# nabeelscicom/DistilCodec_nabeel

Hardware: AMD Instinct MI355X
Metric: 24 kHz samples/s encode+decode at 1/8 GPU; code-index bit-exact vs CPU (higher is better)
Workload: dtype f32

## Files before the change

### distilcodec_nabeel_amd/_native.py

```python
from __future__ import annotations

import ctypes
import glob
import hashlib
import os

import torch

_PKG = os.path.dirname(os.path.abspath(__file__))
LIB_PATH = os.environ.get("DCX_LIB") or os.path.join(_PKG, "libdcx.so")
CSRC = os.path.join(_PKG, "csrc")
HEADER = os.path.join(os.path.dirname(_PKG), "include", "distilcodec_amd.h")

DCX_OK = 0
DCX_ERR_INVALID_ARG = -1
DCX_ERR_MISSING_WEIGHT = -2
DCX_ERR_STATE = -3
DCX_ERR_HIP = -4
DCX_ERR_OOM = -5
DCX_ERR_WORKSPACE = -6
DCX_ERR_UNSUPPORTED = -7
DCX_GEMM_F32 = 0
DCX_GEMM_X6 = 1
DCX_GEMM_BF16 = 2


class NativeUnavailable(RuntimeError):
    pass


class NativeError(RuntimeError):
    def __init__(self, status: int, msg: str):
        super().__init__(f"dcx status {status}: {msg}")
        self.status = status


class DcxConfig(ctypes.Structure):
    _fields_ = [
        ("sample_rate", ctypes.c_int32),
        ("n_fft", ctypes.c_int32), ("hop", ctypes.c_int32), ("win", ctypes.c_int32),
        ("n_mels", ctypes.c_int32),
        ("f_min", ctypes.c_float), ("f_max", ctypes.c_float),
        ("enc_depths", ctypes.c_int32 * 4), ("enc_dims", ctypes.c_int32 * 4),
        ("vq_dim", ctypes.c_int32), ("codebook_dim", ctypes.c_int32), ("codebook_size", ctypes.c_int32),
        ("gen_channels", ctypes.c_int32), ("gen_pre_k", ctypes.c_int32), ("gen_post_k", ctypes.c_int32),
        ("n_ups", ctypes.c_int32), ("up_rates", ctypes.c_int32 * 8), ("up_kernels", ctypes.c_int32 * 8),
        ("n_res", ctypes.c_int32), ("res_kernels", ctypes.c_int32 * 4),
        ("res_dilations", (ctypes.c_int32 * 4) * 4),
    ]


_P = ctypes.c_void_p
_I32 = ctypes.c_int32
_I64 = ctypes.c_int64
_SZ = ctypes.c_size_t

SIGNATURES = {
    "dcx_default_config": (None, [ctypes.POINTER(DcxConfig)]),
    "dcx_create": (ctypes.c_int, [ctypes.POINTER(DcxConfig), ctypes.POINTER(_P)]),
    "dcx_destroy": (None, [_P]),
    "dcx_last_error": (ctypes.c_char_p, [_P]),
    "dcx_status_string": (ctypes.c_char_p, [ctypes.c_int]),
    "dcx_abi_version": (ctypes.c_int, []),
    "dcx_build_id": (ctypes.c_char_p, []),
    "dcx_set_tensor": (ctypes.c_int, [_P, ctypes.c_char_p, _P, _I32, ctypes.POINTER(_I64)]),
    "dcx_finalize": (ctypes.c_int, [_P, _I32]),
    "dcx_set_num_codebooks": (ctypes.c_int, [_P, _I32]),
    "dcx_num_codebooks": (_I32, [_P]),
    "dcx_num_frames": (_I64, [_P, _I64]),
    "dcx_workspace_size": (_SZ, [_P, _I32, _I64]),
    "dcx_mel": (ctypes.c_int, [_P, _P, _I32, _I64, _P, _P, _SZ, _P]),
    "dcx_mel_linear": (ctypes.c_int, [_P, _P, _I32, _I64, _P, _P, _P, _SZ, _P]),
    "dcx_encode": (ctypes.c_int, [_P, _P, _I32, _I64, _P, _P, _SZ, _P]),
    "dcx_vq_encode": (ctypes.c_int, [_P, _P, _I32, _I64, _P, _P, _P, _P, _P, _SZ, _P]),
    "dcx_vq_decode": (ctypes.c_int, [_P, _P, _I32, _I64, _P, _P, _P, _SZ, _P]),
    "dcx_generate": (ctypes.c_int, [_P, _P, _I32, _I64, _P, _P, _SZ, _P]),
    "dcx_encode_decode": (ctypes.c_int, [_P, _P, _I32, _I64, _P, _P, _P, _SZ, _P]),
    "dcx_ragged_plan_size": (_I64, [_I32]),
    "dcx_ragged_plan": (ctypes.c_int, [_P, ctypes.POINTER(_I64), _I32, _P, _I64, ctypes.POINTER(_I64),
                                       ctypes.POINTER(_I64)]),
    "dcx_ragged_workspace_size": (_SZ, [_P, _I32, _I64]),
    "dcx_tokenize_ragged": (ctypes.c_int, [_P, _P, _P, _P, _I32, _I64, _I64, _P, _P, _P, _P, _SZ, _P]),
    "dcx_generate_ragged": (ctypes.c_int, [_P, _P, _P, _I32, _I64, _P, _P, _SZ, _P]),
    "dcx_decode_ragged": (ctypes.c_int, [_P, _P, _P, _I32, _I64, _P, _P, _P, _SZ, _P]),
    "dcx_transpose": (ctypes.c_int, [_P, _P, _I32, _I64, _I64, _P]),
    "dcx_mp3_info": (ctypes.c_int, [_P, _SZ, ctypes.POINTER(_I64), ctypes.POINTER(_I32), ctypes.POINTER(_I32)]),
    "dcx_mp3_decode": (ctypes.c_int, [_P, _SZ, _P, _I64]),
    "dcx_mp3_last_error": (ctypes.c_char_p, []),
    "dcx_mp3_stats": (ctypes.c_int, [ctypes.POINTER(_I64), ctypes.POINTER(_I64)]),
    "dcx_mp3_junk_bytes": (_I64, []),
    "dcx_mp3_bad_frames": (_I64, []),
    "dcx_resample_poly": (ctypes.c_int, [_P, _I32, _I64, _I64, _P, _I32, _I32, _I32, _I64, _P, _I64, _I64, _P]),
    "dcx_set_gemm_mode": (ctypes.c_int, [_P, _I32]),
    "dcx_get_gemm_mode": (_I32, [_P]),
    "dcx_set_split_k": (ctypes.c_int, [_P, _I32]),
    "dcx_set_knob": (ctypes.c_int, [_P, ctypes.c_char_p, _I32]),
    "dcx_get_knob": (ctypes.c_int, [_P, ctypes.c_char_p, ctypes.POINTER(_I32)]),
    "dcx_range_flags": (ctypes.c_int, [_P, ctypes.POINTER(_I32), _I32]),
    "dcx_conv_create": (ctypes.c_int, [_P, _P, _I32, _I32, _I32, _I32, _I32, _I32, ctypes.POINTER(_P)]),
    "dcx_conv_forward": (ctypes.c_int, [_P, _I32, _P, _I32, _I64, _P, _P, _P, _I32, _P]),
    "dcx_conv_destroy": (None, [_P]),
    "dcx_conv_last_kernel": (ctypes.c_char_p, [_P]),
    "dcx_conv_set_knob": (ctypes.c_int, [_P, ctypes.c_char_p, _I32]),
    "dcx_conv_set_h3": (ctypes.c_int, [_P, _I32]),
    "dcx_module_workspace_size": (_SZ, [_P, ctypes.c_char_p, _I32, _I64]),
    "dcx_module_io": (ctypes.c_int, [_P, ctypes.c_char_p, ctypes.POINTER(_I32), ctypes.POINTER(_I32), ctypes.POINTER(_I32)]),
    "dcx_module_forward": (ctypes.c_int, [_P, ctypes.c_char_p, _P, _I32, _I64, _I32, _P, _P, _SZ, _P]),
    "dcx_vq_rescore_stats": (ctypes.c_int, [_P, ctypes.POINTER(_I64), ctypes.POINTER(_I64), _I32]),
    "dcx_profile_enable": (ctypes.c_int, [_P, _I32]),
    "dcx_profile_reset": (ctypes.c_int, [_P]),
    "dcx_profile_count": (_I32, [_P]),
    "dcx_profile_read": (ctypes.c_int, [_P, _I32, ctypes.POINTER(ctypes.c_char_p), ctypes.POINTER(_I64),
                                        ctypes.POINTER(ctypes.c_double), ctypes.POINTER(ctypes.c_double),
                                        ctypes.POINTER(ctypes.c_double)]),
}

_lib = None


def source_build_id() -> str | None:
    names = sorted(os.path.basename(p) for ext in ("cpp", "hip", "h") for p in glob.glob(os.path.join(CSRC, f"*.{ext}")))
    if not names or not os.path.isfile(HEADER):
        return None
    h = hashlib.sha256()
    for path in [os.path.join(CSRC, n) for n in names] + [HEADER]:
        with open(path, "rb") as f:
            h.update(f.read())
    return h.hexdigest()[:16]


def lib() -> ctypes.CDLL:
    global _lib
    if _lib is not None:
        return _lib
    if not os.path.isfile(LIB_PATH):
        raise NativeUnavailable(f"{LIB_PATH} is missing: run `python -c 'import __graft_entry__ as g; g.build()'`")
    try:
        L = ctypes.CDLL(LIB_PATH)
    except OSError as e:
        raise NativeUnavailable(f"cannot load {LIB_PATH}: {e}") from e
    for name, (res, args) in SIGNATURES.items():
        f = getattr(L, name)
        f.restype = res
        f.argtypes = args
    if L.dcx_abi_version() != 4:
        raise NativeUnavailable("libdcx.so ABI version mismatch")
    if not os.environ.get("DCX_LIB"):
        want, have = source_build_id(), L.dcx_build_id().decode()
        if want is not None and have != want:
            raise NativeUnavailable(f"{LIB_PATH} is stale: built from sources {have}, the sources here hash to {want}; "
                                    f"rebuild with `make -C {CSRC}`")
    _lib = L
    return L


def config_from_dict(cfg: dict) -> DcxConfig:
    c = DcxConfig()
    lib().dcx_default_config(ctypes.byref(c))
    s, e, d, q = cfg["spec_transform"], cfg["encoder"], cfg["decoder"], cfg["quantizer"]
    c.sample_rate, c.n_fft, c.hop, c.win = s["sampling_rate"], s["n_fft"], s["hop_size"], s["win_size"]
    c.n_mels, c.f_min, c.f_max = s["num_mels"], float(s["fmin"]), float(s["fmax"] or s["sampling_rate"] // 2)
    for i in range(4):
        c.enc_depths[i], c.enc_dims[i] = e["depths"][i], e["dims"][i]
    c.vq_dim, c.codebook_dim, c.codebook_size = q["input_dim"], q["codebook_dim"], q["codebook_size"]
    c.gen_channels, c.gen_pre_k, c.gen_post_k = d["upsample_initial_channel"], d["pre_conv_kernel_size"], d["post_conv_kernel_size"]
    c.n_ups = len(d["upsample_rates"])
    for i, (u, k) in enumerate(zip(d["upsample_rates"], d["upsample_kernel_sizes"])):
        c.up_rates[i], c.up_kernels[i] = u, k
    c.n_res = len(d["resblock_kernel_sizes"])
    for i, (k, dl) in enumerate(zip(d["resblock_kernel_sizes"], d["resblock_dilation_sizes"])):
        c.res_kernels[i] = k
        for j, v in enumerate(dl):
            c.res_dilations[i][j] = v
    return c
```

### distilcodec_nabeel_amd/csrc/dcx_api.cpp

```cpp
#include "dcx_host.h"

namespace {

void prof_collect(dcx_codec* h) {
  if (h->pending.empty()) return;
  hipDeviceSynchronize();
  for (auto& r : h->pending) {
    float ms = 0.f;
    hipEventElapsedTime(&ms, h->events[r.ev0], h->events[r.ev1]);
    h->prof_launches[r.id] += 1;
    h->prof_ms[r.id] += ms;
    h->prof_flops[r.id] += r.flops;
    h->prof_bytes[r.id] += r.bytes;
  }
  h->pending.clear();
  h->ev_used = 0;
}

constexpr int kPlanMagic = 0x52414731, kPlanHead = 8;
enum { PLAN_MAGIC = 0, PLAN_BATCH, PLAN_FRAMES, PLAN_SAMPLES, PLAN_T16, PLAN_T4, PLAN_RUN, PLAN_RW };
constexpr int64_t kRaggedMaxSamples = INT32_MAX, kRaggedMaxFrames = 1 << 20, kRaggedMaxBatch = 1 << 20;
int64_t plan_words(int64_t batch) { return kPlanHead + 5 * (batch + 1); }

bool seg_from_plan(const int32_t* host, const int32_t* dev, int64_t batch, int64_t samples, int64_t frames,
                   dcx::RaggedSeg& g) {
  if (host[PLAN_MAGIC] != kPlanMagic || host[PLAN_BATCH] != batch || host[PLAN_FRAMES] != frames ||
      host[PLAN_SAMPLES] != samples || batch < 1 || batch > kRaggedMaxBatch || frames < batch ||
      frames > kRaggedMaxFrames)
    return false;
  const int64_t n = batch + 1;
  const int32_t* a = dev + kPlanHead;
  g.cu_samples = a;
  g.cu_frames = a + n;
  g.cu_t16 = a + 2 * n;
  g.cu_t4 = a + 3 * n;
  g.cu_run = a + 4 * n;
  g.batch = (int)batch;
  g.rows = (int)frames;
  g.n_t16 = host[PLAN_T16];
  g.n_t4 = host[PLAN_T4];
  g.n_run = host[PLAN_RUN];
  g.rw = host[PLAN_RW];
  return g.rw == dcx::dwconv_run_rows(frames) && g.n_t16 >= batch && g.n_t16 <= frames && g.n_t4 >= g.n_t16 &&
         g.n_t4 <= frames && g.n_run >= batch && g.n_run <= frames;
}

int check_ready(dcx_codec* h, bool need_gen) {
  if (!h) return DCX_ERR_INVALID_ARG;
  if (!h->finalized) return fail(h, DCX_ERR_STATE, "dcx_finalize has not been called");
  if (need_gen && !h->has_gen) return fail(h, DCX_ERR_STATE, "generator weights were not finalized");
  int dev = -1;
  hipGetDevice(&dev);
  if (dev != h->device) return fail(h, DCX_ERR_STATE, "handle belongs to another HIP device");
  return DCX_OK;
}

int check_clip(dcx_codec* h, int64_t n) {
  if (n <= (h->cfg.win - h->cfg.hop) / 2 || frames_of(h->cfg, n) < 1)
    return fail(h, DCX_ERR_INVALID_ARG, "clip too short for the reflect pad / one STFT frame");
  return DCX_OK;
}

}

extern "C" {

int dcx_abi_version(void) { return DCX_ABI_VERSION; }

#ifndef DCX_BUILD_ID
#define DCX_BUILD_ID "unversioned"
#endif
const char* dcx_build_id(void) { return DCX_BUILD_ID; }

const char* dcx_status_string(int st) {
  switch (st) {
    case DCX_OK: return "ok";
    case DCX_ERR_INVALID_ARG: return "invalid argument";
    case DCX_ERR_MISSING_WEIGHT: return "missing weight";
    case DCX_ERR_STATE: return "invalid state";
    case DCX_ERR_HIP: return "HIP error";
    case DCX_ERR_OOM: return "out of device memory";
    case DCX_ERR_WORKSPACE: return "workspace too small";
    case DCX_ERR_UNSUPPORTED: return "unsupported input format";
    default: return "unknown status";
  }
}

void dcx_default_config(dcx_config* c) {
  std::memset(c, 0, sizeof(*c));
  c->sample_rate = 24000;
  c->n_fft = 1024; c->hop = 256; c->win = 1024; c->n_mels = 128;
  c->f_min = 0.f; c->f_max = 12000.f;
  const int dep[4] = {3, 3, 9, 3}, dim[4] = {256, 512, 768, 1024};
  for (int i = 0; i < 4; ++i) { c->enc_depths[i] = dep[i]; c->enc_dims[i] = dim[i]; }
  c->vq_dim = 1024; c->codebook_dim = 3584; c->codebook_size = 32768;
  c->gen_channels = 1024; c->gen_pre_k = 13; c->gen_post_k = 13;
  c->n_ups = 5;
  const int ur[5] = {8, 4, 2, 2, 2}, uk[5] = {16, 12, 4, 4, 4};
  for (int i = 0; i < 5; ++i) { c->up_rates[i] = ur[i]; c->up_kernels[i] = uk[i]; }
  c->n_res = 3;
  const int rk[3] = {3, 7, 11};
  for (int i = 0; i < 3; ++i) {
    c->res_kernels[i] = rk[i];
    c->res_dilations[i][0] = 1; c->res_dilations[i][1] = 3; c->res_dilations[i][2] = 5;
  }
}

const char* dcx_last_error(const dcx_codec* h) { return h ? h->err.c_str() : "null handle"; }

int dcx_create(const dcx_config* cfg, dcx_codec** out) {
  if (!cfg || !out) return DCX_ERR_INVALID_ARG;
  *out = nullptr;
  const dcx_config& c = *cfg;
  bool ok = c.n_fft == 1024 && c.win == 1024 && c.hop == 256 && c.n_mels % 16 == 0 && c.n_mels > 0 &&
            c.vq_dim == c.enc_dims[3] && c.codebook_dim % 16 == 0 && c.codebook_size % 128 == 0 &&
            c.n_ups >= 1 && c.n_ups <= 8 && c.n_res == 3 && c.gen_pre_k % 2 == 1 && c.gen_post_k % 2 == 1;
  for (int i = 0; i < 4 && ok; ++i) ok = c.enc_dims[i] % 256 == 0 && c.enc_dims[i] <= 1024 && c.enc_depths[i] >= 0;
  int ch = c.gen_channels;
  for (int i = 0; i < c.n_ups && ok; ++i) {
    ok = c.up_rates[i] >= 1 && c.up_rates[i] <= dcx::kMaxPhases && c.up_kernels[i] % c.up_rates[i] == 0 &&
         (c.up_kernels[i] - c.up_rates[i]) % 2 == 0;
    ch /= 2;
    ok = ok && ch % 32 == 0;
  }
  ok = ok && (ch == 32 || ch == 64);
  for (int i = 0; i < 3 && ok; ++i) ok = c.res_kernels[i] % 2 == 1;
  if (!ok) return DCX_ERR_INVALID_ARG;
  auto h = new (std::nothrow) dcx_codec();
  if (!h) return DCX_ERR_OOM;
  h->cfg = c;
  hipGetDevice(&h->device);
  const char* nrp = std::getenv("DCX_NO_RESPAIR");
  h->res_pair = !(nrp && nrp[0] == '1');
  const char* ncp = std::getenv("DCX_NO_COMPACT");
  h->compact = !(ncp && ncp[0] == '1');
  const char* vpr = std::getenv("DCX_VQ_PAIRS_PER_ROW");
  if (vpr && vpr[0]) h->vq_pairs_per_row = std::max(0, std::atoi(vpr));
  knobs_from_env(h->knobs);
  *out = h;
  return DCX_OK;
}

void dcx_destroy(dcx_codec* h) {
  if (!h) return;
  for (void* p : h->allocs) hipFree(p);
  for (auto e : h->events) hipEventDestroy(e);
  if (h->fork_ev) hipEventDestroy(h->fork_ev);
  if (h->join_ev) hipEventDestroy(h->join_ev);
  if (h->side) hipStreamDestroy(h->side);
  delete h;
}

int dcx_set_tensor(dcx_codec* h, const char* name, const float* data, int32_t ndim, const int64_t* shape) {
  if (!h || !name || (!data && ndim > 0) || ndim < 0 || ndim > 8) return fail(h, DCX_ERR_INVALID_ARG, "bad tensor");
  if (h->finalized) return fail(h, DCX_ERR_STATE, "dcx_set_tensor after dcx_finalize");
  HostTensor t;
  t.shape.assign(shape, shape + ndim);
  const int64_t n = t.numel();
  if (n < 0) return fail(h, DCX_ERR_INVALID_ARG, "negative shape");
  t.data.assign(data, data + n);
  h->host[name] = std::move(t);
  return DCX_OK;
}

int dcx_finalize(dcx_codec* h, int32_t with_generator) {
  if (!h) return DCX_ERR_INVALID_ARG;
  if (h->finalized) return fail(h, DCX_ERR_STATE, "already finalized");
  int rc = build_weights(h, true, with_generator);
  if (rc != DCX_OK) return rc;
  rc = build_weights(h, false, with_generator);
  if (rc != DCX_OK) return rc;
  h->has_gen = with_generator != 0;
  if (hipStreamCreateWithFlags(&h->side, hipStreamNonBlocking) != hipSuccess ||
      hipEventCreateWithFlags(&h->fork_ev, hipEventDisableTiming) != hipSuccess ||
      hipEventCreateWithFlags(&h->join_ev, hipEventDisableTiming) != hipSuccess)
    return fail(h, DCX_ERR_HIP, "dcx_finalize: stream / event creation failed");
  h->finalized = true;
  h->host.clear();
  return DCX_OK;
}

int dcx_set_num_codebooks(dcx_codec* h, int32_t n) {
  if (!h) return DCX_ERR_INVALID_ARG;
  if (h->finalized) return fail(h, DCX_ERR_STATE, "dcx_set_num_codebooks after dcx_finalize");
  if (n < 1 || n > DCX_MAX_CODEBOOKS)
    return fail(h, DCX_ERR_INVALID_ARG, "n_codebooks must be in [1, " + std::to_string(DCX_MAX_CODEBOOKS) + "]");
  h->n_layers = n;
  return DCX_OK;
}

int32_t dcx_num_codebooks(const dcx_codec* h) { return h ? h->n_layers : 0; }

int64_t dcx_num_frames(const dcx_codec* h, int64_t n) { return h ? frames_of(h->cfg, n) : 0; }

size_t dcx_workspace_size(const dcx_codec* h, int32_t batch, int64_t frames) {
  if (!h || batch <= 0 || frames <= 0) return 0;
  dcx_codec* hh = const_cast<dcx_codec*>(h);
  const int64_t n = (frames - 1) * h->cfg.hop + h->cfg.n_fft - (h->cfg.win - h->cfg.hop);
  Bump d(nullptr, 0, true);
  stage_encode_decode(hh, nullptr, batch, n, nullptr, nullptr, d, 0);
  size_t need = d.off;
  Bump q(nullptr, 0, true);
  stage_vq_encode(hh, CAct(), batch, (int)frames, nullptr, nullptr, nullptr, nullptr, q, 0);
  need = std::max(need, q.off + (size_t)batch * frames * (h->cfg.codebook_dim + h->cfg.vq_dim) * 4 + 1024);
  if (h->split_k > 1) need += kSplitScratch + 256;
  return need + 4096;
}

struct CallScope {
  dcx_codec* h;
  bool owner = false;
  explicit CallScope(dcx_codec* hh) : h(hh) {
    int expect = 0;
    owner = h && h->busy.compare_exchange_strong(expect, 1);
  }
  ~CallScope() {
    if (owner) {
      h->split_buf = nullptr;
      h->busy.store(0);
    }
  }
};

#define STAGE_PRE(need_gen)                                           \
  int rc_ = check_ready(h, need_gen);                                 \
  if (rc_ != DCX_OK) return rc_;                                      \
  if (batch <= 0) return fail(h, DCX_ERR_INVALID_ARG, "batch must be > 0"); \
  CallScope scope_(h);                                                \
  if (!scope_.owner) return fail(h, DCX_ERR_STATE, "handle in use by a concurrent call (serialise calls per handle)"); \
  hipStream_t s = (hipStream_t)stream;                                \
  Bump ws(workspace, ws_bytes, false);                                \
  h->split_buf = h->split_k > 1 ? (float*)ws.raw(kSplitScratch) : nullptr

int dcx_mel(dcx_codec* h, const float* audio, int32_t batch, int64_t n, float* mel, void* workspace, size_t ws_bytes,
            void* stream) {
  STAGE_PRE(false);
  if (!audio || !mel) return fail(h, DCX_ERR_INVALID_ARG, "null buffer");
  RUN(check_clip(h, n));
  return stage_mel(h, audio, batch, n, Act{mel, nullptr}, ws, s);
}

int dcx_mel_linear(dcx_codec* h, const float* audio, int32_t batch, int64_t n, float* mel, float* log_linear,
                   void* workspace, size_t ws_bytes, void* stream) {
  STAGE_PRE(false);
  if (!audio || !mel || !log_linear) return fail(h, DCX_ERR_INVALID_ARG, "null buffer");
  RUN(check_clip(h, n));
  return stage_mel(h, audio, batch, n, Act{mel, nullptr}, ws, s, log_linear);
}

int dcx_encode(dcx_codec* h, const float* mel, int32_t batch, int64_t frames, float* feat, void* workspace,
               size_t ws_bytes, void* stream) {
  STAGE_PRE(false);
  if (!mel || !feat || frames <= 0) return fail(h, DCX_ERR_INVALID_ARG, "bad arguments");
  return stage_encode(h, CAct(mel, nullptr), batch, (int)frames, Act{feat, nullptr}, ws, s);
}

int dcx_vq_encode(dcx_codec* h, const float* feat, int32_t batch, int64_t frames, int32_t* codes, float* x_pjt_in,
                  float* quantized_fup, float* quantized, void* workspace, size_t ws_bytes, void* stream) {
  STAGE_PRE(false);
  if (!feat || !codes || frames <= 0) return fail(h, DCX_ERR_INVALID_ARG, "bad arguments");
  return stage_vq_encode(h, CAct(feat, nullptr), batch, (int)frames, codes, x_pjt_in, quantized_fup, quantized, ws, s);
}

int dcx_vq_decode(dcx_codec* h, const int32_t* codes, int32_t batch, int64_t frames, float* z, int32_t* n_invalid,
                  void* workspace, size_t ws_bytes, void* stream) {
  STAGE_PRE(false);
  if (!codes || !z || frames <= 0) return fail(h, DCX_ERR_INVALID_ARG, "bad arguments");
  return stage_vq_decode(h, codes, batch, (int)frames, Act{z, nullptr}, n_invalid, ws, s);
}

int dcx_generate(dcx_codec* h, const float* z, int32_t batch, int64_t frames, float* wav, void* workspace,
                 size_t ws_bytes, void* stream) {
  STAGE_PRE(true);
  if (!z || !wav || frames <= 0) return fail(h, DCX_ERR_INVALID_ARG, "bad arguments");
  return stage_generate(h, CAct(z, nullptr), batch, (int)frames, wav, ws, s);
}

int dcx_encode_decode(dcx_codec* h, const float* audio, int32_t batch, int64_t n, int32_t* codes, float* wav,
                      void* workspace, size_t ws_bytes, void* stream) {
  STAGE_PRE(true);
  if (!audio || !codes || !wav) return fail(h, DCX_ERR_INVALID_ARG, "null buffer");
  RUN(check_clip(h, n));
  return stage_encode_decode(h, audio, batch, n, codes, wav, ws, s);
}

int64_t dcx_ragged_plan_size(int32_t batch) { return batch < 1 ? 0 : plan_words(batch); }

int dcx_ragged_plan(dcx_codec* h, const int64_t* clip_samples, int32_t batch, int32_t* plan, int64_t n_words,
                    int64_t* total_samples, int64_t* total_frames) {
  if (!h) return DCX_ERR_INVALID_ARG;
  if (batch < 1 || batch > kRaggedMaxBatch) return fail(h, DCX_ERR_INVALID_ARG, "ragged plan: batch must be in [1, 2^20]");
  if (!clip_samples || !plan) return fail(h, DCX_ERR_INVALID_ARG, "ragged plan: null buffer");
  if (n_words < plan_words(batch))
    return fail(h, DCX_ERR_INVALID_ARG, "ragged plan: the table holds " + std::to_string(n_words) + " words, " +
                                            std::to_string(plan_words(batch)) + " needed (dcx_ragged_plan_size)");
  const int64_t pad = (h->cfg.win - h->cfg.hop) / 2;
  const int64_t n = (int64_t)batch + 1;
  int32_t *cs = plan + kPlanHead, *cf = cs + n, *c16 = cf + n, *c4 = c16 + n, *cr = c4 + n;
  int64_t samples = 0, frames = 0;
  for (int32_t b = 0; b < batch; ++b) {
    const int64_t nb = clip_samples[b];
    if (nb < pad)
      return fail(h, DCX_ERR_INVALID_ARG, "ragged plan: clip " + std::to_string(b) + " has " + std::to_string(nb) +
                                              " samples, fewer than the reflect pad's " + std::to_string(pad));
    if (nb > kRaggedMaxSamples - samples)
      return fail(h, DCX_ERR_INVALID_ARG, "ragged plan: more than 2^31 - 1 samples in all (at clip " + std::to_string(b) + ")");
    samples += nb;
    frames += frames_of(h->cfg, nb + 1);
    if (frames > kRaggedMaxFrames)
      return fail(h, DCX_ERR_INVALID_ARG, "ragged plan: more than 2^20 frames in all (at clip " + std::to_string(b) + ")");
  }
  const int rw = dcx::dwconv_run_rows(frames);
  cs[0] = cf[0] = c16[0] = c4[0] = cr[0] = 0;
  for (int32_t b = 0; b < batch; ++b) {
    const int64_t T = frames_of(h->cfg, clip_samples[b] + 1);
    cs[b + 1] = (int32_t)(cs[b] + clip_samples[b]);
    cf[b + 1] = (int32_t)(cf[b] + T);
    c16[b + 1] = (int32_t)(c16[b] + (T + 15) / 16);
    c4[b + 1] = (int32_t)(c4[b] + (T + 3) / 4);
    cr[b + 1] = (int32_t)(cr[b] + (T + rw - 1) / rw);
  }
  plan[PLAN_MAGIC] = kPlanMagic;
  plan[PLAN_BATCH] = batch;
  plan[PLAN_FRAMES] = (int32_t)frames;
  plan[PLAN_SAMPLES] = (int32_t)samples;
  plan[PLAN_T16] = c16[batch];
  plan[PLAN_T4] = c4[batch];
  plan[PLAN_RUN] = cr[batch];
  plan[PLAN_RW] = rw;
  if (total_samples) *total_samples = samples;
  if (total_frames) *total_frames = frames;
  return DCX_OK;
}

size_t dcx_ragged_workspace_size(const dcx_codec* h, int32_t batch, int64_t total_frames) {
  if (!h || batch < 1 || total_frames < batch || total_frames > kRaggedMaxFrames) return 0;
  dcx::RaggedSeg g{};
  g.batch = batch;
  g.rows = (int)total_frames;
  Bump d(nullptr, 0, true);
  tokenize_ragged_rows(const_cast<dcx_codec*>(h), nullptr, g, nullptr, nullptr, nullptr, d, 0);
  return d.off + 4096;
}

int dcx_tokenize_ragged(dcx_codec* h, const float* audio_packed, const int32_t* plan_dev, const int32_t* plan_host,
                        int32_t batch, int64_t total_samples, int64_t total_frames, int32_t* codes, float* x_pjt_in,
                        float* quantized_fup, void* workspace, size_t ws_bytes, void* stream) {
  STAGE_PRE(false);
  if (!audio_packed || !plan_dev || !plan_host || !codes) return fail(h, DCX_ERR_INVALID_ARG, "null buffer");
  if (h->gemm_mode == DCX_GEMM_F32)
    return fail(h, DCX_ERR_INVALID_ARG, "dcx_tokenize_ragged runs in DCX_GEMM_X6 or DCX_GEMM_BF16 (the packed tensors are planes)");
  if (h->split_k >= 2)
    return fail(h, DCX_ERR_STATE, "dcx_tokenize_ragged with split-K on: the partial sums share one scratch region");
  dcx::RaggedSeg g{};
  if (!seg_from_plan(plan_host, plan_dev, batch, total_samples, total_frames, g))
    return fail(h, DCX_ERR_INVALID_ARG, "ragged plan does not match batch / total_samples / total_frames (dcx_ragged_plan)");
  return tokenize_ragged_rows(h, audio_packed, g, codes, x_pjt_in, quantized_fup, ws, s);
}

static int ragged_decode_pre(dcx_codec* h, const void* in, const int32_t* lengths_dev, int64_t frames_max,
                             const float* wav) {
  if (!in || !lengths_dev || !wav || frames_max <= 0 || frames_max > INT32_MAX / 256)
    return fail(h, DCX_ERR_INVALID_ARG, "ragged decode: null buffer or bad frames_max");
  if (h->split_k >= 2)
    return fail(h, DCX_ERR_STATE, "ragged decode with split-K on: the split kernels' reduce is not length-aware");
  if (h->gemm_mode != DCX_GEMM_X6)
    return fail(h, DCX_ERR_INVALID_ARG, "ragged decode runs in DCX_GEMM_X6 (the other modes' kernels are not length-aware)");
  return DCX_OK;
}

int dcx_generate_ragged(dcx_codec* h, const float* z, const int32_t* lengths_dev, int32_t batch, int64_t frames_max,
                        float* wav, void* workspace, size_t ws_bytes, void* stream) {
  if (h && (!z || !lengths_dev)) return fail(h, DCX_ERR_INVALID_ARG, "ragged decode: null buffer");
  STAGE_PRE(true);
  RUN(ragged_decode_pre(h, z, lengths_dev, frames_max, wav));
  return stage_generate(h, CAct(z, nullptr), batch, (int)frames_max, wav, ws, s, lengths_dev);
}

int dcx_decode_ragged(dcx_codec* h, const int32_t* codes, const int32_t* lengths_dev, int32_t batch,
                      int64_t frames_max, float* wav, int32_t* n_invalid, void* workspace, size_t ws_bytes,
                      void* stream) {
  if (h && (!codes || !lengths_dev)) return fail(h, DCX_ERR_INVALID_ARG, "ragged decode: null buffer");
  STAGE_PRE(true);
  RUN(ragged_decode_pre(h, codes, lengths_dev, frames_max, wav));
  return stage_decode_ragged(h, codes, lengths_dev, batch, (int)frames_max, wav, n_invalid, ws, s);
}

int dcx_module_io(const dcx_codec* h, const char* module, int32_t* in_channels, int32_t* out_channels,
                  int32_t* out_rate) {
  if (!h || !module) return DCX_ERR_INVALID_ARG;
  int ci = 0, co = 0, r = 1;
  if (!module_io(h, module, ci, co, r)) return DCX_ERR_INVALID_ARG;
  if (in_channels) *in_channels = ci;
  if (out_channels) *out_channels = co;
  if (out_rate) *out_rate = r;
  return DCX_OK;
}

size_t dcx_module_workspace_size(const dcx_codec* h, const char* module, int32_t batch, int64_t rows) {
  if (!h || !module || batch <= 0 || rows <= 0 || !h->finalized) return 0;
  Bump d(nullptr, 0, true);
  if (stage_module(const_cast<dcx_codec*>(h), module, nullptr, batch, (int)rows, nullptr, d, 0) != DCX_OK) return 0;
  return d.off + 4096 + (h->split_k > 1 ? kSplitScratch + 256 : 0);
}

int dcx_module_forward(dcx_codec* h, const char* module, const float* x, int32_t batch, int64_t rows,
                       int32_t channels, void* y, void* workspace, size_t ws_bytes, void* stream) {
  STAGE_PRE(false);
  if (!module || !x || !y || rows <= 0 || rows > (1 << 30)) return fail(h, DCX_ERR_INVALID_ARG, "bad arguments");
  int ci = 0, co = 0, r = 1;
  if (!module_io(h, module, ci, co, r)) return fail(h, DCX_ERR_INVALID_ARG, std::string("unknown module: ") + module);
  if (channels != ci)
    return fail(h, DCX_ERR_INVALID_ARG, std::string(module) + " takes " + std::to_string(ci) + " input channels, got " +
                                            std::to_string(channels));
  return stage_module(h, module, x, batch, (int)rows, y, ws, s);
}

int dcx_transpose(const float* in, float* out, int32_t batch, int64_t rows, int64_t cols, void* stream) {
  if (!in || !out || batch <= 0 || rows <= 0 || cols <= 0) return DCX_ERR_INVALID_ARG;
  return dcx::launch_transpose(in, out, batch, rows, cols, (hipStream_t)stream) == hipSuccess ? DCX_OK : DCX_ERR_HIP;
}

int dcx_resample_poly(const float* x, int32_t batch, int64_t n_in, int64_t x_stride, const double* h, int32_t h_len,
                      int32_t up, int32_t down, int64_t pre, float* y, int64_t n_out, int64_t y_stride, void* stream) {
  if (!x || !h || !y || batch <= 0 || n_in <= 0 || n_out <= 0 || h_len <= 0 || up <= 0 || down <= 0 || pre < 0 ||
      x_stride < n_in || y_stride < n_out || batch > 65535)
    return DCX_ERR_INVALID_ARG;
  if ((pre + n_out) > (INT64_MAX / down)) return DCX_ERR_INVALID_ARG;
  return dcx::launch_resample_poly(x, batch, n_in, x_stride, h, h_len, up, down, pre, y, n_out, y_stride,
                                   (hipStream_t)stream) == hipSuccess
             ? DCX_OK
             : DCX_ERR_HIP;
}

int dcx_set_gemm_mode(dcx_codec* h, int32_t mode) {
  if (!h) return DCX_ERR_INVALID_ARG;
  if (mode != DCX_GEMM_F32 && mode != DCX_GEMM_X6 && mode != DCX_GEMM_BF16)
    return fail(h, DCX_ERR_INVALID_ARG, "unknown GEMM mode");
  h->gemm_mode = mode;
  return DCX_OK;
}

int32_t dcx_get_gemm_mode(const dcx_codec* h) { return h ? h->gemm_mode : -1; }

int dcx_set_split_k(dcx_codec* h, int32_t max_splits) {
  if (!h || max_splits < 0 || max_splits > kSplitMax) return DCX_ERR_INVALID_ARG;
  h->split_k = max_splits;
  return DCX_OK;
}

int dcx_set_knob(dcx_codec* h, const char* name, int32_t value) {
  if (!h || !name) return DCX_ERR_INVALID_ARG;
  CallScope scope(h);
  if (!scope.owner) return fail(h, DCX_ERR_STATE, "dcx_set_knob during a stage call");
  const auto k = knob_slot(name);
  if (!k) return fail(h, DCX_ERR_INVALID_ARG, std::string("unknown knob: ") + name);
  h->knobs.*k = value;
  return DCX_OK;
}

int dcx_get_knob(const dcx_codec* h, const char* name, int32_t* value) {
  if (!h || !name || !value) return DCX_ERR_INVALID_ARG;
  const auto k = knob_slot(name);
  if (!k) return DCX_ERR_INVALID_ARG;
  *value = h->knobs.*k;
  return DCX_OK;
}

int dcx_range_flags(dcx_codec* h, int32_t* flags, int32_t reset) {
  if (!h || !flags) return DCX_ERR_INVALID_ARG;
  *flags = 0;
  if (!h->rflag) return DCX_OK;
  int v = 0;
  if (hipDeviceSynchronize() != hipSuccess || hipMemcpy(&v, h->rflag, sizeof v, hipMemcpyDeviceToHost) != hipSuccess)
    return fail(h, DCX_ERR_HIP, "reading the range flags failed");
  *flags = v;
  if (reset && hipMemset(h->rflag, 0, sizeof v) != hipSuccess) return fail(h, DCX_ERR_HIP, "resetting the range flags failed");
  return DCX_OK;
}

}

struct dcx_conv {
  dcx_codec scratch;
  ConvW w;
  unsigned short* planes = nullptr;
  size_t planes_cap = 0;
  bool h3 = false;
  int* range = nullptr;
  size_t range_cap = 0;
};

template <class T>
static bool grow(T*& p, size_t& cap, size_t need) {
  if (need <= cap) return true;
  if (p) hipFree(p);
  p = nullptr;
  cap = 0;
  if (hipMalloc(&p, need * sizeof(T)) != hipSuccess) return false;
  cap = need;
  return true;
}

extern "C" {

int dcx_conv_create(const float* weight, const float* bias, int32_t cin, int32_t cout, int32_t k, int32_t dilation,
                    int32_t transposed, int32_t stride, dcx_conv** out) {
  if (!weight || !out || cin <= 0 || cout <= 0 || k <= 0 || dilation <= 0 || stride <= 0) return DCX_ERR_INVALID_ARG;
  if (cin % 16 || cout % 32) return DCX_ERR_INVALID_ARG;
  if (transposed && (k % stride || (k - stride) % 2 || stride > dcx::kMaxPhases)) return DCX_ERR_INVALID_ARG;
  if (!transposed && (k % 2 == 0)) return DCX_ERR_INVALID_ARG;
  auto c = new (std::nothrow) dcx_conv();
  if (!c) return DCX_ERR_OOM;
  dcx_codec* h = &c->scratch;
  HostTensor wt;
  const int64_t n = (int64_t)cin * cout * k;
  wt.shape = transposed ? std::vector<int64_t>{cin, cout, k} : std::vector<int64_t>{cout, cin, k};
  wt.data.assign(weight, weight + n);
  h->host["c.weight"] = wt;
  HostTensor bt;
  bt.shape = {cout};
  if (bias) bt.data.assign(bias, bias + cout); else bt.data.assign(cout, 0.f);
  h->host["c.bias"] = bt;
  const int code = build_conv(h, cin, cout, k, dilation, transposed != 0, stride, c->w);
  h->host.clear();
  if (code != DCX_OK) {
    dcx_conv_destroy(c);
    return code;
  }
  *out = c;
  return DCX_OK;
}

int dcx_conv_forward(dcx_conv* c, int32_t gemm_mode, const float* x, int32_t batch, int64_t lin, float* y,
                     float* y_silu, const float* res, int32_t epi, void* stream) {
  if (!c || !x || batch <= 0 || lin <= 0 || (!y && !y_silu)) return DCX_ERR_INVALID_ARG;
  if (epi != dcx::EPI_BIAS && epi != dcx::EPI_GELU && epi != dcx::EPI_RES) return DCX_ERR_INVALID_ARG;
  if (epi == dcx::EPI_RES && !res) return DCX_ERR_INVALID_ARG;
  dcx_codec* h = &c->scratch;
  h->gemm_mode = gemm_mode;
  hipStream_t s = (hipStream_t)stream;
  CAct xa(x, nullptr);
  if (gemm_mode != DCX_GEMM_F32 && gemm_mode != DCX_GEMM_X6 && gemm_mode != DCX_GEMM_BF16) return DCX_ERR_INVALID_ARG;
  if (gemm_mode != DCX_GEMM_F32 && !f32_input_ok(c->w)) {
    const size_t need = (size_t)batch * lin * c->w.cin * 3;
    if (!grow(c->planes, c->planes_cap, need)) return DCX_ERR_OOM;
    const bool h3 = c->h3 && (c->w.taps >= 2 ? takes_h3_conv(h, c->w, lin) : takes_h3(h, c->w));
    if (h3) {
      const long long rows = (long long)batch * lin;
      const size_t words = (size_t)batch + (size_t)std::max<long long>(batch, rows);
      if (!grow(c->range, c->range_cap, words)) return DCX_ERR_OOM;
      float* am = reinterpret_cast<float*>(c->range);
      int* ash = c->range + batch;
      xa.r = Rng{};
      if (c->w.taps >= 2) {
        if (dcx::launch_h2_ranged(x, nullptr, c->planes, batch, lin, c->w.cin, 0, 0.f, am, ash, h->rflag, s) != hipSuccess)
          return fail(h, DCX_ERR_HIP, "h3 input split (per clip) failed");
        xa.r.ash = ash;
        xa.r.amax = am;
      } else {
        if (dcx::launch_h2_rows(x, c->planes, rows, c->w.cin, ash, s) != hipSuccess)
          return fail(h, DCX_ERR_HIP, "h3 input split (per row) failed: Cin must be 256, 512, 768, 1024 or a multiple of 32 below 256");
        xa.r.ash_row = ash;
      }
      xa.lay = dcx::LAYOUT_H2;
    } else if (dcx::launch_split_planes(x, c->planes, (long long)batch * lin, c->w.cin, dcx::LAYOUT_PLANES, s) != hipSuccess) {
      return DCX_ERR_HIP;
    }
    xa.p = c->planes;
  }
  ConvCall cc = framed(xa, batch, (int)lin, c->w.cin);
  cc.y = y;
  cc.y2 = y_silu;
  cc.res = res;
  cc.epi = epi;
  return run_conv(h, c->w, cc, s);
}

void dcx_conv_destroy(dcx_conv* c) {
  if (!c) return;
  if (c->planes) hipFree(c->planes);
  if (c->range) hipFree(c->range);
  for (void* p : c->scratch.allocs) hipFree(p);
  delete c;
}

const char* dcx_conv_last_kernel(const dcx_conv* c) { return c ? c->scratch.last_kname : ""; }

int dcx_conv_set_knob(dcx_conv* c, const char* name, int32_t value) {
  if (!c || !name) return DCX_ERR_INVALID_ARG;
  const auto k = knob_slot(name);
  if (!k) return fail(&c->scratch, DCX_ERR_INVALID_ARG, std::string("unknown knob: ") + name);
  c->scratch.knobs.*k = value;
  return DCX_OK;
}

int dcx_conv_set_h3(dcx_conv* c, int32_t on) {
  if (!c) return DCX_ERR_INVALID_ARG;
  c->h3 = on != 0;
  return DCX_OK;
}

int dcx_profile_enable(dcx_codec* h, int32_t on) {
  if (!h) return DCX_ERR_INVALID_ARG;
  h->prof = on != 0;
  return DCX_OK;
}

int dcx_profile_reset(dcx_codec* h) {
  if (!h) return DCX_ERR_INVALID_ARG;
  prof_collect(h);
  for (size_t i = 0; i < h->prof_names.size(); ++i) {
    h->prof_launches[i] = 0;
    h->prof_ms[i] = h->prof_flops[i] = h->prof_bytes[i] = 0;
  }
  return DCX_OK;
}

int dcx_vq_rescore_stats(dcx_codec* h, int64_t* rows_rescored, int64_t* codes_rescored, int32_t reset) {
  if (!h || !h->vq_stats) return DCX_ERR_STATE;
  h->vq_stats_on = true;
  int v[2] = {0, 0};
  if (hipDeviceSynchronize() != hipSuccess || hipMemcpy(v, h->vq_stats, sizeof v, hipMemcpyDeviceToHost) != hipSuccess)
    return fail(h, DCX_ERR_HIP, "reading VQ rescore counters failed");
  if (rows_rescored) *rows_rescored = v[0];
  if (codes_rescored) *codes_rescored = v[1];
  if (reset && hipMemset(h->vq_stats, 0, sizeof v) != hipSuccess)
    return fail(h, DCX_ERR_HIP, "resetting VQ rescore counters failed");
  return DCX_OK;
}

int32_t dcx_profile_count(const dcx_codec* h) { return h ? (int32_t)h->prof_names.size() : 0; }

int dcx_profile_read(dcx_codec* h, int32_t i, const char** name, int64_t* launches, double* ms, double* flops,
                     double* bytes) {
  if (!h) return DCX_ERR_INVALID_ARG;
  prof_collect(h);
  if (i < 0 || i >= (int32_t)h->prof_names.size()) return DCX_ERR_INVALID_ARG;
  if (name) *name = h->prof_names[i].c_str();
  if (launches) *launches = h->prof_launches[i];
  if (ms) *ms = h->prof_ms[i];
  if (flops) *flops = h->prof_flops[i];
  if (bytes) *bytes = h->prof_bytes[i];
  return DCX_OK;
}

}
```

### distilcodec_nabeel_amd/csrc/dcx_conv_common.h

```cpp
#pragma once
#include <algorithm>
#include <type_traits>

#include "dcx_kernels.h"
#include "dcx_planes.h"

namespace dcx {

typedef float f32x16 __attribute__((ext_vector_type(16)));
typedef float f32x4 __attribute__((ext_vector_type(4)));
typedef float f32x2 __attribute__((ext_vector_type(2)));
typedef short s16x8 __attribute__((ext_vector_type(8)));
typedef short s16x4 __attribute__((ext_vector_type(4)));
typedef __bf16 bf16x8 __attribute__((ext_vector_type(8)));

constexpr int BK = 16;
constexpr int LDSK = 20;
template <bool SWZ>
struct XRow {
  static constexpr int kStride = SWZ ? 48 : 56;
  __device__ static __forceinline__ int half(int row, int h) { return SWZ ? h ^ ((row >> 3) & 1) : h; }
  __device__ static __forceinline__ int off(int row, int piece) {
    const int h = piece >= 3;
    return row * kStride + (half(row, h) * 3 + piece - 3 * h) * 8;
  }
};

__device__ __forceinline__ float silu_f(float v) { return v * __builtin_amdgcn_rcpf(1.0f + __expf(-v)); }
__device__ __forceinline__ float gelu_f(float v) { return 0.5f * v * (1.0f + erff(v * 0.70710678118654752440f)); }
__device__ __forceinline__ float gelu_bf16_f(float v) {
#ifdef DCX_GELU_ERF
  return gelu_f(v);
#endif
  const float z = fabsf(v) * 0.70710678118654752440f;
  const float t = __builtin_amdgcn_rcpf(fmaf(0.5f, z, 1.0f));
  float q = 0.17087277f;
  q = fmaf(q, t, -0.82215223f);
  q = fmaf(q, t, 1.48851587f);
  q = fmaf(q, t, -1.13520398f);
  q = fmaf(q, t, 0.27886807f);
  q = fmaf(q, t, -0.18628806f);
  q = fmaf(q, t, 0.09678418f);
  q = fmaf(q, t, 0.37409196f);
  q = fmaf(q, t, 1.00002368f);
  const float c = t * __expf(fmaf(t, q, fmaf(-z, z, -1.26551223f)));
  const float e = v >= 0.0f ? 1.0f - c : c - 1.0f;
  return 0.5f * v * (1.0f + e);
}

__device__ __forceinline__ f32x2 gelu_bf16_f2(f32x2 v) {
#ifdef DCX_GELU_SCALAR
  return f32x2{gelu_bf16_f(v[0]), gelu_bf16_f(v[1])};
#endif
  const f32x2 z = __builtin_elementwise_abs(v) * 0.70710678118654752440f;
  const f32x2 d = __builtin_elementwise_fma(f32x2{0.5f, 0.5f}, z, f32x2{1.0f, 1.0f});
  const f32x2 t = {__builtin_amdgcn_rcpf(d[0]), __builtin_amdgcn_rcpf(d[1])};
  auto fm = [&](f32x2 q, float c) { return __builtin_elementwise_fma(q, t, f32x2{c, c}); };
  f32x2 q = {0.17087277f, 0.17087277f};
  q = fm(q, -0.82215223f);
  q = fm(q, 1.48851587f);
  q = fm(q, -1.13520398f);
  q = fm(q, 0.27886807f);
  q = fm(q, -0.18628806f);
  q = fm(q, 0.09678418f);
  q = fm(q, 0.37409196f);
  q = fm(q, 1.00002368f);
  const f32x2 arg = __builtin_elementwise_fma(t, q, __builtin_elementwise_fma(-z, z, f32x2{-1.26551223f, -1.26551223f}));
  const f32x2 c = t * f32x2{__expf(arg[0]), __expf(arg[1])};
  const f32x2 e = {v[0] >= 0.0f ? 1.0f - c[0] : c[0] - 1.0f, v[1] >= 0.0f ? 1.0f - c[1] : c[1] - 1.0f};
  return 0.5f * v * (1.0f + e);
}

__device__ __forceinline__ int xcd_remap(int bid, int nwg) {
  const int xcd = bid & 7, q = nwg >> 3, r = nwg & 7;
  return (xcd < r ? xcd * (q + 1) : r * (q + 1) + (xcd - r) * q) + (bid >> 3);
}

__device__ __forceinline__ void flat_tile(int tpc, int batch, int& wg, int& b, int& ph) {
  const int t = xcd_remap(blockIdx.x, gridDim.x);
  const int per_ph = tpc * batch;
  ph = t / per_ph;
  const int r = t - ph * per_ph;
  b = r / tpc;
  wg = r - b * tpc;
}

__device__ __forceinline__ void ksplit_slice(const ConvParams& p, int b, int& clip, int& c0, int& nchunks) {
  clip = b;
  c0 = 0;
  nchunks = p.Cin / BK;
  if (p.ksplit > 1) {
    const int clips = p.batch / p.ksplit, sl = b / clips;
    clip = b - sl * clips;
    const int nunits = nchunks / p.kunit, base = nunits / p.ksplit, extra = nunits % p.ksplit;
    c0 = (sl * base + min(sl, extra)) * p.kunit;
    nchunks = (base + (sl < extra ? 1 : 0)) * p.kunit;
  }
}

static __device__ __attribute__((used, aligned(16))) float g_zero_row[32] = {0.f};

#if defined(DCX_CLOCK_DIAG) || defined(DCX_SEG_DIAG) || defined(DCX_TILE_DIAG)
#define DCX_DIAG 1
constexpr int kTileDiagMax = 16384;
[[maybe_unused]] static __device__ unsigned long long g_clock_diag[3], g_seg_diag[13], g_seg_diag8[49];
[[maybe_unused]] static __device__ unsigned long long g_tile_diag[kTileDiagMax * 6];
[[maybe_unused]] static __device__ unsigned int g_tile_cnt;
enum DiagSet : int { DIAG_CLOCK, DIAG_SEG, DIAG_SEG8, DIAG_TILES };
static int diag_read(int set, unsigned long long* out, int n, int reset) {
  if (set == DIAG_TILES) {
    unsigned int cnt = 0;
    if (hipMemcpyFromSymbol(&cnt, HIP_SYMBOL(g_tile_cnt), sizeof cnt) != hipSuccess) return -1;
    cnt = std::min(cnt, (unsigned)std::max(0, std::min(n, kTileDiagMax)));
    if (cnt && hipMemcpyFromSymbol(out, HIP_SYMBOL(g_tile_diag), sizeof(unsigned long long) * 6 * cnt) != hipSuccess) return -1;
    const unsigned int z = 0;
    if (reset && hipMemcpyToSymbol(HIP_SYMBOL(g_tile_cnt), &z, sizeof z) != hipSuccess) return -1;
    return (int)cnt;
  }
  const void* sym = set == DIAG_CLOCK ? (const void*)g_clock_diag : set == DIAG_SEG ? (const void*)g_seg_diag : (const void*)g_seg_diag8;
  unsigned long long v[49] = {};
  if (n > 49 || hipMemcpyFromSymbol(v, sym, sizeof(unsigned long long) * n) != hipSuccess) return -1;
  for (int i = 0; i < n; ++i) out[i] += v[i];
  const unsigned long long z[49] = {};
  if (reset && hipMemcpyToSymbol(sym, z, sizeof(unsigned long long) * n) != hipSuccess) return -1;
  return 0;
}
#define DCX_DIAG_FILE(tag) \
  int diag_##tag(int set, unsigned long long* out, int n, int reset) { return diag_read(set, out, n, reset); }
#else
#define DCX_DIAG_FILE(tag)
#endif
#ifdef DCX_SEG_DIAG
#define DCX_SEGT(v) const unsigned long long v = __builtin_amdgcn_s_memtime()
#else
#define DCX_SEGT(v)
#endif
#ifdef DCX_TILE_DIAG
#define DCX_TILET(v) const unsigned long long v = __builtin_amdgcn_s_memrealtime()
#else
#define DCX_TILET(v)
#endif

struct EpiPre {
  int osh;
  float acur;
  bool track;
};
template <int RROW>
__device__ __forceinline__ EpiPre epi_range_pre(const ConvParams& p, const ConvParams& pr, int b) {
  EpiPre e{0, 0.f, false};
  const bool h2o = (p.y6 && p.y_layout == LAYOUT_H2) || (p.y6s && p.ys_layout != LAYOUT_PLANES);
  const bool h2row = (RROW & 2) && h2o && pr.yb.rowwise;
  if (h2o && !h2row) {
    const float bnd = range_bound(pr.yb, b);
    e.osh = __builtin_amdgcn_readfirstlane(h2_shift(bnd));
    if (threadIdx.x == 0) {
      if (pr.y_ash) pr.y_ash[b] = e.osh;
      if (pr.rflag && !(bnd <= 3.0e38f)) atomicOr(pr.rflag, RANGE_NONFINITE);
    }
  }
  const bool track = pr.y_amax != nullptr;
  e.track = track;
  e.acur = track && !h2row ? __builtin_bit_cast(float, __builtin_amdgcn_readfirstlane(
                                                           __builtin_bit_cast(int, range_cur(pr.y_amax, b))))
                           : 0.f;
  return e;
}

template <int BM, int BN, int WM, int WN, int LDS_FLOATS, int NT, int RROW = 2, bool RAG = true, typename AccT>
__device__ __forceinline__ void epilogue_lds(const ConvParams& p, const ConvParams& pr, AccT& acc, int q0, int co0,
                                             int b, int ph, float* smem, const EpiPre* pre = nullptr) {
  constexpr int WR = BM / WM, WC = BN / WN;
  constexpr int TM = WR / 32, TN = WC / 32;
  constexpr bool M16 = sizeof(acc[0][0]) == 16;
  static_assert(sizeof(acc) == WR * WC * 4 / 64, "accumulator tile");
  constexpr int LDSW = BN + 4;
  constexpr int RPP = (BM * LDSW <= LDS_FLOATS) ? BM
                      : (BM / 2 * LDSW <= LDS_FLOATS) ? BM / 2
                      : (BM / 4 * LDSW <= LDS_FLOATS) ? BM / 4 : WR;
  static_assert(RPP % WR == 0 && RPP * LDSW <= LDS_FLOATS, "epilogue pass does not fit LDS");
  const int tid = threadIdx.x, lane = tid & 63, wave = tid >> 6;
  const int wm = wave / WN, wn = wave % WN;
  const int lrow = lane & 31, rhalf = 4 * (lane >> 5);
  const long long ob = (long long)b * p.y_bstride;
  unsigned short* y6 = p.y6 ? p.y6 + ob * layout_u16(p.y_layout) : nullptr;
  unsigned short* y6s = p.y6s ? p.y6s + ob * (p.ys_layout != LAYOUT_PLANES ? 2 : 3) : nullptr;
  const bool h2o = (y6 && p.y_layout == LAYOUT_H2) || (y6s && p.ys_layout != LAYOUT_PLANES);
  constexpr bool RIN = RROW & 1, ROUT = RROW & 2;
  const bool h2row = ROUT && h2o && pr.yb.rowwise;
  int osh = 0;
  if (pre) {
    osh = pre->osh;
  } else if (h2o && !h2row) {
    const float bnd = range_bound(pr.yb, b);
    osh = __builtin_amdgcn_readfirstlane(h2_shift(bnd));
    if (tid == 0) {
      if (pr.y_ash) pr.y_ash[b] = osh;
      if (pr.rflag && !(bnd <= 3.0e38f)) atomicOr(pr.rflag, RANGE_NONFINITE);
    }
  }
  const float osc =
      __builtin_bit_cast(float, __builtin_amdgcn_readfirstlane(__builtin_bit_cast(int, __builtin_ldexpf(1.0f, osh))));
#ifdef DCX_DIAG_NORANGE
  const bool track = false;
#else
  const bool track = pre ? pre->track : pr.y_amax != nullptr;
#endif
  const float acur = pre ? pre->acur : track && !h2row ? range_cur(pr.y_amax, b) : 0.f;
  float vmax = 0.f;
  const int lq_live = RAG ? clip_rows(pr.clip_len, pr.len_mul, b, p.Lq) : p.Lq;
#ifdef DCX_EPI4
  constexpr int G = 4;
#else
  constexpr int G = 8;
#endif
  constexpr int NH = G / 4;
  static_assert(NT % (BN / G) == 0, "each thread keeps one channel group");
  const int cg = (tid % (BN / G)) * G, trow = tid / (BN / G), co = co0 + cg;
  const int hsw = G == 8 ? (lane >> 3) & 1 : 0;
  f32x4 bias4[NH], gamma4[NH];
#pragma unroll
  for (int h = 0; h < NH; ++h) {
    bias4[h] = p.bias ? *reinterpret_cast<const f32x4*>(p.bias + co + 4 * h) : f32x4{0.f, 0.f, 0.f, 0.f};
    gamma4[h] = p.epi == EPI_GAMMA_RES ? *reinterpret_cast<const f32x4*>(p.gamma + co + 4 * h) : f32x4{0.f, 0.f, 0.f, 0.f};
  }
#ifdef DCX_DIAG_NOEPI
  if (q0 >= 0) return;
#endif
#ifdef DCX_DIAG_DUP
  if (p.diag_skip == 2) return;
#endif
  auto stage_acc = [&](int r0) {
    __syncthreads();
    if (wm * WR >= r0 && wm * WR < r0 + RPP) {
      if constexpr (M16) {
#pragma unroll
        for (int i = 0; i < WR / 16; ++i)
#pragma unroll
          for (int j = 0; j < WC / 16; ++j)
#pragma unroll
            for (int e = 0; e < 4; ++e) {
              const int row = wm * WR + i * 16 + 4 * (lane >> 4) + e - r0;
              smem[row * LDSW + wn * WC + j * 16 + (lane & 15)] = acc[i][j][e];
            }
      } else {
#pragma unroll
        for (int i = 0; i < TM; ++i)
#pragma unroll
          for (int j = 0; j < TN; ++j)
#pragma unroll
            for (int r = 0; r < 16; ++r) {
              const int row = wm * WR + i * 32 + (r & 3) + 8 * (r >> 2) + rhalf - r0;
              smem[row * LDSW + wn * WC + j * 32 + lrow] = acc[i][j][r];
            }
      }
    }
    __syncthreads();
  };
  constexpr int RSTEP = NT / (BN / G), ROWS_T = RPP / RSTEP;
  static_assert(RPP % RSTEP == 0, "epilogue rows per thread");
  const bool need_r = p.epi == EPI_GAMMA_RES || p.epi == EPI_RES;
  const bool need_m = p.mean_mode == MEAN_MID || p.mean_mode == MEAN_LAST;
  auto batch = [&](int r0, int rb, bool stage, auto ibt) {
    constexpr int IB = decltype(ibt)::value;
    f32x4 r[IB][NH], m[IB][NH];
    auto lofs = [&](int k) {
      const int q = min(q0 + r0 + trow + (rb + k) * RSTEP, p.Lq - 1);
      return ob + ((long long)q * p.out_mul + ph) * p.ldy + co;
    };
    if (need_r) {
#pragma unroll
      for (int k = 0; k < IB; ++k)
#pragma unroll
        for (int h = 0; h < NH; ++h) r[k][h] = *reinterpret_cast<const f32x4*>(p.res + lofs(k) + 4 * h);
    }
    if (need_m) {
#pragma unroll
      for (int k = 0; k < IB; ++k)
#pragma unroll
        for (int h = 0; h < NH; ++h) m[k][h] = *reinterpret_cast<const f32x4*>(p.macc + lofs(k) + 4 * h);
    }
    auto row_bound = [&](int q) { return fmaf(pr.yb.g[0], fmaxf(pr.yb.m[0][(long long)b * p.Lq + q], pr.yb.f[0]), pr.yb.c); };
    float rin[RIN ? IB : 1], rbnd[RIN ? IB : 1];
    if constexpr (RIN) {
#pragma unroll
      for (int k = 0; k < IB; ++k) {
        const int q = min(q0 + r0 + trow + (rb + k) * RSTEP, p.Lq - 1);
        rin[k] = pr.x_ash_row ? __builtin_ldexpf(1.0f, -pr.x_ash_row[(long long)b * p.Lin + q]) : 1.0f;
        rbnd[k] = h2row ? row_bound(q) : 0.f;
      }
    }
    if (stage) stage_acc(r0);
#pragma unroll
    for (int k = 0; k < IB; ++k) {
      const int rl = trow + (rb + k) * RSTEP;
      const int q = q0 + r0 + rl;
      if (q >= p.Lq) continue;
      const long long orow = (long long)q * p.out_mul + ph;
      const long long o = ob + orow * p.ldy + co;
      f32x4 x[NH];
      const float rin_ = RIN ? rin[RIN ? k : 0] : 1.0f;
      if constexpr (NH == 2) {
        const f32x4 u = *reinterpret_cast<const f32x4*>(smem + rl * LDSW + cg + 4 * hsw);
        const f32x4 v = *reinterpret_cast<const f32x4*>(smem + rl * LDSW + cg + 4 * (1 - hsw));
        x[0] = (hsw ? v : u) * rin_ + bias4[0];
        x[1] = (hsw ? u : v) * rin_ + bias4[1];
      } else {
        x[0] = *reinterpret_cast<const f32x4*>(smem + rl * LDSW + cg) * rin_ + bias4[0];
      }
#pragma unroll
      for (int h = 0; h < NH; ++h) {
        if (p.round_bf16) x[h] = round_bf16x4(x[h]);
        switch (p.epi) {
          case EPI_GELU:
            if (p.w6) {
#ifndef DCX_EPI_NOGELU
#pragma unroll
              for (int e = 0; e < 4; e += 2) {
                const f32x2 g = gelu_bf16_f2(f32x2{x[h][e], x[h][e + 1]});
                x[h][e] = g[0];
                x[h][e + 1] = g[1];
              }
#endif
              if (p.round_bf16 && (p.y || y6s || p.y2 || p.y_layout != LAYOUT_BF16)) x[h] = round_bf16x4(x[h]);
            } else {
#pragma unroll
              for (int e = 0; e < 4; ++e) x[h][e] = gelu_f(x[h][e]);
            }
            break;
          case EPI_GAMMA_RES: x[h] = r[k][h] + gamma4[h] * x[h]; break;
          case EPI_RES:
            x[h] = r[k][h] + x[h];
            if (p.round_bf16) x[h] = round_bf16x4(x[h]);
            break;
          case EPI_LOGCLAMP:
#pragma unroll
            for (int e = 0; e < 4; ++e) x[h][e] = logf(fmaxf(x[h][e], 1e-5f));
            break;
          default: break;
        }
        if (RAG && q >= lq_live) x[h] = f32x4{0.f, 0.f, 0.f, 0.f};
      }
#ifdef DCX_EPI_NOSTORE
      if (x[0][0] != -0x1.234p-100f) continue;
#endif
#ifdef DCX_DIAG_DUP
      if (p.diag_skip == 1 && x[0][0] != -0x1.234p-100f) continue;
#endif
      if (p.mean_mode == MEAN_FIRST) {
#pragma unroll
        for (int h = 0; h < NH; ++h) *reinterpret_cast<f32x4*>(p.macc + o + 4 * h) = x[h];
        continue;
      } else if (p.mean_mode == MEAN_MID) {
#pragma unroll
        for (int h = 0; h < NH; ++h) *reinterpret_cast<f32x4*>(p.macc + o + 4 * h) = RAG && q >= lq_live ? x[h] : m[k][h] + x[h];
        continue;
      } else if (p.mean_mode == MEAN_LAST) {
#pragma unroll
        for (int h = 0; h < NH; ++h) {
          x[h] = RAG && q >= lq_live ? x[h] : (m[k][h] + x[h]) / 3.0f;
          if (p.round_bf16) x[h] = round_bf16x4(x[h]);
        }
      }
      float rsc = osc;
      if (h2row) {
        const long long grow = (long long)b * p.Lq + q;
        const float bnd = RIN ? rbnd[RIN ? k : 0] : row_bound(q);
        const int sh = h2_shift(bnd);
        rsc = __builtin_ldexpf(1.0f, sh);
        if (cg == 0 && pr.y_ash) pr.y_ash[grow] = sh;
        if (pr.rflag && !(bnd <= 3.0e38f)) atomicOr(pr.rflag, RANGE_NONFINITE);
      }
      if (track) {
        const float ts = h2row ? rsc : 1.0f;
#pragma unroll
        for (int h = 0; h < NH; ++h)
#pragma unroll
          for (int e = 0; e < 4; ++e) vmax = fmaxf(vmax, fabsf(x[h][e]) * ts);
      }
      if (p.y) {
#pragma unroll
        for (int h = 0; h < NH; ++h) *reinterpret_cast<f32x4*>(p.y + o + 4 * h) = x[h];
      }
      if constexpr (G == 8) {
        float xv[8];
#pragma unroll
        for (int e = 0; e < 8; ++e) xv[e] = x[e >> 2][e & 3];
        if (y6) {
          if (p.y_layout == LAYOUT_BF16) store_bf16x8(y6, orow, p.Cout, co, xv);
          else if ((int)p.y_layout == 2) store_hm8(y6, orow, p.Cout, co, xv);
          else if (p.y_layout == LAYOUT_H2) store_h2_8<false>(y6, orow, p.Cout, co, xv, rsc);
          else store_planes8(y6, orow, p.Cout, co, xv);
        }
        if (p.y2 || y6s) {
          float sv[8];
#pragma unroll
          for (int e = 0; e < 8; ++e) sv[e] = p.round_bf16 ? bf16_val(bf16_bits(silu_f(xv[e]))) : silu_f(xv[e]);
          if (p.y2) {
            *reinterpret_cast<f32x4*>(p.y2 + o) = f32x4{sv[0], sv[1], sv[2], sv[3]};
            *reinterpret_cast<f32x4*>(p.y2 + o + 4) = f32x4{sv[4], sv[5], sv[6], sv[7]};
          }
          if (y6s) {
            if (p.ys_layout != LAYOUT_PLANES) store_h2_8<false>(y6s, orow, p.Cout, co, sv, rsc);
            else store_planes8(y6s, orow, p.Cout, co, sv);
          }
        }
      } else {
        if (y6) {
          if (p.y_layout == LAYOUT_BF16) store_bf16x4(y6, orow, p.Cout, co, x[0][0], x[0][1], x[0][2], x[0][3]);
          else if ((int)p.y_layout == 2) store_hm4(y6, orow, p.Cout, co, x[0][0], x[0][1], x[0][2], x[0][3]);
          else if (p.y_layout == LAYOUT_H2) store_h2_4<false>(y6, orow, p.Cout, co, x[0][0], x[0][1], x[0][2], x[0][3], rsc);
          else store_planes4(y6, orow, p.Cout, co, x[0][0], x[0][1], x[0][2], x[0][3]);
        }
        if (p.y2 || y6s) {
          f32x4 sv;
#pragma unroll
          for (int e = 0; e < 4; ++e) sv[e] = p.round_bf16 ? bf16_val(bf16_bits(silu_f(x[0][e]))) : silu_f(x[0][e]);
          if (p.y2) *reinterpret_cast<f32x4*>(p.y2 + o) = sv;
          if (y6s) {
            if (p.ys_layout != LAYOUT_PLANES) store_h2_4<false>(y6s, orow, p.Cout, co, sv[0], sv[1], sv[2], sv[3], rsc);
            else store_planes4(y6s, orow, p.Cout, co, sv[0], sv[1], sv[2], sv[3]);
          }
        }
      }
    }
  };
  constexpr int IBF0 = 8 / NH, IBM0 = 4 / NH;
  constexpr auto div_cap = [](int n, int cap) {
    int d = n < cap ? n : cap;
    while (n % d) --d;
    return d;
  };
  constexpr int IBF = div_cap(ROWS_T, IBF0), IBM = div_cap(ROWS_T, IBM0);
  static_assert(ROWS_T % IBF == 0 && ROWS_T % IBM == 0, "epilogue batches");
#pragma unroll 1
  for (int r0 = 0; r0 < BM; r0 += RPP) {
    if (need_m) {
#pragma unroll
      for (int rb = 0; rb < ROWS_T; rb += IBM) batch(r0, rb, rb == 0, std::integral_constant<int, IBM>{});
    } else {
#pragma unroll
      for (int rb = 0; rb < ROWS_T; rb += IBF) batch(r0, rb, rb == 0, std::integral_constant<int, IBF>{});
    }
  }
  if (track)
    range_report_wg(vmax, h2row ? nullptr : pr.y_amax, b, h2row ? 65504.0f : h2o ? 65504.0f / osc : __builtin_inff(),
                    pr.rflag, acur, smem, NT);
}

__device__ __forceinline__ bool tile_dead(const ConvParams& p, const ConvParams& pr, int b, int q0) {
  return pr.clip_len != nullptr && q0 >= clip_rows(pr.clip_len, pr.len_mul, b, p.Lq);
}
template <int BM, int BN, int NT>
__device__ __forceinline__ void epilogue_dead(const ConvParams& p, const ConvParams& pr, int q0, int co0, int b, int ph) {
  const long long ob = (long long)b * p.y_bstride;
  unsigned short* y6 = p.y6 ? p.y6 + ob * layout_u16(p.y_layout) : nullptr;
  unsigned short* y6s = p.y6s ? p.y6s + ob * (p.ys_layout != LAYOUT_PLANES ? 2 : 3) : nullptr;
  const bool h2o = (y6 && p.y_layout == LAYOUT_H2) || (y6s && p.ys_layout != LAYOUT_PLANES);
  if (h2o && threadIdx.x == 0) {
    const float bnd = range_bound(pr.yb, b);
    if (pr.y_ash) pr.y_ash[b] = h2_shift(bnd);
    if (pr.rflag && !(bnd <= 3.0e38f)) atomicOr(pr.rflag, RANGE_NONFINITE);
  }
  const f32x4 z4 = {0.f, 0.f, 0.f, 0.f};
  const float z8[8] = {0.f, 0.f, 0.f, 0.f, 0.f, 0.f, 0.f, 0.f};
  constexpr int CG = BN / 8;
  for (int i = threadIdx.x; i < BM * CG; i += NT) {
    const int q = q0 + i / CG, co = co0 + (i % CG) * 8;
    if (q >= p.Lq) break;
    const long long orow = (long long)q * p.out_mul + ph;
    const long long o = ob + orow * p.ldy + co;
    if (p.mean_mode == MEAN_FIRST || p.mean_mode == MEAN_MID) {
      *reinterpret_cast<f32x4*>(p.macc + o) = z4;
      *reinterpret_cast<f32x4*>(p.macc + o + 4) = z4;
      continue;
    }
    if (p.y) {
      *reinterpret_cast<f32x4*>(p.y + o) = z4;
      *reinterpret_cast<f32x4*>(p.y + o + 4) = z4;
    }
    if (y6) {
      if (p.y_layout == LAYOUT_BF16) store_bf16x8(y6, orow, p.Cout, co, z8);
      else if (p.y_layout == LAYOUT_H2) store_h2_8<false>(y6, orow, p.Cout, co, z8, 1.0f);
      else store_planes8(y6, orow, p.Cout, co, z8);
    }
    if (p.y2) {
      *reinterpret_cast<f32x4*>(p.y2 + o) = z4;
      *reinterpret_cast<f32x4*>(p.y2 + o + 4) = z4;
    }
    if (y6s) {
      if (p.ys_layout != LAYOUT_PLANES) store_h2_8<false>(y6s, orow, p.Cout, co, z8, 1.0f);
      else store_planes8(y6s, orow, p.Cout, co, z8);
    }
  }
}

typedef __attribute__((address_space(3))) void* lds_ptr_t;

__device__ __forceinline__ void dma16(__amdgpu_buffer_rsrc_t r, unsigned short* lds, int voff, int soff) {
  __builtin_amdgcn_raw_ptr_buffer_load_lds(r, (lds_ptr_t)lds, 16, voff, soff, 0, 0);
}
__device__ __forceinline__ void seg_barrier() { asm volatile("s_waitcnt lgkmcnt(0)\n\ts_barrier" ::: "memory"); }
__device__ __forceinline__ void wait_dma(int n) {
#define DCX_W(k) \
  case k: asm volatile("s_waitcnt vmcnt(" #k ")" ::: "memory"); break;
  switch (n) {
    DCX_W(1) DCX_W(2) DCX_W(3) DCX_W(4) DCX_W(5) DCX_W(6) DCX_W(7) DCX_W(8) DCX_W(9) DCX_W(10) DCX_W(11)
    DCX_W(12) DCX_W(13) DCX_W(14) DCX_W(15) DCX_W(16) DCX_W(17) DCX_W(18) DCX_W(19) DCX_W(20) DCX_W(21) DCX_W(22)
    DCX_W(23)
    default: asm volatile("s_waitcnt vmcnt(0)" ::: "memory");
  }
#undef DCX_W
}

}
```

### distilcodec_nabeel_amd/csrc/dcx_conv_h3.hip

```cpp
#include "dcx_conv_common.h"
#include "dcx_conv_launch.h"
#include "dcx_conv_pingpong.h"
#include "dcx_a3_layout.h"
#include "dcx_w3_layout.h"

namespace dcx {

DCX_DIAG_FILE(h3)

typedef _Float16 f16x8 __attribute__((ext_vector_type(8)));

template <int BM, int BN>
__device__ __forceinline__ bool ragged_tile_done(const ConvParams& p, const ConvParams& pr, int wg, int b, int ph) {
  int q0, co0;
  tile_origin<BM, BN>(p, wg, q0, co0);
  if (!tile_dead(p, pr, b, q0)) return false;
  epilogue_dead<BM, BN, 512>(p, pr, q0, co0, b, ph);
  return true;
}

template <int BN, int HALO, bool RAG = false>
__device__ __forceinline__ void x3dq_tile(const ConvParams& p, const ConvParams& pr, const int wg, const int b, const int ph) {
  constexpr int BM = 32768 / BN, WN = BN / 64, WM = 8 / WN;
  constexpr int NA = HALO ? 2 : 3;
  constexpr int WR = BM / WM, WC = BN / WN, TM = WR / 16, TN = WC / 16;
  constexpr int AR = BM + HALO;
  constexpr int A_G = AR / 16, B_G = BN / 16;
  constexpr int A_PW = A_G / 4, B_PW = B_G / 4;
  constexpr int ABUF = AR * 128, BBUF = BN * 128;
  constexpr int LDS_B = NA * ABUF + 3 * BBUF;
  static_assert(WR == 64 && WC == 64 && A_G % 4 == 0 && B_G % 4 == 0 && AR % 64 == 0, "tile shape");
  static_assert(LDS_B <= 160 * 1024, "LDS");
  __shared__ __attribute__((aligned(16))) unsigned short lds[LDS_B / 2];

  if constexpr (RAG)
    if (ragged_tile_done<BM, BN>(p, pr, wg, b, ph)) return;
  const TileGeo g = tile_geo<BM, BN, WN>(p, wg, ph, p.Cin / 32);
  const int lane = g.lane, group = g.group, gw = g.gw, wm = g.wm, wn = g.wn, q0 = g.q0, co0 = g.co0;
  const int nchunks = g.nchunks, taps = g.taps, nsteps = g.nsteps, lo_rel = g.lo_rel, row0 = g.row0;
  const int arow = p.ldx * 4;
  const __amdgpu_buffer_rsrc_t rx = x_desc<4, HALO>(p, b, row0, BM);
  const int rbase = HALO ? row0 : 0;
  const __amdgpu_buffer_rsrc_t rw = __builtin_amdgcn_make_buffer_rsrc(
      (void*)(p.w3 + w3_step(taps, p.Cin, p.Cout, ph, 0, 0)), 0, taps * nchunks * p.Cout * 128, 0x00020000);

  int a_off[A_PW], b_off[B_PW];
#pragma unroll
  for (int i = 0; i < A_PW; ++i) {
    const int u = (group * A_G + i * 4 + gw) * 64;
    const int pc = u / AR, row = u - pc * AR + lane;
    a_off[i] = (rbase + row) * arow + (pc & 3) * 32 + (pc >> 2) * 16;
  }
#pragma unroll
  for (int i = 0; i < B_PW; ++i) {
    b_off[i] = w3_wide_lane(co0, lane) + w3_wide_piece(BN, group * B_G + i * 4 + gw);
  }
  unsigned short* const a_dst = lds + (group * A_G + gw) * 512;
  unsigned short* const b_dst = lds + NA * ABUF / 2 + (group * B_G + gw) * 512;
  [[maybe_unused]] bool in_loop = false;
  auto dma_step = [&](int c, int m, int slot) {
#ifdef DCX_X3_NODMA
    if (in_loop) return 0;
#endif
    int n = B_PW;
    if (m == 0) {
#pragma unroll
      for (int i = 0; i < A_PW; ++i)
        dma16(rx, a_dst + (HALO ? (c & 1) : slot) * (ABUF / 2) + i * 2048, a_off[i] + c * 128, 0);
      n += A_PW;
    }
    const int soff = w3_step_bytes(nchunks, p.Cout, m, c);
#pragma unroll
    for (int i = 0; i < B_PW; ++i) dma16(rw, b_dst + slot * (BBUF / 2) + i * 2048, b_off[i], soff);
    return n;
  };

  const int l15 = lane & 15, kg = lane >> 4;
  const int pah = kg * AR * 16, pal = (4 + kg) * AR * 16;
  const int pbh = kg * BN * 16, pbl = (4 + kg) * BN * 16;
  const char* const ldsb = reinterpret_cast<const char*>(lds);
  const int bcol = NA * ABUF + (wn * WC + l15) * 16;
  s16x8 aq[TM][2], bq[TN][2];
  auto readF = [&](int c, int m, int slot) {
    const char* a = ldsb + (HALO ? (c & 1) : slot) * ABUF + (wm * WR + m * p.in_step - lo_rel + l15) * 16;
    const char* bb = ldsb + bcol + slot * BBUF;
#pragma unroll
    for (int j = 0; j < TN; ++j) {
      bq[j][0] = *reinterpret_cast<const s16x8*>(bb + j * 256 + pbh);
      bq[j][1] = *reinterpret_cast<const s16x8*>(bb + j * 256 + pbl);
    }
#pragma unroll
    for (int i = 0; i < TM; ++i) {
      aq[i][0] = *reinterpret_cast<const s16x8*>(a + i * 256 + pah);
      aq[i][1] = *reinterpret_cast<const s16x8*>(a + i * 256 + pal);
    }
  };
  f32x4 acc[TM][TN];
  zero_acc(acc);
  auto mfma = [&]() {
    __builtin_amdgcn_s_setprio(1);
#pragma unroll
    for (int k = 0; k < 3; ++k) {
      const int sa = k == 1 ? 1 : 0, sb = k == 0 ? 1 : 0;
#pragma unroll
      for (int i = 0; i < TM; ++i)
#pragma unroll
        for (int j = 0; j < TN; ++j)
          acc[i][j] = __builtin_amdgcn_mfma_f32_16x16x32_f16(__builtin_bit_cast(f16x8, aq[i][sa]),
                                                             __builtin_bit_cast(f16x8, bq[j][sb]), acc[i][j], 0, 0, 0);
    }
    __builtin_amdgcn_s_setprio(0);
  };

  const StepPos l3 = pingpong3_prologue(nsteps, taps, dma_step);
  const EpiPre epre = epi_range_pre<HALO == 0 ? 3 : 0>(p, pr, b);
  const float unscale = __builtin_bit_cast(float, __builtin_amdgcn_readfirstlane(__builtin_bit_cast(int,
      __builtin_ldexpf(1.0f, -(p.w3_shift + (pr.x_ash ? pr.x_ash[b] : pr.x_ash_c))))));
  pingpong3_drain();
  in_loop = true;
  pingpong3_loop<true>(group, nsteps, taps, l3, dma_step, readF, mfma);
#pragma unroll
  for (int i = 0; i < TM; ++i)
#pragma unroll
    for (int j = 0; j < TN; ++j) acc[i][j] *= unscale;
  epilogue_lds<BM, BN, WM, WN, LDS_B / 4, 512, HALO == 0 ? 3 : 0, RAG>(p, pr, acc, q0, co0, b, ph, reinterpret_cast<float*>(lds), &epre);
}

template <int BN, int HALO, bool RAG = false>
__global__ void __launch_bounds__(512, 2) conv_gemm_x3dq(const ConvParams p) {
  int wg, b, ph;
  flat_tile(((p.Lq + 32768 / BN - 1) / (32768 / BN)) * (p.Cout / BN), p.batch, wg, b, ph);
  x3dq_tile<BN, HALO, RAG>(p, p, wg, b, ph);
}

template <int BN, bool RAG = false>
__global__ void __launch_bounds__(512, 2) conv_gemm_x3dq_group(const ConvGroup g) {
  ConvParams p;
  int local, b;
  const ConvParams& pr = group_member(g, p, local, b);
  x3dq_tile<BN, 64, RAG>(p, pr, local, b, 0);
}

template <int HALO, bool SPLIT, int BN = 256, bool RAG = false, bool GROUPED = false>
__device__ __forceinline__ void x3dw_tile(const ConvParams& p, const ConvParams& pr, const int wg, const int b, const int ph) {
  constexpr int BM = BN == 256 ? 256 : 384, WN = BN / 128, WM = 8 / WN;
  constexpr int WR = BM / WM, WC = 128, TM = WR / 16, TN = WC / 16;
  constexpr int AR = BM + HALO;
  constexpr int A_N = AR / 8, B_N = BN / 8;
  constexpr int A_PW = A_N / 4;
  constexpr int ABUF = AR * 128, BBUF = BN * 128;
  constexpr int NA = 2;
  constexpr int LDS_B = NA * ABUF + 2 * BBUF;
  static_assert(A_N % 4 == 0 && B_N % 4 == 0 && AR % 64 == 0, "tile shape");
  static_assert(LDS_B + 16 <= 160 * 1024, "LDS");
  __shared__ __attribute__((aligned(16))) unsigned short lds[LDS_B / 2 + 8];
  unsigned int* const rd_cnt = reinterpret_cast<unsigned int*>(lds + LDS_B / 2);

  const int tid = threadIdx.x, lane = tid & 63;
  [[maybe_unused]] const int wave = tid >> 6;
  const int group = __builtin_amdgcn_readfirstlane(tid >> 8);
  const int gw = __builtin_amdgcn_readfirstlane((tid >> 6) & 3);
  const int wm = wave / WN, wn = wave % WN;
  const int ntiles = p.Cout / BN;
  const int mt = wg / ntiles, nt = wg - mt * ntiles;
  const int q0 = mt * BM, co0 = nt * BN;
  if (RAG && tile_dead(p, pr, b, q0)) {
    epilogue_dead<BM, BN, 512>(p, pr, q0, co0, b, ph);
    return;
  }
  const int nchunks = p.Cin / 32;
  const int taps = p.taps;
  const int nsteps = nchunks * taps;
  const int lo_rel = p.in_step < 0 ? (taps - 1) * p.in_step : 0;
  const int row0 = q0 + p.in_base[ph] + lo_rel;
  const int arow = p.ldx * 4;
  const __amdgpu_buffer_rsrc_t rx = x_desc<4, HALO>(p, b, row0, BM);
  const int rbase = HALO ? row0 : 0;
  const __amdgpu_buffer_rsrc_t rw = __builtin_amdgcn_make_buffer_rsrc(
      (void*)(p.w3 + w3_step(taps, p.Cin, p.Cout, ph, 0, 0)), 0, taps * nchunks * p.Cout * 128, 0x00020000);

  constexpr bool ROWS = !(HALO && !SPLIT && BN == 256 && !RAG && !GROUPED);
  const int a_lane = ROWS ? a3_src_lane(rbase, arow, lane) : (rbase + lane) * arow;
  const int b_lane = w3_wide_lane(co0, lane);
  [[maybe_unused]] bool in_loop = false;
  auto dmaA1 = [&](int c, int slot, int i) {
#ifdef DCX_X3_NODMA
    if (in_loop) return;
#endif
    const int k = i * 4 + gw;
    const int abuf = HALO ? (c & 1) : slot;
    if constexpr (ROWS) {
      dma16(rx, lds + abuf * (ABUF / 2) + k * 512, a_lane + a3_src_inst(arow, k, c), 0);
    } else {
      const int u = k * 64, pc = u / AR, row = u - pc * AR;
      dma16(rx, lds + abuf * (ABUF / 2) + k * 512, a_lane + row * arow + (pc & 3) * 32 + (pc >> 2) * 16 + c * 128, 0);
    }
  };
#ifndef DCX_X3W_BG0_DIV
#define DCX_X3W_BG0_DIV 2
#endif
  constexpr int B_G0 = !SPLIT ? B_N : HALO ? B_N / DCX_X3W_BG0_DIV : 0;
  constexpr int B_W0 = B_G0 / 4, B_W1 = (B_N - B_G0) / 4;
  auto dmaB1 = [&](int c, int m, int slot, int i) {
#ifdef DCX_X3_NODMA
    if (in_loop) return;
#endif
    const int k = (group ? B_G0 : 0) + i * 4 + gw;
    dma16(rw, lds + NA * ABUF / 2 + slot * (BBUF / 2) + k * 512, b_lane, w3_step_bytes(nchunks, p.Cout, m, c) + w3_wide_piece(BN, k));
  };
  auto dma_step = [&](int c, int m, int slot) {
    if (m == 0) {
#pragma unroll
      for (int i = 0; i < A_PW; ++i) dmaA1(c, slot, i);
    }
#pragma unroll
    for (int i = 0; i < B_W0; ++i) dmaB1(c, m, slot, i);
  };
  auto dma_step1 = [&](int c, int m, int slot) {
#pragma unroll
    for (int i = 0; i < B_W1; ++i) dmaB1(c, m, slot, i);
  };

  const int l15 = lane & 15, kg = lane >> 4;
  const char* const ldsb = reinterpret_cast<const char*>(lds);
  const int a_row = wm * WR + l15;
  static_assert(WR % kA3BlockRows == 0 && a3_image(16, 0) == 2048, "row blocks as immediates");
  const char* const b_rd = ldsb + NA * ABUF + kg * BN * 16 + (wn * WC + l15) * 16;
  s16x8 aq[TM][2], bq[TN][2];
  auto readF = [&](int c, int m, int slot) {
    const int a_r = a_row + (HALO ? m * p.in_step - lo_rel : 0);
    const int ah = (HALO ? (c & 1) : slot) * ABUF + (ROWS ? a3_image(a_r, kg) : kg * AR * 16 + a_r * 16);
    const char* a = ldsb + ah;
    const char* al = ldsb + (ROWS ? ah ^ kA3PlaneXor : ah + 4 * AR * 16);
    const char* bb = b_rd + slot * BBUF;
#pragma unroll
    for (int j = 0; j < TN; ++j) {
      bq[j][0] = *reinterpret_cast<const s16x8*>(bb + j * 256);
      bq[j][1] = *reinterpret_cast<const s16x8*>(bb + j * 256 + 4 * BN * 16);
    }
#pragma unroll
    for (int i = 0; i < TM; ++i) {
      aq[i][0] = *reinterpret_cast<const s16x8*>(a + i * (ROWS ? 2048 : 256));
      aq[i][1] = *reinterpret_cast<const s16x8*>(al + i * (ROWS ? 2048 : 256));
    }
  };
  f32x4 acc[TM][TN];
  zero_acc(acc);
  auto mfma = [&]() {
    __builtin_amdgcn_s_setprio(1);
#pragma unroll
    for (int k = 0; k < 3; ++k) {
      const int sa = k == 1 ? 1 : 0, sb = k == 0 ? 1 : 0;
#pragma unroll
      for (int i = 0; i < TM; ++i) {
#pragma unroll
        for (int j = 0; j < TN; ++j)
          acc[i][j] = __builtin_amdgcn_mfma_f32_16x16x32_f16(__builtin_bit_cast(f16x8, aq[i][sa]),
                                                             __builtin_bit_cast(f16x8, bq[j][sb]), acc[i][j], 0, 0, 0);
      }
    }
    __builtin_amdgcn_s_setprio(0);
  };

  int cl = 0, ml = 0;
  if (SPLIT && tid == 0) *rd_cnt = 0u;
  for (int t = 0; t < 2 && t < nsteps; ++t) {
    if (group == 0) dma_step(cl, ml, t);
    else if (SPLIT) dma_step1(cl, ml, t);
    step_adv(cl, ml, taps);
  }
  const EpiPre epre = epi_range_pre<HALO == 0 ? 3 : 0>(p, pr, b);
  const float unscale = __builtin_bit_cast(float, __builtin_amdgcn_readfirstlane(__builtin_bit_cast(int,
      __builtin_ldexpf(1.0f, -(p.w3_shift + (pr.x_ash ? pr.x_ash[b] : pr.x_ash_c))))));
  asm volatile("s_waitcnt vmcnt(0)" ::: "memory");
  seg_barrier();
  in_loop = true;
#ifdef DCX_SEG_DIAG
  unsigned long long sd[6] = {};
#endif
  int cr = 0, mr = 0;
  if (group == 0) {
    readF(0, 0, 0);
    if (SPLIT) {
      asm volatile("s_waitcnt lgkmcnt(0)" ::: "memory");
      if (lane == 0) __hip_atomic_fetch_add(rd_cnt, 1u, __ATOMIC_RELAXED, __HIP_MEMORY_SCOPE_WORKGROUP);
    }
    step_adv(cr, mr, taps);
    for (int s = 0; s < nsteps; ++s) {
      DCX_SEGT(ta);
      mfma();
      asm volatile("s_waitcnt vmcnt(0)" ::: "memory");
      DCX_SEGT(tb);
      seg_barrier();
      DCX_SEGT(tc);
      if (s + 2 < nsteps) {
        dma_step(cl, ml, s & 1);
        step_adv(cl, ml, taps);
      }
      DCX_SEGT(tr);
      if (s + 1 < nsteps) readF(cr, mr, (s + 1) & 1);
      DCX_SEGT(tq);
      DCX_SEGT(td);
      seg_barrier();
      DCX_SEGT(te);
#ifdef DCX_SEG_DIAG
      sd[0] += tb - ta; sd[1] += tc - tb; sd[2] += td - tc; sd[3] += te - td; sd[4] += tr - tc; sd[5] += tq - tr;
#endif
      step_adv(cr, mr, taps);
    }
  } else {
    for (int s = 0; s < nsteps; ++s) {
      DCX_SEGT(ta);
      readF(cr, mr, s & 1);
      if (SPLIT) {
        int n = 0;
        if (s + 2 < nsteps) {
          asm volatile("s_waitcnt lgkmcnt(0)" ::: "memory");
          if (lane == 0) __hip_atomic_fetch_add(rd_cnt, 1u, __ATOMIC_RELAXED, __HIP_MEMORY_SCOPE_WORKGROUP);
          const unsigned int want = 4u * (unsigned)(s + 2);
          while (__hip_atomic_load(rd_cnt, __ATOMIC_RELAXED, __HIP_MEMORY_SCOPE_WORKGROUP) < want) {
          }
          dma_step1(cl, ml, s & 1);
          step_adv(cl, ml, taps);
          n = B_W1;
        }
        wait_dma(n);
      }
      DCX_SEGT(tb);
      seg_barrier();
      DCX_SEGT(tc);
      mfma();
      DCX_SEGT(td);
      seg_barrier();
      DCX_SEGT(te);
#ifdef DCX_SEG_DIAG
      sd[2] += tb - ta; sd[3] += tc - tb; sd[0] += td - tc; sd[1] += te - td; sd[5] += tb - ta;
#endif
      step_adv(cr, mr, taps);
    }
  }
#ifdef DCX_SEG_DIAG
  if ((threadIdx.x & 255) == 0) {
#pragma unroll
    for (int i = 0; i < 6; ++i) atomicAdd(&g_seg_diag[group * 6 + i], sd[i]);
    if (group == 0) atomicAdd(&g_seg_diag[12], (unsigned long long)nsteps);
  }
  if (lane == 0) {
#pragma unroll
    for (int i = 0; i < 6; ++i) atomicAdd(&g_seg_diag8[wave * 6 + i], sd[i]);
    if (wave == 0) atomicAdd(&g_seg_diag8[48], (unsigned long long)nsteps);
  }
#endif
  asm volatile("s_waitcnt vmcnt(0)" ::: "memory");
#pragma unroll
  for (int i = 0; i < TM; ++i)
#pragma unroll
    for (int j = 0; j < TN; ++j) acc[i][j] *= unscale;
  epilogue_lds<BM, BN, WM, WN, LDS_B / 4, 512, HALO == 0 ? 3 : 0, RAG>(p, pr, acc, q0, co0, b, ph, reinterpret_cast<float*>(lds), &epre);
}

template <int HALO, bool SPLIT, int BN = 256, bool RAG = false>
__global__ void __launch_bounds__(512, 2) conv_gemm_x3dw(const ConvParams p) {
  constexpr int BM = BN == 256 ? 256 : 384;
  int wg, b, ph;
  flat_tile(((p.Lq + BM - 1) / BM) * (p.Cout / BN), p.batch, wg, b, ph);
  x3dw_tile<HALO, SPLIT, BN, RAG>(p, p, wg, b, ph);
}

template <bool SPLIT, int BN = 256, bool RAG = false>
__global__ void __launch_bounds__(512, 2) conv_gemm_x3dw_group(const ConvGroup g) {
  ConvParams p;
  int local, b;
  const ConvParams& pr = group_member(g, p, local, b);
  x3dw_tile<64, SPLIT, BN, RAG, true>(p, pr, local, b, 0);
}

bool x3dq_ok(const ConvParams& p, int bn, bool wide) {
  const int span = (p.taps - 1) * (p.in_step < 0 ? -p.in_step : p.in_step);
  if (!p.x6 || !p.w3 || p.x_layout != LAYOUT_H2 || p.Cin % 32 || p.Cout % bn || p.ksplit > 1) return false;
  const long long arow = (long long)p.ldx * 4;
  if ((long long)p.taps * p.Cin * p.Cout * 4 >= (1LL << 31)) return false;
  if (p.taps == 1) {
    for (int i = 0; i < kMaxPhases; ++i)
      if (p.in_base[i] < 0) return false;
    return 256LL * arow < (1LL << 31);
  }
  return p.taps >= (wide ? 2 : 3) && span > 0 && span <= 64 && (long long)(p.Lin + 1024) * arow < (1LL << 31);
}
int x3dq_bn(const ConvParams& p) {
  const int k = p.kn ? p.kn->h3_bn : 0;
  if (p.Cout % 256) return (k == 128 && p.taps >= 3) || p.taps < 2 ? 128 : 384;
  if (p.taps == 2) return 512;
  return k == 128 ? 128 : k == 256 ? 256 : 512;
}

template <int BN>
hipError_t launch_x3dq(const ConvParams& p, int batch, int phases, hipStream_t s, const char** kname) {
  constexpr int BM = 32768 / BN;
  if (p.taps == 1) {
    if (p.clip_len) return hipErrorNotSupported;
    if (kname) *kname = BN == 256 ? "conv_gemm_x3dm<128,256>" : "conv_gemm_x3dm<256,128>";
    return launch_flat<BM, BN>(conv_gemm_x3dq<BN, 0>, p, batch, phases, 512, s);
  }
  if (kname) *kname = BN == 256 ? "conv_gemm_x3dq<128,256,halo>" : "conv_gemm_x3dq<256,128,halo>";
  if (p.clip_len) return launch_flat<BM, BN>(conv_gemm_x3dq<BN, 64, true>, p, batch, phases, 512, s);
  return launch_flat<BM, BN>(conv_gemm_x3dq<BN, 64>, p, batch, phases, 512, s);
}

template hipError_t launch_x3dq<256>(const ConvParams&, int, int, hipStream_t, const char**);
template hipError_t launch_x3dq<128>(const ConvParams&, int, int, hipStream_t, const char**);

hipError_t launch_x3dw(const ConvParams& p, int bsel, int batch, int phases, hipStream_t s, const char** kname) {
  const bool sp = knobs(p).h3_split;
  if (p.clip_len) {
    if (p.taps == 1) return hipErrorNotSupported;
    if (bsel == 384) {
      if (kname) *kname = "conv_gemm_x3dw<384,128,halo>";
      return sp ? launch_flat<384, 128>(conv_gemm_x3dw<64, true, 128, true>, p, batch, phases, 512, s)
                : launch_flat<384, 128>(conv_gemm_x3dw<64, false, 128, true>, p, batch, phases, 512, s);
    }
    if (kname) *kname = "conv_gemm_x3dw<256,256,halo>";
    return sp ? launch_flat<256, 256>(conv_gemm_x3dw<64, true, 256, true>, p, batch, phases, 512, s)
              : launch_flat<256, 256>(conv_gemm_x3dw<64, false, 256, true>, p, batch, phases, 512, s);
  }
  if (bsel == 384) {
    if (kname) *kname = "conv_gemm_x3dw<384,128,halo>";
    return sp ? launch_flat<384, 128>(conv_gemm_x3dw<64, true, 128>, p, batch, phases, 512, s)
              : launch_flat<384, 128>(conv_gemm_x3dw<64, false, 128>, p, batch, phases, 512, s);
  }
  if (p.taps == 1) {
    if (kname) *kname = "conv_gemm_x3dw<256,256>";
    return sp ? launch_flat<256, 256>(conv_gemm_x3dw<0, true>, p, batch, phases, 512, s)
              : launch_flat<256, 256>(conv_gemm_x3dw<0, false>, p, batch, phases, 512, s);
  }
  if (kname) *kname = "conv_gemm_x3dw<256,256,halo>";
  return sp ? launch_flat<256, 256>(conv_gemm_x3dw<64, true>, p, batch, phases, 512, s)
            : launch_flat<256, 256>(conv_gemm_x3dw<64, false>, p, batch, phases, 512, s);
}

hipError_t launch_h3_group(const ConvGroup& g, int bsel, bool split, unsigned blocks, hipStream_t s, const char** kname) {
  if (g.p[0].clip_len) {
    if (bsel == 384) {
      if (kname) *kname = "conv_gemm_x3dw_group<384,128,halo>";
      if (split) hipLaunchKernelGGL((conv_gemm_x3dw_group<true, 128, true>), dim3(blocks), dim3(512), 0, s, g);
      else hipLaunchKernelGGL((conv_gemm_x3dw_group<false, 128, true>), dim3(blocks), dim3(512), 0, s, g);
    } else if (bsel == 512) {
      if (kname) *kname = "conv_gemm_x3dw_group<256,256,halo>";
      if (split) hipLaunchKernelGGL((conv_gemm_x3dw_group<true, 256, true>), dim3(blocks), dim3(512), 0, s, g);
      else hipLaunchKernelGGL((conv_gemm_x3dw_group<false, 256, true>), dim3(blocks), dim3(512), 0, s, g);
    } else if (bsel == 256) {
      if (kname) *kname = "conv_gemm_x3dq_group<128,256,halo>";
      hipLaunchKernelGGL((conv_gemm_x3dq_group<256, true>), dim3(blocks), dim3(512), 0, s, g);
    } else {
      if (kname) *kname = "conv_gemm_x3dq_group<256,128,halo>";
      hipLaunchKernelGGL((conv_gemm_x3dq_group<128, true>), dim3(blocks), dim3(512), 0, s, g);
    }
    return hipGetLastError();
  }
  if (bsel == 384) {
    if (kname) *kname = "conv_gemm_x3dw_group<384,128,halo>";
    if (split) hipLaunchKernelGGL((conv_gemm_x3dw_group<true, 128>), dim3(blocks), dim3(512), 0, s, g);
    else hipLaunchKernelGGL((conv_gemm_x3dw_group<false, 128>), dim3(blocks), dim3(512), 0, s, g);
  } else if (bsel == 512) {
    if (kname) *kname = "conv_gemm_x3dw_group<256,256,halo>";
    if (split) hipLaunchKernelGGL(conv_gemm_x3dw_group<true>, dim3(blocks), dim3(512), 0, s, g);
    else hipLaunchKernelGGL(conv_gemm_x3dw_group<false>, dim3(blocks), dim3(512), 0, s, g);
  } else if (bsel == 256) {
    if (kname) *kname = "conv_gemm_x3dq_group<128,256,halo>";
    hipLaunchKernelGGL((conv_gemm_x3dq_group<256>), dim3(blocks), dim3(512), 0, s, g);
  } else {
    if (kname) *kname = "conv_gemm_x3dq_group<256,128,halo>";
    hipLaunchKernelGGL((conv_gemm_x3dq_group<128>), dim3(blocks), dim3(512), 0, s, g);
  }
  return hipGetLastError();
}

}
```

### distilcodec_nabeel_amd/csrc/dcx_dispatch.cpp

```cpp
#include "dcx_host.h"

namespace dcx::host {

void prog_add(dcx::RangeProg& p, float g, const Rng& r) {
  p.m[p.n] = r.amax;
  p.g[p.n] = g;
  p.f[p.n] = r.amax_f;
  ++p.n;
}
dcx::RangeProg prog_conv(const ConvW& w, const Rng& in) {
  dcx::RangeProg p{};
  p.c = w.b_abs;
  prog_add(p, w.g_abs, in);
  return p;
}
static dcx::RangeProg prog_conv_rows(const ConvW& w, const float* in_row_amax) {
  dcx::RangeProg p{};
  p.rowwise = 1;
  p.c = w.b_abs;
  p.m[0] = in_row_amax;
  p.g[0] = w.g_abs;
  p.n = 1;
  return p;
}

Act conv_input(dcx_codec* h, Bump& ws, size_t n) {
  Act a;
  if (x6_mode(h)) a.p = ws.u16(3 * n);
  else a.f = ws.f(n);
  return a;
}

bool f32_input_ok(const ConvW& w) { return w.cin <= 128 && w.cout <= 64 && w.taps >= 2; }

static const struct {
  const char* name;
  int dcx::Knobs::*slot;
} kKnobs[] = {
    {"DCX_RP_R", &dcx::Knobs::rp_rows},                   {"DCX_RP_OLD", &dcx::Knobs::rp_old},
    {"DCX_RP_G64", &dcx::Knobs::rp_g64},                  {"DCX_GELU_LUT", &dcx::Knobs::gelu_lut},
    {"DCX_BF16_PERSIST", &dcx::Knobs::bf16_persist},      {"DCX_BF16_REG_EPI", &dcx::Knobs::bf16_reg_epi},
    {"DCX_DWCONV_TILED", &dcx::Knobs::dwconv_tiled},      {"DCX_SPLIT_MIN_STEPS", &dcx::Knobs::split_min_steps},
    {"DCX_SPLIT_GROUP_OFF", &dcx::Knobs::split_group_off}, {"DCX_H3", &dcx::Knobs::h3},
    {"DCX_H3_BN", &dcx::Knobs::h3_bn},                    {"DCX_H3_1X1", &dcx::Knobs::h3_1x1},
    {"DCX_H3_SPLIT", &dcx::Knobs::h3_split},              {"DCX_H3_PAIRS", &dcx::Knobs::h3_pairs},
    {"DCX_RP_RING", &dcx::Knobs::rp_ring},                {"DCX_ENC_STREAMS", &dcx::Knobs::enc_streams}};

int dcx::Knobs::*knob_slot(const std::string& n) {
  for (const auto& k : kKnobs)
    if (n == k.name) return k.slot;
  return nullptr;
}

void knobs_from_env(dcx::Knobs& k) {
  for (const auto& kn : kKnobs) {
    const char* e = std::getenv(kn.name);
    if (e && *e) k.*kn.slot = std::atoi(e);
  }
}

int conv_params(dcx_codec* h, const ConvW& w, const ConvCall& c, bool force_f32, ConvParams& p) {
  const bool x6 = x6_mode(h) && !force_f32;
  const bool x6_f32in = x6 && !c.x.p && c.x.f && f32_input_ok(w);
  if (c.silu_in && !x6_f32in) return fail(h, DCX_ERR_STATE, "internal: silu_in needs an fp32-input conv");
  if (x6 ? ((!c.x.p && !x6_f32in) || !w.w6) : !c.x.f)
    return fail(h, DCX_ERR_STATE, "internal: conv input missing for GEMM mode");
  p = ConvParams{};
  p.x = c.x.f;
  p.x6 = x6 ? c.x.p : nullptr;
  p.w = w.w;
  p.w6 = x6 ? w.w6 : nullptr;
  const bool one = x6 && h->gemm_mode == DCX_GEMM_BF16 && !c.exact;
  p.bias = one && w.b16 ? w.b16 : w.b;
  p.gamma = c.gamma;
  p.res = c.res;
  p.y = c.y;
  p.y2 = c.y2;
  p.y6 = c.y6;
  p.y6s = c.y6s;
  p.macc = c.macc;
  p.x_bstride = c.x_bstride;
  p.ldy = w.cout;
  p.y_bstride = (long long)c.Lq * w.out_mul * p.ldy;
  p.w_phase_stride = (long long)w.cout * w.taps * w.cin;
  p.Lin = c.Lin;
  p.Lq = c.Lq;
  p.Cin = w.cin;
  p.Cout = w.cout;
  p.ldx = c.ldx ? c.ldx : w.cin;
  p.taps = w.taps;
  p.in_step = w.in_step;
  p.out_mul = w.out_mul;
  for (int i = 0; i < dcx::kMaxPhases; ++i) p.in_base[i] = w.in_base[i];
  p.epi = c.epi;
  p.mean_mode = c.mean;
  p.nprod = one ? 1 : 6;
  p.round_bf16 = one;
  p.silu_in = c.silu_in;
  p.fixed_tiles = c.fixed_tiles ? 1 : 0;
  p.x_layout = x6 && c.x.p ? c.x.lay : LAYOUT_PLANES;
  p.y_layout = c.y6 ? c.y_lay : LAYOUT_PLANES;
  p.ys_layout = c.y6s ? c.ys_lay : LAYOUT_PLANES;
  if (p.x_layout == LAYOUT_H2) {
    if (!w.w3 || one) return fail(h, DCX_ERR_STATE, "internal: h2 input without h3 weights");
    p.w3 = w.w3;
    p.w3_shift = w.w3_shift;
    p.x_ash = c.x.r.ash;
    p.x_ash_c = c.x.r.ash_c;
    p.x_ash_row = c.x.r.ash_row;
    if (p.x_ash_row && (w.taps != 1 || w.phases != 1 || w.in_base[0] != 0))
      return fail(h, DCX_ERR_STATE, "internal: per-row input ranges need a one-tap conv");
  }
  p.y_ash = c.y_ash;
  p.y_amax = c.y_amax;
  p.yb = c.yb;
  p.rflag = h->rflag;
  p.clip_len = c.lens;
  p.len_mul = c.len_mul;
  if (c.lens && (c.len_mul < 1 || !x6 || one)) return fail(h, DCX_ERR_STATE, "internal: ragged conv outside x6 mode");
  p.wc = one && h->compact ? w.wc : nullptr;
  p.kn = &h->knobs;
  for (Layout l : {p.x_layout, p.y_layout, p.ys_layout})
    if (l != LAYOUT_PLANES && l != LAYOUT_BF16 && l != LAYOUT_H2) return fail(h, DCX_ERR_STATE, "internal: not a layout");
  if (p.ys_layout == LAYOUT_BF16) return fail(h, DCX_ERR_STATE, "internal: y6s takes planes or h2 only");
  if (p.x_layout == LAYOUT_BF16 && !one) return fail(h, DCX_ERR_STATE, "internal: compact layout outside bf16 mode");
  if (p.y_layout == LAYOUT_H2 && (!x6 || one)) return fail(h, DCX_ERR_STATE, "internal: h2 layout outside x6 mode");
  return DCX_OK;
}

bool takes_compact(const dcx_codec* h, const ConvW& w, long long rows) {
  return h->compact && h->gemm_mode == DCX_GEMM_BF16 && w.wc && w.taps == 1 && w.phases == 1 && w.in_base[0] == 0 &&
         rows < (1LL << 31) && dcx::bf16dm_takes(w.cin, w.cout, (int)rows, w.cin, 1);
}

Layout input_layout(const dcx_codec* h, const ConvW& w, long long rows, bool h3_ranges) {
  return takes_compact(h, w, rows) ? LAYOUT_BF16 : h3_ranges && takes_h3(h, w) ? LAYOUT_H2 : LAYOUT_PLANES;
}

bool h3_rows_ok(long long rows, int cin) { return (rows + 1024) * cin * 4LL < (1LL << 31); }

bool takes_h3_conv(const dcx_codec* h, const ConvW& w, long long rows) {
  return h->knobs.h3 && h->gemm_mode == DCX_GEMM_X6 && h->split_k < 2 && w.w3 && w.taps >= 2 && w.cout % 128 == 0 &&
         h3_rows_ok(rows, w.cin);
}

bool takes_h3(const dcx_codec* h, const ConvW& w) {
  return h->knobs.h3_1x1 && h->gemm_mode == DCX_GEMM_X6 && h->split_k < 2 && w.w3 && w.taps == 1 && w.phases == 1 &&
         w.in_base[0] == 0 && w.cout % 128 == 0;
}

double conv_flops(const ConvW& w, const ConvCall& c) { return 2.0 * c.batch * c.Lq * w.phases * w.cout * w.cin * w.taps; }
double conv_bytes(const ConvW& w, const ConvCall& c) {
  const double outs = (double)c.batch * c.Lq * w.phases * w.cout;
  return 4.0 * ((double)c.batch * c.Lin * w.cin + outs + (double)w.phases * w.cout * w.taps * w.cin);
}

static int split_factor(const dcx_codec* h, const ConvW& w, const ConvCall& c, const ConvParams& p) {
  if (h->split_k < 2 || !h->split_buf || p.nprod != 6 || !p.w6 || !p.x6 || p.x_layout != LAYOUT_PLANES || w.cout % 128) return 1;
  const long long out = (long long)c.batch * c.Lq * w.out_mul * w.cout;
  if (out > kSplitMaxOut || (w.cin / 16) % (w.taps % 2 ? 2 : 1)) return 1;
  const long long tiles = (long long)c.batch * ((c.Lq + 255) / 256) * std::max(1, w.cout / 128) * w.phases;
  if (tiles >= 128) return 1;
  if ((long long)w.taps * (w.cin / 16) < h->knobs.split_min_steps) return 1;
  const int unit = w.taps % 2 ? 2 : 1;
  const long long nunits = (w.cin / 16) / unit;
  return (int)std::min<long long>({(long long)std::min(h->split_k, kSplitMax), std::max<long long>(1, 256 / tiles), nunits});
}

static ConvParams kslice_params(const ConvParams& p, const ConvW& w, int S, float* part) {
  ConvParams q = p;
  q.ksplit = S;
  q.kunit = w.taps % 2 ? 2 : 1;
  q.bias = q.gamma = q.res = nullptr;
  q.macc = nullptr;
  q.y = part;
  q.y2 = nullptr;
  q.y6 = q.y6s = nullptr;
  q.epi = dcx::EPI_BIAS;
  q.mean_mode = dcx::MEAN_NONE;
  q.y_layout = LAYOUT_PLANES;
  q.round_bf16 = 0;
  q.y_ash = nullptr;
  q.y_amax = nullptr;
  return q;
}

static int run_conv_split(dcx_codec* h, const ConvW& w, const ConvCall& c, const ConvParams& p, int S, hipStream_t s) {
  ProfScope ps(h, s);
  const ConvParams q = kslice_params(p, w, S, h->split_buf);
  const char* kname = "conv";
  HIPCHK(h, dcx::launch_conv(q, c.batch * S, w.phases, s, &kname));
  h->last_kname = kname;
  HIPCHK(h, dcx::launch_splitk_epilogue(p, h->split_buf, S, (long long)c.batch * p.y_bstride, c.batch, w.phases, s));
  ps.done((std::string("splitk:") + kname).c_str(), conv_flops(w, c), conv_bytes(w, c));
  return DCX_OK;
}

#ifdef DCX_DIAG_DUP
static int diag_dup_mode() {
  const char* e = std::getenv("DCX_DIAG_DUP");
  return e && (e[0] == '1' || e[0] == '2') ? e[0] - '0' : 0;
}
#endif

int run_conv(dcx_codec* h, const ConvW& w, const ConvCall& c, hipStream_t s, bool force_f32) {
  ConvParams p;
  RUN(conv_params(h, w, c, force_f32, p));
  const int S = force_f32 ? 1 : split_factor(h, w, c, p);
  if (S > 1 && c.lens) return fail(h, DCX_ERR_STATE, "internal: ragged conv in the split-K mode");
  if (S > 1) return run_conv_split(h, w, c, p, S, s);
#ifdef DCX_DIAG_DUP
  if (const int dm = diag_dup_mode()) {
    ConvParams q = p;
    q.diag_skip = dm;
    ProfScope pd(h, s);
    const char* kn = "conv";
    HIPCHK(h, dcx::launch_conv(q, c.batch, w.phases, s, &kn));
    pd.done((std::string("diag:") + kn).c_str(), conv_flops(w, c), conv_bytes(w, c));
  }
#endif
  ProfScope ps(h, s);
  const char* kname = "conv";
  HIPCHK(h, dcx::launch_conv(p, c.batch, w.phases, s, &kname));
  h->last_kname = kname;
  ps.done(kname, conv_flops(w, c), conv_bytes(w, c));
  return DCX_OK;
}

int run_conv_group_split(dcx_codec* h, const ConvW* const* w, const ConvCall* c, ConvParams* p, int n, double fl,
                         double by, hipStream_t s) {
  if (n < 2 || h->knobs.split_group_off) return 1;
  long long tiles[dcx::kMaxGroup], out[dcx::kMaxGroup], chunks[dcx::kMaxGroup];
  int S[dcx::kMaxGroup], smax[dcx::kMaxGroup];
  const bool chain = p[0].mean_mode != dcx::MEAN_NONE;
  if (chain) {
    if (p[0].mean_mode != dcx::MEAN_FIRST || p[n - 1].mean_mode != dcx::MEAN_LAST) return 1;
    for (int i = 1; i < n - 1; ++i)
      if (p[i].mean_mode != dcx::MEAN_MID) return 1;
    for (int i = 1; i < n; ++i)
      if (p[i].macc != p[0].macc || c[i].Lq != c[0].Lq || w[i]->cout != w[0]->cout) return 1;
  }
  long long total = 0;
  for (int i = 0; i < n; ++i) {
    if (split_factor(h, *w[i], c[i], p[i]) < 2 || w[i]->taps < 3 || w[i]->out_mul != 1) return 1;
    tiles[i] = (long long)c[i].batch * ((c[i].Lq + 255) / 256) * (w[i]->cout / 128);
    out[i] = (long long)c[i].batch * p[i].y_bstride;
    const int unit = w[i]->taps % 2 ? 2 : 1;
    chunks[i] = (long long)w[i]->taps * (w[i]->cin / 16);
    smax[i] = (int)std::min<long long>(std::min(h->split_k, kSplitMax), (w[i]->cin / 16) / unit);
    S[i] = 2;
    if (S[i] > smax[i]) return 1;
    total += S[i] * tiles[i];
  }
  if (total > 256) return 1;
  for (;;) {
    int best = -1;
    for (int i = 0; i < n; ++i)
      if (S[i] < smax[i] && total + tiles[i] <= 256 &&
          (best < 0 || chunks[i] * S[best] > chunks[best] * S[i]))
        best = i;
    if (best < 0) break;
    ++S[best];
    total += tiles[best];
  }
  long long need = 0;
  for (int i = 0; i < n; ++i) need += S[i] > 1 ? S[i] * out[i] : 0;
  if (need > kSplitMax * kSplitMaxOut) return 1;
  ProfScope ps(h, s);
  ConvParams q[dcx::kMaxGroup], r[dcx::kMaxGroup];
  const float* part[dcx::kMaxGroup];
  int rs[dcx::kMaxGroup];
  long long rstride[dcx::kMaxGroup];
  int nr = 0;
  long long off = 0;
  for (int i = 0; i < n; ++i) {
    q[i] = p[i];
    q[i].ksplit = S[i];
    if (S[i] > 1) {
      q[i] = kslice_params(p[i], *w[i], S[i], h->split_buf + off);
      r[nr] = p[i];
      part[nr] = h->split_buf + off;
      rs[nr] = S[i];
      rstride[nr] = out[i];
      ++nr;
      off += S[i] * out[i];
    }
  }
  const char* kname = "conv_group";
  const hipError_t e = dcx::launch_conv_split_group(q, n, c[0].batch, s, &kname);
  if (e == hipErrorNotSupported) return 1;
  HIPCHK(h, e);
  if (nr) HIPCHK(h, dcx::launch_splitk_epilogue_group(r, part, rs, rstride, nr, c[0].batch, chain, s));
  ps.done((std::string("splitk:") + kname).c_str(), fl, by);
  return DCX_OK;
}

int run_conv_group(dcx_codec* h, const ConvW* const* w, const ConvCall* c, int n, hipStream_t s) {
  ConvParams p[dcx::kMaxGroup];
  double fl = 0, by = 0;
  bool same = true;
  for (int i = 0; i < n; ++i) {
    RUN(conv_params(h, *w[i], c[i], false, p[i]));
    fl += conv_flops(*w[i], c[i]);
    by += conv_bytes(*w[i], c[i]);
    same = same && c[i].batch == c[0].batch && w[i]->phases == 1;
  }
  if (same && n > 1 && h->split_k >= 2) {
    const int rc = run_conv_group_split(h, w, c, p, n, fl, by, s);
    if (rc != 1) return rc;
  }
  if (same && n > 1) {
#ifdef DCX_DIAG_DUP
    if (const int dm = diag_dup_mode()) {
      ConvParams q[dcx::kMaxGroup];
      for (int i = 0; i < n; ++i) {
        q[i] = p[i];
        q[i].diag_skip = dm;
      }
      ProfScope pd(h, s);
      const char* kn = "conv_group";
      const hipError_t e = dcx::launch_conv_group(q, n, c[0].batch, s, &kn);
      if (e == hipSuccess) pd.done((std::string("diag:") + kn).c_str(), fl, by);
    }
#endif
    ProfScope ps(h, s);
    const char* kname = "conv_group";
    const hipError_t e = dcx::launch_conv_group(p, n, c[0].batch, s, &kname);
    if (e == hipSuccess) {
      ps.done(kname, fl, by);
      return DCX_OK;
    }
    if (e != hipErrorNotSupported) HIPCHK(h, e);
  }
  for (int i = 0; i < n; ++i) RUN(run_conv(h, *w[i], c[i], s));
  return DCX_OK;
}

ConvCall pointwise(CAct x, long long rows) {
  ConvCall c;
  c.x = x;
  c.x_bstride = 0;
  c.batch = 1;
  c.Lin = c.Lq = (int)rows;
  c.ldx = 0;
  return c;
}
ConvCall framed(CAct x, int B, int L, int C) {
  ConvCall c;
  c.x = x;
  c.x_bstride = (long long)L * C;
  c.batch = B;
  c.Lin = c.Lq = L;
  c.ldx = C;
  return c;
}


int ensure_planes(dcx_codec* h, CAct& a, long long rows, int C, Bump& ws, hipStream_t s, Layout want, int clips,
                  const int* lens) {
  const bool rh2 = want == LAYOUT_H2;
  if (rh2 && a.p && a.lay != LAYOUT_H2 && a.f) a.p = nullptr;
  if (!x6_mode(h) || a.p) return DCX_OK;
  unsigned short* p = ws.u16((size_t)rows * C * 3);
  float* am = rh2 && clips ? ws.f((size_t)clips) : nullptr;
  int* ash = rh2 ? ws.i((size_t)(clips ? clips : rows)) : nullptr;
  WS_READY(h, ws, "workspace too small");
  if (lens && !(rh2 && clips)) return fail(h, DCX_ERR_STATE, "internal: ragged tensor outside the ranged h2 split");
  if (rh2 && clips) {
    if (clips < 1 || rows % clips) return fail(h, DCX_ERR_STATE, "internal: ranged split of a ragged batch");
    LAUNCH(h, s, "h2_ranged", 0, 12.0 * rows * C,
           dcx::launch_h2_ranged(a.f, nullptr, p, clips, rows / clips, C, 0, 0.f, am, ash, h->rflag, s, lens, 1));
    a.r = Rng{};
    a.r.ash = ash;
    a.r.amax = am;
  } else if (rh2) {
    LAUNCH(h, s, "h2_rows", 0, 8.0 * rows * C, dcx::launch_h2_rows(a.f, p, rows, C, ash, s));
    a.r = Rng{};
    a.r.ash_row = ash;
  } else {
    LAUNCH(h, s, "split_planes", 0, (want == LAYOUT_BF16 ? 6.0 : 10.0) * rows * C,
           dcx::launch_split_planes(a.f, p, rows, C, want, s));
  }
  a.p = p;
  a.lay = want;
  return DCX_OK;
}

int run_block(dcx_codec* h, const BlockW& bw, float* x, unsigned short* out6, int B, int T, Act ln, Act hid,
              hipStream_t s, Layout out_lay, const dcx::RaggedSeg* rg) {
  const long long M = (long long)B * T;
  const int C = bw.C;
  if (out6 && out_lay == LAYOUT_H2) return fail(h, DCX_ERR_STATE, "internal: a block output in h2 goes through launch_h2_rows");
  ln.lay = input_layout(h, bw.pw1, M, ln.row_ash && ln.row_amax);
  hid.lay = input_layout(h, bw.pw2, M, hid.row_ash);
  ln.r = Rng{};
  hid.r = Rng{};
  ln.r.ash_row = ln.row_ash;
  hid.r.ash_row = hid.row_ash;
  if (rg) {
    if (B != 1 || T != rg->rows) return fail(h, DCX_ERR_STATE, "internal: ragged block rows");
    LAUNCH(h, s, "dwconv_ln_ragged", 14.0 * M * C, 8.0 * M * C,
           dcx::launch_dwconv_ln_ragged(x, ln.f, ln.p, ln.lay, bw.dww, bw.dwb, bw.ln.w, bw.ln.b, *rg, C,
                                        h->gemm_mode == DCX_GEMM_BF16 ? 1 : 0, &h->knobs, s, ln.row_ash, ln.row_amax));
  } else {
    LAUNCH(h, s, "dwconv_ln", 14.0 * M * C, 8.0 * M * C,
           dcx::launch_dwconv_ln(x, ln.f, ln.p, ln.lay, bw.dww, bw.dwb, bw.ln.w, bw.ln.b, B, T, C,
                                 h->gemm_mode == DCX_GEMM_BF16 ? 1 : 0, &h->knobs, s, ln.row_ash, ln.row_amax));
  }
  ConvCall c1 = pointwise(ln, M);
  c1.out_to(hid);
  c1.epi = dcx::EPI_GELU;
  if (hid.p && hid.lay == LAYOUT_H2) {
    c1.yb = prog_conv_rows(bw.pw1, ln.row_amax);
    c1.y_ash = hid.row_ash;
  }
  RUN(run_conv(h, bw.pw1, c1, s));
  ConvCall c2 = pointwise(hid, M);
  c2.y = x;
  c2.y6 = out6;
  c2.y_lay = out_lay;
  c2.res = x;
  c2.gamma = bw.gamma;
  c2.epi = dcx::EPI_GAMMA_RES;
  RUN(run_conv(h, bw.pw2, c2, s));
  return DCX_OK;
}

int run_ln(dcx_codec* h, const LnW& l, const float* x, Act y, long long rows, hipStream_t s, bool bf16_in) {
  const int form = bf16_in && h->gemm_mode == DCX_GEMM_BF16 ? 2 : 1;
  if (y.p && y.lay == LAYOUT_H2 && !y.row_ash) return fail(h, DCX_ERR_STATE, "internal: h2 LayerNorm output without row ranges");
  LAUNCH(h, s, "ln_rows", 8.0 * rows * l.C, 8.0 * rows * l.C,
         dcx::launch_ln_rows(x, y.f, y.p, y.lay, l.w, l.b, rows, l.C, 1e-6f, form, s,
                             y.row_ash, y.row_amax));
  return DCX_OK;
}

void row_ranges(dcx_codec* h, Bump& ws, long long M, Act& ln, Act& hid) {
  if (!x6_mode(h)) return;
  ln.row_ash = ws.i((size_t)M);
  ln.row_amax = ws.f((size_t)M);
  hid.row_ash = ws.i((size_t)M);
}

}
```

### distilcodec_nabeel_amd/csrc/dcx_kernels.h

```cpp
#pragma once
#include <hip/hip_runtime.h>
#include <stdint.h>

namespace dcx {

enum Epi : int {
  EPI_BIAS = 0,
  EPI_GELU = 1,
  EPI_GAMMA_RES = 2,
  EPI_RES = 3,
  EPI_LOGCLAMP = 4,
};

enum Mean : int { MEAN_NONE = 0, MEAN_FIRST = 1, MEAN_MID = 2, MEAN_LAST = 3 };

constexpr int kMaxPhases = 8;

enum Layout : int { LAYOUT_PLANES = 0, LAYOUT_BF16 = 1, LAYOUT_H2 = 3 };
__host__ __device__ constexpr int layout_u16(Layout l) { return l == LAYOUT_BF16 ? 1 : (int)l >= 2 ? 2 : 3; }

constexpr int kH2Top = 15;
constexpr int kH2ShiftMax = 64;
__host__ __device__ inline int h2_shift(float bound) {
  if (!(bound <= 3.0e38f)) return 0;
  if (bound < 1e-30f) return kH2ShiftMax;
  int e = 0;
  (void)frexpf(bound, &e);
  const int a = kH2Top - e;
  return a < -kH2ShiftMax ? -kH2ShiftMax : a > kH2ShiftMax ? kH2ShiftMax : a;
}
enum RangeFlag : int { RANGE_NONFINITE = 1, RANGE_OVER = 2 };
constexpr int kRangeTerms = 6;
struct RangeProg {
  const float* m[kRangeTerms];
  float g[kRangeTerms], f[kRangeTerms];
  float c;
  int n;
  int rowwise;
};
__device__ __forceinline__ float range_bound(const RangeProg& r, long long b) {
  float v = r.c;
#pragma unroll
  for (int i = 0; i < kRangeTerms; ++i)
    if (i < r.n) v += r.g[i] * fmaxf(r.m[i] ? r.m[i][b] : 0.f, r.f[i]);
  return v;
}
__device__ __forceinline__ float range_cur(const float* amax, long long b) {
  return amax ? __hip_atomic_load(amax + b, __ATOMIC_RELAXED, __HIP_MEMORY_SCOPE_AGENT) : 0.f;
}
__device__ __forceinline__ void range_report_wg(float vmax, float* amax, int b, float lim, int* rflag, float cur,
                                                float* red, int nt) {
#pragma unroll
  for (int off = 32; off >= 1; off >>= 1) vmax = fmaxf(vmax, __shfl_xor(vmax, off, 64));
  asm volatile("s_waitcnt lgkmcnt(0)\n\ts_barrier" ::: "memory");
  if ((threadIdx.x & 63) == 0) red[threadIdx.x >> 6] = vmax;
  asm volatile("s_waitcnt lgkmcnt(0)\n\ts_barrier" ::: "memory");
  float m = 0.f;
  if (threadIdx.x == 0) {
    m = red[0];
    for (int w = 1; w < nt / 64; ++w) m = fmaxf(m, red[w]);
  }
  asm volatile("s_waitcnt lgkmcnt(0)\n\ts_barrier" ::: "memory");
  if (threadIdx.x == 0) {
    if (amax && m > cur) atomicMax(reinterpret_cast<unsigned*>(amax + b), __float_as_uint(m));
    if (rflag && m > lim) atomicOr(rflag, RANGE_OVER);
  }
}
__device__ __forceinline__ void range_report(float vmax, float* amax, int b, float lim, int* rflag, float cur = -1.f) {
#pragma unroll
  for (int off = 32; off >= 1; off >>= 1) vmax = fmaxf(vmax, __shfl_xor(vmax, off, 64));
  if ((threadIdx.x & 63) == 0) {
    if (amax && vmax > cur) atomicMax(reinterpret_cast<unsigned*>(amax + b), __float_as_uint(vmax));
    if (rflag && vmax > lim) atomicOr(rflag, RANGE_OVER);
  }
}

struct Knobs {
  int rp_rows = 0;
  int rp_old = 0;
  int rp_g64 = 0;
  int gelu_lut = -1;
  int bf16_persist = 1;
  int bf16_reg_epi = 1;
  int dwconv_tiled = 0;
  int split_min_steps = 0;
  int split_group_off = 0;
  int h3 = 1;
  int h3_bn = 0;
  int h3_split = 1;
  int h3_pairs = 1;
  int h3_1x1 = 1;
  int rp_ring = 1;
  int enc_streams = 2;
};

struct ConvParams {
  const float* x;
  const unsigned short* x6;
  const float* w;
  const unsigned short* w6;
  const float* bias;
  const float* gamma;
  const float* res;
  float* y;
  float* y2;
  float* macc;
  unsigned short* y6;
  unsigned short* y6s;
  long long x_bstride;
  long long y_bstride;
  long long w_phase_stride;
  int Lin, Lq, Cin, Cout, ldx, ldy;
  int taps, in_step, out_mul;
  int in_base[kMaxPhases];
  int epi, mean_mode;
  const float* x2;
  const float* e2;
  float* part_val;
  int* part_idx;
  float* part_val2;
  int nprod, round_bf16;
  int batch, phases;
  int silu_in;
  Layout x_layout, y_layout;
  const unsigned short* wc;
  int ksplit, kunit;
  int diag_skip;
  int gelu_lut;
  const Knobs* kn;
  int fixed_tiles;
  const unsigned short* w3;
  int w3_shift;
  Layout ys_layout;
  const int* x_ash;
  int x_ash_c;
  const int* x_ash_row;
  int* y_ash;
  float* y_amax;
  RangeProg yb;
  int* rflag;
  const int* clip_len;
  int len_mul;
};

__device__ __forceinline__ int clip_rows(const int* clip_len, int len_mul, int b, int full) {
  if (!clip_len) return full;
  const long long r = (long long)max(clip_len[b], 0) * len_mul;
  return __builtin_amdgcn_readfirstlane((int)(r < full ? r : full));
}

constexpr int kMaxGroup = 3;
struct ConvGroup {
  ConvParams p[kMaxGroup];
  int start[kMaxGroup + 1];
  int tiles_per_clip[kMaxGroup];
};

struct SplitEpiGroup {
  ConvParams p[kMaxGroup];
  const float* part[kMaxGroup];
  int splits[kMaxGroup];
  long long stride[kMaxGroup], total4[kMaxGroup];
  int start[kMaxGroup + 1];
  int chain;
};

struct ResPairParams {
  const float* src[kMaxGroup];
  float* dst[kMaxGroup];
  const unsigned short* w1[kMaxGroup];
  const unsigned short* w2[kMaxGroup];
  const float* b1[kMaxGroup];
  const float* b2[kMaxGroup];
  int taps[kMaxGroup], dil[kMaxGroup];
  int nmem;
  float* mean_out;
  long long bstride;
  int L, batch, C;
  int h3;
  int w3_shift1[kMaxGroup], w3_shift2[kMaxGroup];
  const float* src_amax[kMaxGroup];
  float* dst_amax[kMaxGroup];
  float g1[kMaxGroup], bm1[kMaxGroup];
  int* rflag;
  const Knobs* kn;
  const int* clip_len;
  int len_mul;
};

hipError_t launch_conv(const ConvParams& p, int batch, int phases, hipStream_t s, const char** kname);
hipError_t launch_conv_group(const ConvParams* ps, int n, int batch, hipStream_t s, const char** kname);
hipError_t launch_res_pair(const ResPairParams& p, hipStream_t s, const char** kname);
hipError_t launch_splitk_epilogue(const ConvParams& p, const float* partials, int splits, long long stride, int batch,
                                  int phases, hipStream_t s);
hipError_t launch_conv_split_group(const ConvParams* ps, int n, int batch, hipStream_t s, const char** kname);
hipError_t launch_splitk_epilogue_group(const ConvParams* ps, const float* const* partials, const int* splits,
                                        const long long* strides, int n, int batch, bool chain, hipStream_t s);
hipError_t launch_vq_argmin(const ConvParams& p, int rows, hipStream_t s, const char** kname);
int vq_argmin_ntiles(int ncodes);
int vq_prefilter_ntiles(int ncodes, int dim, Layout x_layout);
hipError_t launch_vq_prefilter(const ConvParams& p, int rows, bool x_bf16, hipStream_t s, const char** kname);
bool vq_b1_takes(int ncodes, int dim);
constexpr float kVqPrefilterBound = 2.5e-4f;
double vq_prefilter_cx(Layout x_layout, int ncodes, int dim, float emax, float dmax);
struct VqRescoreArgs {
  const float *part_val, *part_val2;
  const int* part_idx;
  long long rows;
  int ntiles, tile_codes, dim;
  const float *x, *x2, *xr2;
  const double* x2d;
  const float* codebook;
  const double* e2d;
  double cx;
  float emax, e2max;
  int32_t* codes;
  int* stats;
  int2* pairs;
  double* cdist;
  int* ccode;
  long long cap;
  int2* row_list;
  unsigned long long* npairs;
};
hipError_t launch_vq_certify(const VqRescoreArgs& a, hipStream_t s);
hipError_t launch_vq_pair_eval(const VqRescoreArgs& a, hipStream_t s);
hipError_t launch_vq_pair_reduce(const VqRescoreArgs& a, hipStream_t s);
hipError_t launch_vq_reduce(const float* part_val, const int* part_idx, int rows, int ntiles, int32_t* codes,
                            hipStream_t s);
hipError_t launch_row_sqnorm(const float* x, long long rows, int C, float* out, double* x2d, float* xr2,
                             unsigned long long* zero_me, hipStream_t s);
hipError_t launch_ln_rows(const float* x, float* y, unsigned short* y6, Layout lay, const float* w, const float* b,
                          long long rows, int C, float eps, int channels_first_form, hipStream_t s,
                          int* ash_row = nullptr, float* amax_row = nullptr);
hipError_t launch_dwconv_ln(const float* x, float* y, unsigned short* y6, Layout lay, const float* dww, const float* dwb,
                            const float* lnw, const float* lnb, int batch, int L, int C, int bf16, const Knobs* kn,
                            hipStream_t s, int* ash_row = nullptr, float* amax_row = nullptr);
hipError_t launch_h2_rows(const float* x, unsigned short* y6, long long rows, int C, int* ash_row, hipStream_t s);
hipError_t launch_h2_ranged(const float* x, float* yf, unsigned short* y6, int batch, long long L, int C, int silu,
                            float floor, float* amax, int* ash, int* rflag, hipStream_t s,
                            const int* clip_len = nullptr, int len_mul = 1);
hipError_t launch_zero_words(void* p, long long n, hipStream_t s);
hipError_t launch_clip_amax(const float* x, int batch, long long L, int C, float* amax, hipStream_t s,
                            const int* clip_len = nullptr, int len_mul = 1);
int device_cus();
bool bf16dm_takes(int cin, int cout, int lq, int ldx, int phases);
struct RaggedSeg {
  const int *cu_samples, *cu_frames, *cu_t16, *cu_t4, *cu_run;
  int batch, rw;
  int rows, n_t16, n_t4, n_run;
};
inline int dwconv_run_rows(long long rows) {
  return rows >= 2048LL * 32 ? 32 : rows >= 2048LL * 16 ? 16 : rows >= 2048LL * 8 ? 8 : 4;
}
hipError_t launch_ragged_frames(const float* audio, const RaggedSeg& g, float* frames, unsigned short* frames6,
                                int n_fft, int hop, int pad, hipStream_t s);
hipError_t launch_ragged_unfold(const void* x, void* y, const RaggedSeg& g, int row_bytes, int taps, hipStream_t s);
hipError_t launch_dwconv_ln_ragged(const float* x, float* y, unsigned short* y6, Layout lay, const float* dww,
                                   const float* dwb, const float* lnw, const float* lnb, const RaggedSeg& g, int C,
                                   int bf16, const Knobs* kn, hipStream_t s, int* ash_row = nullptr,
                                   float* amax_row = nullptr);
hipError_t launch_frame_pad(const float* audio, float* frames, unsigned short* frames6, int batch, long long n, int rows,
                            int hop, int pad_left, hipStream_t s);
hipError_t launch_silu_act(const float* x, float* yf, unsigned short* y6, long long rows, int C, hipStream_t s,
                           Layout lay = LAYOUT_PLANES);
hipError_t launch_spec_mag(const float* spec, float* mag, unsigned short* mag6, float* loglin, long long rows, int nbins,
                           int ld_out, hipStream_t s);
hipError_t launch_split_planes(const float* x, unsigned short* y6, long long rows, int C, Layout lay, hipStream_t s);
hipError_t launch_gather_rows(const float* table, int ntable, const int32_t* idx, long long rows, int width,
                              float* out, int32_t* n_invalid, int masked_row, hipStream_t s,
                              const int* clip_len = nullptr, long long frames = 0);
constexpr int kMaxCodebooks = 8;
struct VqResidualArgs {
  const float* src;
  const float* codebook;
  const int32_t* ck;
  int32_t* codes_out;
  float* dst;
  unsigned short* op6;
  Layout op_layout;
  float *x2, *xr2;
  double* x2d;
  unsigned long long* zero_me;
  float* fup;
  int fup_first;
  long long rows;
  int dim, ncodes, R;
};
hipError_t launch_vq_residual_step(const VqResidualArgs& a, hipStream_t s);
struct GatherSumArgs {
  const float* table[kMaxCodebooks];
  const int32_t* idx;
  float* out;
  unsigned short* out6;
  Layout out_layout;
  int32_t* n_invalid;
  const int* clip_len;
  long long frames;
  long long rows;
  int dim, ncodes, R;
};
hipError_t launch_gather_sum_rows(const GatherSumArgs& a, hipStream_t s);
hipError_t launch_zero_tail_rows(float* x, int batch, long long L, int C, const int* clip_len, int len_mul,
                                 hipStream_t s);
hipError_t launch_conv_post_tanh(const float* x, const float* w, float bias, float* out, int batch, int L, int C,
                                 int k, int bf16, hipStream_t s, const int* clip_len = nullptr, int len_mul = 1);
hipError_t launch_transpose(const float* in, float* out, int batch, long long rows, long long cols, hipStream_t s);
hipError_t launch_resample_poly(const float* x, int batch, long long n_in, long long xs, const double* h, int hlen,
                                int up, int down, long long pre, float* y, long long n_out, long long ys,
                                hipStream_t s);

}
```

### distilcodec_nabeel_amd/engine.py

```python
from __future__ import annotations

import contextlib
import ctypes
import os

import numpy as np
import torch

from . import _native
from .config import check_supported


_TRAINING_ONLY = ("_codebook.embed_avg", "_codebook.cluster_size")

KNOB_DEFAULTS = {
    "DCX_RP_R": 0, "DCX_RP_OLD": 0, "DCX_RP_G64": 0, "DCX_GELU_LUT": -1,
    "DCX_BF16_PERSIST": 1, "DCX_BF16_REG_EPI": 1, "DCX_DWCONV_TILED": 0, "DCX_SPLIT_MIN_STEPS": 0,
    "DCX_SPLIT_GROUP_OFF": 0, "DCX_H3": 1, "DCX_H3_BN": 0, "DCX_H3_1X1": 1, "DCX_H3_SPLIT": 1, "DCX_H3_PAIRS": 1, "DCX_RP_RING": 1,
    "DCX_ENC_STREAMS": 2,
}

GEMM_MODES = {"f32": _native.DCX_GEMM_F32, "x6": _native.DCX_GEMM_X6, "bf16": _native.DCX_GEMM_BF16}


class NativeCodec:

    def __init__(self, cfg: dict, state: dict, device, with_generator: bool = True, gemm: str | None = None):
        check_supported(cfg)
        self.cfg = cfg
        self.device = torch.device(device)
        if self.device.type != "cuda":
            raise _native.NativeUnavailable("the DistilCodec MI355X path needs a GPU device (cuda:N on ROCm)")
        if not torch.cuda.is_available():
            raise _native.NativeUnavailable("no GPU visible to torch: the HIP path cannot run here")
        self.L = _native.lib()
        self.c = _native.config_from_dict(cfg)
        self.D = cfg["quantizer"]["input_dim"]
        self.CD = cfg["quantizer"]["codebook_dim"]
        self.NC = cfg["quantizer"]["codebook_size"]
        self.n_mels = cfg["spec_transform"]["num_mels"]
        self.hop = cfg["spec_transform"]["hop_size"]
        self.with_generator = with_generator
        self._ws = None
        h = ctypes.c_void_p()
        with torch.cuda.device(self.device):
            self._check(self.L.dcx_create(ctypes.byref(self.c), ctypes.byref(h)), None)
            self.h = h
            self.gemm = gemm or os.environ.get("DCX_GEMM", "x6")
            if self.gemm not in GEMM_MODES:
                raise ValueError(f"unknown GEMM mode {self.gemm!r}; expected one of {sorted(GEMM_MODES)}")
            self._check(self.L.dcx_set_gemm_mode(self.h, GEMM_MODES[self.gemm]))
            self._check(self.L.dcx_set_num_codebooks(self.h, int(cfg["quantizer"]["n_codebooks"])))
            self.R = int(self.L.dcx_num_codebooks(self.h))
            for part in ("encoder", "quantizer") + (("generator",) if with_generator else ()):
                for k, v in state[part].items():
                    if k.endswith(_TRAINING_ONLY):
                        continue
                    a = np.ascontiguousarray(np.asarray(v, dtype=np.float32))
                    shape = (ctypes.c_int64 * max(a.ndim, 1))(*a.shape)
                    self._check(self.L.dcx_set_tensor(self.h, f"{part}.{k}".encode(), a.ctypes.data_as(ctypes.c_void_p),
                                                      a.ndim, shape))
            self._check(self.L.dcx_finalize(self.h, 1 if with_generator else 0))

    def _check(self, rc, h="self"):
        if rc == _native.DCX_OK:
            return
        msg = ""
        handle = self.h if h == "self" else h
        if handle:
            msg = self.L.dcx_last_error(handle).decode()
        msg = msg or self.L.dcx_status_string(rc).decode()
        if rc == _native.DCX_ERR_INVALID_ARG:
            raise ValueError(msg)
        if rc == _native.DCX_ERR_MISSING_WEIGHT:
            raise KeyError(msg)
        raise _native.NativeError(rc, msg)

    def __del__(self):
        h = getattr(self, "h", None)
        if h:
            try:
                self.L.dcx_destroy(h)
            except Exception:
                pass
            self.h = None

    def _stream(self):
        return ctypes.c_void_p(torch.cuda.current_stream(self.device).cuda_stream)

    def workspace_size(self, batch: int, frames: int) -> int:
        return int(self.L.dcx_workspace_size(self.h, batch, frames))

    def workspace(self, batch: int, frames: int, ws: torch.Tensor | None = None) -> torch.Tensor:
        return self._workspace_of(self.workspace_size(batch, frames), ws)

    def _workspace_of(self, need: int, ws: torch.Tensor | None) -> torch.Tensor:
        if ws is not None:
            if ws.device != self.device or ws.dtype != torch.uint8 or not ws.is_contiguous() or ws.numel() < need:
                raise ValueError(f"workspace must be a contiguous uint8 tensor on {self.device} of >= {need} bytes")
            return ws
        if self._ws is None or self._ws.numel() < need:
            self._ws = None
            self._ws = torch.empty(need, dtype=torch.uint8, device=self.device)
        return self._ws

    def _codes_shape(self, *lead) -> tuple:
        return tuple(lead) if self.R == 1 else tuple(lead) + (self.R,)

    def _codes_in(self, codes) -> torch.Tensor:
        codes = self._dev(codes, torch.int32)
        want = 2 if self.R == 1 else 3
        if codes.ndim != want or (self.R > 1 and codes.shape[2] != self.R):
            raise ValueError(f"codes must be shaped {self._codes_shape('B', 'T')}, got {tuple(codes.shape)}")
        return codes

    @staticmethod
    def _ptr(t):
        return ctypes.c_void_p(t.data_ptr()) if t is not None else None

    def _dev(self, t, dtype):
        t = torch.as_tensor(t)
        if t.device != self.device or t.dtype != dtype or not t.is_contiguous():
            t = t.to(device=self.device, dtype=dtype).contiguous()
        return t

    def set_gemm(self, mode: str) -> None:
        self._check(self.L.dcx_set_gemm_mode(self.h, GEMM_MODES[mode]))
        self.gemm = mode

    def set_split_k(self, max_splits: int) -> None:
        self._check(self.L.dcx_set_split_k(self.h, int(max_splits)))
        self._ws = None

    def set_knob(self, name: str, value: int) -> None:
        self._check(self.L.dcx_set_knob(self.h, name.encode(), int(value)))

    def get_knob(self, name: str) -> int:
        v = ctypes.c_int32(0)
        self._check(self.L.dcx_get_knob(self.h, name.encode(), ctypes.byref(v)))
        return v.value

    @contextlib.contextmanager
    def knobs(self, **values):
        saved = {k: self.get_knob(k) for k in values}
        for k, v in values.items():
            self.set_knob(k, v)
        try:
            yield self
        finally:
            for k, v in saved.items():
                self.set_knob(k, v)

    def range_flags(self, reset: bool = False) -> int:
        v = ctypes.c_int32(0)
        self._check(self.L.dcx_range_flags(self.h, ctypes.byref(v), int(reset)))
        return v.value

    def num_frames(self, n_samples: int) -> int:
        return int(self.L.dcx_num_frames(self.h, n_samples))

    def mel(self, audio: torch.Tensor, ws: torch.Tensor | None = None, linear: bool = False):
        audio = self._dev(audio, torch.float32)
        B, N = audio.shape
        T = self.num_frames(N)
        out = torch.empty(B, T, self.n_mels, device=self.device)
        ws = self.workspace(B, T, ws)
        with torch.cuda.device(self.device):
            if linear:
                lin = torch.empty(B, T, self.cfg["spec_transform"]["n_fft"] // 2 + 1, device=self.device)
                self._check(self.L.dcx_mel_linear(self.h, self._ptr(audio), B, N, self._ptr(out), self._ptr(lin),
                                                  self._ptr(ws), ws.numel(), self._stream()))
                return out, lin
            self._check(self.L.dcx_mel(self.h, self._ptr(audio), B, N, self._ptr(out), self._ptr(ws), ws.numel(), self._stream()))
        return out

    def encode(self, mel: torch.Tensor, ws: torch.Tensor | None = None) -> torch.Tensor:
        mel = self._dev(mel, torch.float32)
        B, T, _ = mel.shape
        out = torch.empty(B, T, self.cfg["encoder"]["dims"][-1], device=self.device)
        ws = self.workspace(B, T, ws)
        with torch.cuda.device(self.device):
            self._check(self.L.dcx_encode(self.h, self._ptr(mel), B, T, self._ptr(out), self._ptr(ws), ws.numel(), self._stream()))
        return out

    def vq_encode(self, feat: torch.Tensor, want_pjt_in=True, want_fup=True, want_quantized=True,
                  ws: torch.Tensor | None = None):
        feat = self._dev(feat, torch.float32)
        B, T, _ = feat.shape
        codes = torch.empty(self._codes_shape(B, T), dtype=torch.int32, device=self.device)
        pin = torch.empty(B, T, self.CD, device=self.device) if want_pjt_in else None
        fup = torch.empty(B, T, self.CD, device=self.device) if want_fup else None
        q = torch.empty(B, T, self.D, device=self.device) if want_quantized else None
        ws = self.workspace(B, T, ws)
        with torch.cuda.device(self.device):
            self._check(self.L.dcx_vq_encode(self.h, self._ptr(feat), B, T, self._ptr(codes), self._ptr(pin), self._ptr(fup),
                                             self._ptr(q), self._ptr(ws), ws.numel(), self._stream()))
        return codes, pin, fup, q

    def vq_decode(self, codes: torch.Tensor, ws: torch.Tensor | None = None) -> torch.Tensor:
        codes = self._codes_in(codes)
        B, T = codes.shape[:2]
        z = torch.empty(B, T, self.D, device=self.device)
        ws = self.workspace(B, T, ws)
        with torch.cuda.device(self.device):
            self._check(self.L.dcx_vq_decode(self.h, self._ptr(codes), B, T, self._ptr(z), None, self._ptr(ws), ws.numel(),
                                             self._stream()))
        return z

    def generate(self, z: torch.Tensor, ws: torch.Tensor | None = None) -> torch.Tensor:
        if not self.with_generator:
            raise RuntimeError("this engine was built without generator weights")
        z = self._dev(z, torch.float32)
        B, T, _ = z.shape
        wav = torch.empty(B, self.hop * T, device=self.device)
        ws = self.workspace(B, T, ws)
        with torch.cuda.device(self.device):
            self._check(self.L.dcx_generate(self.h, self._ptr(z), B, T, self._ptr(wav), self._ptr(ws), ws.numel(), self._stream()))
        return wav

    def encode_decode(self, audio: torch.Tensor, codes: torch.Tensor | None = None, wav: torch.Tensor | None = None,
                      ws: torch.Tensor | None = None):
        audio = self._dev(audio, torch.float32)
        B, N = audio.shape
        T = self.num_frames(N)
        if codes is None:
            codes = torch.empty(self._codes_shape(B, T), dtype=torch.int32, device=self.device)
        elif self.R > 1 and (tuple(codes.shape) != self._codes_shape(B, T) or codes.dtype != torch.int32 or not codes.is_contiguous()):
            raise ValueError(f"codes must be a contiguous int32 tensor shaped {self._codes_shape(B, T)}")
        if wav is None:
            wav = torch.empty(B, self.hop * T, device=self.device)
        ws = self.workspace(B, T, ws)
        with torch.cuda.device(self.device):
            self._check(self.L.dcx_encode_decode(self.h, self._ptr(audio), B, N, self._ptr(codes), self._ptr(wav), self._ptr(ws),
                                                 ws.numel(), self._stream()))
        return codes, wav

    def ragged_plan(self, lengths) -> tuple[np.ndarray, int, int]:
        n = np.ascontiguousarray(np.asarray(lengths, dtype=np.int64).reshape(-1))
        B = int(n.shape[0])
        words = int(self.L.dcx_ragged_plan_size(B))
        plan = np.zeros(max(words, 1), dtype=np.int32)
        ts, tf = ctypes.c_int64(0), ctypes.c_int64(0)
        self._check(self.L.dcx_ragged_plan(self.h, n.ctypes.data_as(ctypes.POINTER(ctypes.c_int64)), B,
                                           plan.ctypes.data_as(ctypes.c_void_p), words, ctypes.byref(ts), ctypes.byref(tf)))
        return plan, ts.value, tf.value

    def tokenize_ragged(self, clips, want_pjt_in: bool = False, want_fup: bool = False, ws: torch.Tensor | None = None):
        if len(clips) == 0:
            raise ValueError("tokenize_ragged needs at least one clip")
        flat = [torch.as_tensor(c).reshape(-1) for c in clips]
        lengths = [int(c.numel()) for c in flat]
        plan, total_samples, total_frames = self.ragged_plan(lengths)
        B = len(flat)
        audio = torch.cat([c.to(device=self.device, dtype=torch.float32) for c in flat])
        plan_dev = torch.from_numpy(plan).to(self.device)
        offsets = torch.tensor(np.concatenate([[0], np.cumsum([self.num_frames(n + 1) for n in lengths])]), dtype=torch.int64)
        assert int(offsets[-1]) == total_frames
        codes = torch.empty(self._codes_shape(total_frames), dtype=torch.int32, device=self.device)
        pin = torch.empty(total_frames, self.CD, device=self.device) if want_pjt_in else None
        fup = torch.empty(total_frames, self.CD, device=self.device) if want_fup else None
        ws = self._workspace_of(int(self.L.dcx_ragged_workspace_size(self.h, B, total_frames)), ws)
        with torch.cuda.device(self.device):
            self._check(self.L.dcx_tokenize_ragged(self.h, self._ptr(audio), self._ptr(plan_dev),
                                                   plan.ctypes.data_as(ctypes.c_void_p), B, total_samples, total_frames,
                                                   self._ptr(codes), self._ptr(pin), self._ptr(fup), self._ptr(ws),
                                                   ws.numel(), self._stream()))
        return codes, offsets, pin, fup

    def _ragged_lengths(self, lengths, B: int, T: int) -> torch.Tensor:
        if isinstance(lengths, torch.Tensor) and lengths.is_cuda:
            if lengths.dtype != torch.int32 or lengths.numel() != B or not lengths.is_contiguous():
                raise ValueError(f"device lengths must be contiguous int32 [{B}]")
            return lengths
        from .ragged import check_lengths
        return torch.from_numpy(check_lengths(lengths, B, T)).to(self.device)

    def generate_ragged(self, z: torch.Tensor, lengths, ws: torch.Tensor | None = None,
                        wav: torch.Tensor | None = None) -> torch.Tensor:
        if not self.with_generator:
            raise RuntimeError("this engine was built without generator weights")
        z = self._dev(z, torch.float32)
        B, T, _ = z.shape
        lens = self._ragged_lengths(lengths, B, T)
        if wav is None:
            wav = torch.empty(B, self.hop * T, device=self.device)
        ws = self.workspace(B, T, ws)
        with torch.cuda.device(self.device):
            self._check(self.L.dcx_generate_ragged(self.h, self._ptr(z), self._ptr(lens), B, T, self._ptr(wav), self._ptr(ws),
                                                   ws.numel(), self._stream()))
        return wav

    def decode_ragged(self, codes: torch.Tensor, lengths, ws: torch.Tensor | None = None,
                      wav: torch.Tensor | None = None, n_invalid: torch.Tensor | None = None) -> torch.Tensor:
        if not self.with_generator:
            raise RuntimeError("this engine was built without generator weights")
        codes = self._codes_in(codes)
        B, T = codes.shape[:2]
        lens = self._ragged_lengths(lengths, B, T)
        if wav is None:
            wav = torch.empty(B, self.hop * T, device=self.device)
        ws = self.workspace(B, T, ws)
        with torch.cuda.device(self.device):
            self._check(self.L.dcx_decode_ragged(self.h, self._ptr(codes), self._ptr(lens), B, T, self._ptr(wav),
                                                 self._ptr(n_invalid), self._ptr(ws), ws.numel(), self._stream()))
        return wav

    def module_io(self, name: str) -> tuple[int, int, int]:
        ci, co, r = ctypes.c_int32(), ctypes.c_int32(), ctypes.c_int32()
        self._check(self.L.dcx_module_io(self.h, name.encode(), ctypes.byref(ci), ctypes.byref(co), ctypes.byref(r)))
        return ci.value, co.value, r.value

    def module(self, name: str, x: torch.Tensor) -> torch.Tensor:
        cin, cout, rate = self.module_io(name)
        x = self._dev(x, torch.float32)
        if x.ndim != 3 or x.shape[2] != cin:
            raise ValueError(f"{name} takes (B, L, {cin}) input, got {tuple(x.shape)}")
        B, L, C = x.shape
        n = name.encode()
        need = int(self.L.dcx_module_workspace_size(self.h, n, B, L))
        if need == 0:
            raise ValueError(f"module {name!r} cannot run on this handle")
        if cout == 0:
            y = torch.empty(B, L, dtype=torch.int32, device=self.device)
        else:
            y = torch.empty(B, L * rate, cout, device=self.device)
        ws = torch.empty(need, dtype=torch.uint8, device=self.device)
        with torch.cuda.device(self.device):
            self._check(self.L.dcx_module_forward(self.h, n, self._ptr(x), B, L, C, self._ptr(y), self._ptr(ws), ws.numel(),
                                                  self._stream()))
        return y

    def transpose(self, x: torch.Tensor) -> torch.Tensor:
        x = self._dev(x, torch.float32)
        B, R, C = x.shape
        out = torch.empty(B, C, R, device=self.device)
        with torch.cuda.device(self.device):
            rc = self.L.dcx_transpose(self._ptr(x), self._ptr(out), B, R, C, self._stream())
        if rc != _native.DCX_OK:
            raise _native.NativeError(rc, "dcx_transpose failed")
        return out

    def profile(self, on: bool):
        self._check(self.L.dcx_profile_enable(self.h, 1 if on else 0))

    def vq_rescore_stats(self, reset: bool = False) -> tuple[int, int]:
        import ctypes
        r, c = ctypes.c_int64(0), ctypes.c_int64(0)
        self._check(self.L.dcx_vq_rescore_stats(self.h, ctypes.byref(r), ctypes.byref(c), int(reset)))
        return r.value, c.value

    def profile_reset(self):
        self._check(self.L.dcx_profile_reset(self.h))

    def profile_read(self) -> dict:
        out = {}
        n = self.L.dcx_profile_count(self.h)
        for i in range(n):
            name = ctypes.c_char_p()
            launches = ctypes.c_int64()
            ms, fl, by = ctypes.c_double(), ctypes.c_double(), ctypes.c_double()
            self._check(self.L.dcx_profile_read(self.h, i, ctypes.byref(name), ctypes.byref(launches), ctypes.byref(ms),
                                                ctypes.byref(fl), ctypes.byref(by)))
            out[name.value.decode()] = {"launches": launches.value, "ms": ms.value, "flops": fl.value, "bytes": by.value}
        return out


class NativeConv:

    def __init__(self, weight: np.ndarray, bias=None, dilation: int = 1, transposed: bool = False, stride: int = 1,
                 h3: bool = False):
        self.L = _native.lib()
        w = np.ascontiguousarray(weight, dtype=np.float32)
        if transposed:
            self.cin, self.cout, self.k = w.shape
        else:
            self.cout, self.cin, self.k = w.shape
        b = None if bias is None else np.ascontiguousarray(bias, dtype=np.float32)
        self.stride = stride if transposed else 1
        self._b = b
        h = ctypes.c_void_p()
        rc = self.L.dcx_conv_create(w.ctypes.data_as(ctypes.c_void_p), None if b is None else b.ctypes.data_as(ctypes.c_void_p),
                                    self.cin, self.cout, self.k, dilation, 1 if transposed else 0, stride, ctypes.byref(h))
        if rc != _native.DCX_OK:
            raise ValueError(f"dcx_conv_create failed: {self.L.dcx_status_string(rc).decode()}")
        self.h = h
        if h3 and self.L.dcx_conv_set_h3(self.h, 1) != _native.DCX_OK:
            raise ValueError("dcx_conv_set_h3 failed")

    def set_knob(self, name: str, value: int):
        rc = self.L.dcx_conv_set_knob(self.h, name.encode(), int(value))
        if rc != _native.DCX_OK:
            raise _native.NativeError(rc, f"dcx_conv_set_knob({name}) failed")

    @property
    def last_kernel(self) -> str:
        return self.L.dcx_conv_last_kernel(self.h).decode()

    def __del__(self):
        h = getattr(self, "h", None)
        if h:
            self.L.dcx_conv_destroy(h)
            self.h = None

    def __call__(self, x: torch.Tensor, gemm: str = "x6", epi: int = 0, res: torch.Tensor | None = None,
                 want_y: bool = True, want_silu: bool = False):
        B, Lin, C = x.shape
        assert C == self.cin and x.is_cuda and x.dtype == torch.float32 and x.is_contiguous()
        Lout = Lin * self.stride
        y = torch.empty(B, Lout, self.cout, device=x.device) if want_y else None
        ys = torch.empty(B, Lout, self.cout, device=x.device) if want_silu else None
        ptr = lambda t: ctypes.c_void_p(t.data_ptr()) if t is not None else None
        rc = self.L.dcx_conv_forward(self.h, GEMM_MODES[gemm], ptr(x), B, Lin, ptr(y), ptr(ys), ptr(res), epi,
                                     ctypes.c_void_p(torch.cuda.current_stream(x.device).cuda_stream))
        if rc != _native.DCX_OK:
            raise _native.NativeError(rc, "dcx_conv_forward failed")
        return (y, ys) if want_silu else y
```

### include/distilcodec_amd.h

```cpp
#ifndef DISTILCODEC_AMD_H
#define DISTILCODEC_AMD_H

#include <stddef.h>
#include <stdint.h>

#ifdef __cplusplus
extern "C" {
#endif

#define DCX_ABI_VERSION 4
#define DCX_MAX_CODEBOOKS 8

enum {
  DCX_OK = 0,
  DCX_ERR_INVALID_ARG = -1,
  DCX_ERR_MISSING_WEIGHT = -2,
  DCX_ERR_STATE = -3,
  DCX_ERR_HIP = -4,
  DCX_ERR_OOM = -5,
  DCX_ERR_WORKSPACE = -6,
  DCX_ERR_UNSUPPORTED = -7
};

typedef struct dcx_codec dcx_codec;

typedef struct dcx_config {
  int32_t sample_rate;
  int32_t n_fft, hop, win;
  int32_t n_mels;
  float f_min, f_max;
  int32_t enc_depths[4];
  int32_t enc_dims[4];
  int32_t vq_dim;
  int32_t codebook_dim;
  int32_t codebook_size;
  int32_t gen_channels;
  int32_t gen_pre_k, gen_post_k;
  int32_t n_ups;
  int32_t up_rates[8];
  int32_t up_kernels[8];
  int32_t n_res;
  int32_t res_kernels[4];
  int32_t res_dilations[4][4];
} dcx_config;

void dcx_default_config(dcx_config* cfg);

int dcx_create(const dcx_config* cfg, dcx_codec** out);
void dcx_destroy(dcx_codec* h);
const char* dcx_last_error(const dcx_codec* h);
const char* dcx_status_string(int status);
int dcx_abi_version(void);
const char* dcx_build_id(void);

int dcx_set_tensor(dcx_codec* h, const char* name, const float* host_data, int32_t ndim, const int64_t* shape);
int dcx_finalize(dcx_codec* h, int32_t with_generator);

int dcx_set_num_codebooks(dcx_codec* h, int32_t n);
int32_t dcx_num_codebooks(const dcx_codec* h);

int64_t dcx_num_frames(const dcx_codec* h, int64_t n_samples);
size_t dcx_workspace_size(const dcx_codec* h, int32_t batch, int64_t frames);

int dcx_mel(dcx_codec* h, const float* audio, int32_t batch, int64_t n_samples, float* mel,
            void* workspace, size_t ws_bytes, void* stream);
int dcx_mel_linear(dcx_codec* h, const float* audio, int32_t batch, int64_t n_samples, float* mel, float* log_linear,
                   void* workspace, size_t ws_bytes, void* stream);

int dcx_encode(dcx_codec* h, const float* mel, int32_t batch, int64_t frames, float* feat,
               void* workspace, size_t ws_bytes, void* stream);

int dcx_vq_encode(dcx_codec* h, const float* feat, int32_t batch, int64_t frames, int32_t* codes,
                  float* x_pjt_in, float* quantized_fup, float* quantized,
                  void* workspace, size_t ws_bytes, void* stream);

int dcx_vq_decode(dcx_codec* h, const int32_t* codes, int32_t batch, int64_t frames, float* z,
                  int32_t* n_invalid, void* workspace, size_t ws_bytes, void* stream);

int dcx_generate(dcx_codec* h, const float* z, int32_t batch, int64_t frames, float* wav,
                 void* workspace, size_t ws_bytes, void* stream);

int dcx_encode_decode(dcx_codec* h, const float* audio, int32_t batch, int64_t n_samples,
                      int32_t* codes, float* wav, void* workspace, size_t ws_bytes, void* stream);

int64_t dcx_ragged_plan_size(int32_t batch);
int dcx_ragged_plan(dcx_codec* h, const int64_t* clip_samples, int32_t batch, int32_t* plan, int64_t plan_words,
                    int64_t* total_samples, int64_t* total_frames);
size_t dcx_ragged_workspace_size(const dcx_codec* h, int32_t batch, int64_t total_frames);
int dcx_tokenize_ragged(dcx_codec* h, const float* audio_packed, const int32_t* plan_dev, const int32_t* plan_host,
                        int32_t batch, int64_t total_samples, int64_t total_frames, int32_t* codes, float* x_pjt_in,
                        float* quantized_fup, void* workspace, size_t ws_bytes, void* stream);

int dcx_generate_ragged(dcx_codec* h, const float* z, const int32_t* lengths_dev, int32_t batch, int64_t frames_max,
                        float* wav, void* workspace, size_t ws_bytes, void* stream);
int dcx_decode_ragged(dcx_codec* h, const int32_t* codes, const int32_t* lengths_dev, int32_t batch,
                      int64_t frames_max, float* wav, int32_t* n_invalid, void* workspace, size_t ws_bytes,
                      void* stream);

int dcx_resample_poly(const float* x, int32_t batch, int64_t n_in, int64_t x_stride, const double* h, int32_t h_len,
                      int32_t up, int32_t down, int64_t pre, float* y, int64_t n_out, int64_t y_stride, void* stream);

int dcx_mp3_info(const uint8_t* data, size_t nbytes, int64_t* samples, int32_t* sample_rate, int32_t* channels);
int dcx_mp3_decode(const uint8_t* data, size_t nbytes, float* out, int64_t capacity);
const char* dcx_mp3_last_error(void);
int dcx_mp3_stats(int64_t* granules, int64_t* exact);
int64_t dcx_mp3_junk_bytes(void);
int64_t dcx_mp3_bad_frames(void);

int dcx_transpose(const float* in, float* out, int32_t batch, int64_t rows, int64_t cols, void* stream);

#define DCX_GEMM_F32 0
#define DCX_GEMM_X6 1
#define DCX_GEMM_BF16 2
int dcx_set_gemm_mode(dcx_codec* h, int32_t mode);
int32_t dcx_get_gemm_mode(const dcx_codec* h);

int dcx_set_split_k(dcx_codec* h, int32_t max_splits);

int dcx_set_knob(dcx_codec* h, const char* name, int32_t value);
int dcx_get_knob(const dcx_codec* h, const char* name, int32_t* value);

int dcx_range_flags(dcx_codec* h, int32_t* flags, int32_t reset);

typedef struct dcx_conv dcx_conv;
int dcx_conv_create(const float* weight, const float* bias, int32_t cin, int32_t cout, int32_t k, int32_t dilation,
                    int32_t transposed, int32_t stride, dcx_conv** out);
int dcx_conv_forward(dcx_conv* c, int32_t gemm_mode, const float* x, int32_t batch, int64_t lin, float* y,
                     float* y_silu, const float* res, int32_t epi, void* stream);
void dcx_conv_destroy(dcx_conv* c);
const char* dcx_conv_last_kernel(const dcx_conv* c);
int dcx_conv_set_knob(dcx_conv* c, const char* name, int32_t value);
int dcx_conv_set_h3(dcx_conv* c, int32_t on);

int dcx_module_io(const dcx_codec* h, const char* module, int32_t* in_channels, int32_t* out_channels,
                  int32_t* out_rate);
size_t dcx_module_workspace_size(const dcx_codec* h, const char* module, int32_t batch, int64_t rows);
int dcx_module_forward(dcx_codec* h, const char* module, const float* x, int32_t batch, int64_t rows,
                       int32_t channels, void* y, void* workspace, size_t ws_bytes, void* stream);

int dcx_vq_rescore_stats(dcx_codec* h, int64_t* rows_rescored, int64_t* codes_rescored, int32_t reset);

int dcx_profile_enable(dcx_codec* h, int32_t on);
int dcx_profile_reset(dcx_codec* h);
int32_t dcx_profile_count(const dcx_codec* h);
int dcx_profile_read(dcx_codec* h, int32_t i, const char** name, int64_t* launches, double* ms,
                     double* flops, double* bytes);

#ifdef __cplusplus
}
#endif
#endif
```

Baseline: 51.05 million.

## Specialize h3 conv epilogue into compile-time forms per output combination

Adds templated EpiForm epilogue variants that fix the epilogue op, mean mode and output set at compile time. The h3 conv kernels can then select a specialized epilogue instead of the generic runtime-branching one, which is meant to cut branching, register pressure and redundant loads and stores. It also adds a test entry point for h3 convs, launch counters per form, and knobs to fall back to the generic epilogue or to turn off conv grouping. The risks are larger code size, more template instantiations, and numerical divergence between the specialized and generic paths.

```diff
diff --git a/distilcodec_nabeel_amd/_native.py b/distilcodec_nabeel_amd/_native.py
--- a/distilcodec_nabeel_amd/_native.py
+++ b/distilcodec_nabeel_amd/_native.py
@@ -55,6 +55,11 @@
 _I64 = ctypes.c_int64
 _SZ = ctypes.c_size_t
 
+class ConvH3Out(ctypes.Structure):
+    _fields_ = [(n, ctypes.c_void_p) for n in ("y", "y_silu", "y_silu_h2", "y_ash", "y_amax", "res", "res_amax", "macc",
+                                               "macc_amax", "lens")] + [("epi", ctypes.c_int32), ("mean", ctypes.c_int32)]
+
+
 SIGNATURES = {
     "dcx_default_config": (None, [ctypes.POINTER(DcxConfig)]),
     "dcx_create": (ctypes.c_int, [ctypes.POINTER(DcxConfig), ctypes.POINTER(_P)]),
@@ -101,6 +106,8 @@
     "dcx_conv_forward": (ctypes.c_int, [_P, _I32, _P, _I32, _I64, _P, _P, _P, _I32, _P]),
     "dcx_conv_destroy": (None, [_P]),
     "dcx_conv_last_kernel": (ctypes.c_char_p, [_P]),
+    "dcx_conv_forward_h3": (ctypes.c_int, [_P, _P, _I32, ctypes.c_int64, _P, _P]),
+    "dcx_epi_form_launches": (ctypes.c_int, [ctypes.POINTER(ctypes.c_int64), _I32, _I32]),
     "dcx_conv_set_knob": (ctypes.c_int, [_P, ctypes.c_char_p, _I32]),
     "dcx_conv_set_h3": (ctypes.c_int, [_P, _I32]),
     "dcx_module_workspace_size": (_SZ, [_P, ctypes.c_char_p, _I32, _I64]),
diff --git a/distilcodec_nabeel_amd/csrc/dcx_api.cpp b/distilcodec_nabeel_amd/csrc/dcx_api.cpp
--- a/distilcodec_nabeel_amd/csrc/dcx_api.cpp
+++ b/distilcodec_nabeel_amd/csrc/dcx_api.cpp
@@ -532,20 +532,21 @@
   return DCX_OK;
 }
 
-int dcx_conv_forward(dcx_conv* c, int32_t gemm_mode, const float* x, int32_t batch, int64_t lin, float* y,
-                     float* y_silu, const float* res, int32_t epi, void* stream) {
-  if (!c || !x || batch <= 0 || lin <= 0 || (!y && !y_silu)) return DCX_ERR_INVALID_ARG;
-  if (epi != dcx::EPI_BIAS && epi != dcx::EPI_GELU && epi != dcx::EPI_RES) return DCX_ERR_INVALID_ARG;
-  if (epi == dcx::EPI_RES && !res) return DCX_ERR_INVALID_ARG;
+}
+
+template <class Outputs>
+static int conv_forward(dcx_conv* c, int32_t gemm_mode, const float* x, int32_t batch, int64_t lin, void* stream,
+                        Outputs outputs) {
   dcx_codec* h = &c->scratch;
   h->gemm_mode = gemm_mode;
   hipStream_t s = (hipStream_t)stream;
   CAct xa(x, nullptr);
+  bool h3 = false;
   if (gemm_mode != DCX_GEMM_F32 && gemm_mode != DCX_GEMM_X6 && gemm_mode != DCX_GEMM_BF16) return DCX_ERR_INVALID_ARG;
   if (gemm_mode != DCX_GEMM_F32 && !f32_input_ok(c->w)) {
     const size_t need = (size_t)batch * lin * c->w.cin * 3;
     if (!grow(c->planes, c->planes_cap, need)) return DCX_ERR_OOM;
-    const bool h3 = c->h3 && (c->w.taps >= 2 ? takes_h3_conv(h, c->w, lin) : takes_h3(h, c->w));
+    h3 = c->h3 && (c->w.taps >= 2 ? takes_h3_conv(h, c->w, lin) : takes_h3(h, c->w));
     if (h3) {
       const long long rows = (long long)batch * lin;
       const size_t words = (size_t)batch + (size_t)std::max<long long>(batch, rows);
@@ -570,11 +571,51 @@
     xa.p = c->planes;
   }
   ConvCall cc = framed(xa, batch, (int)lin, c->w.cin);
-  cc.y = y;
-  cc.y2 = y_silu;
-  cc.res = res;
-  cc.epi = epi;
-  return run_conv(h, c->w, cc, s);
+  const int code = outputs(cc, h3);
+  return code != DCX_OK ? code : run_conv(h, c->w, cc, s);
+}
+
+extern "C" {
+
+int dcx_conv_forward(dcx_conv* c, int32_t gemm_mode, const float* x, int32_t batch, int64_t lin, float* y,
+                     float* y_silu, const float* res, int32_t epi, void* stream) {
+  if (!c || !x || batch <= 0 || lin <= 0 || (!y && !y_silu)) return DCX_ERR_INVALID_ARG;
+  if (epi != dcx::EPI_BIAS && epi != dcx::EPI_GELU && epi != dcx::EPI_RES) return DCX_ERR_INVALID_ARG;
+  if (epi == dcx::EPI_RES && !res) return DCX_ERR_INVALID_ARG;
+  return conv_forward(c, gemm_mode, x, batch, lin, stream, [&](ConvCall& cc, bool) -> int {
+    cc.y = y;
+    cc.y2 = y_silu;
+    cc.res = res;
+    cc.epi = epi;
+    return DCX_OK;
+  });
+}
+
+int dcx_conv_forward_h3(dcx_conv* c, const float* x, int32_t batch, int64_t lin, const dcx_conv_h3_out* o, void* stream) {
+  if (!c || !x || !o || batch <= 0 || lin <= 0 || c->w.taps < 2 || c->w.phases != 1) return DCX_ERR_INVALID_ARG;
+  if (o->epi != dcx::EPI_BIAS && o->epi != dcx::EPI_RES) return DCX_ERR_INVALID_ARG;
+  if (o->mean < dcx::MEAN_NONE || o->mean > dcx::MEAN_LAST || (o->mean != dcx::MEAN_NONE && !o->macc)) return DCX_ERR_INVALID_ARG;
+  if (o->epi == dcx::EPI_RES && (!o->res || !o->res_amax)) return DCX_ERR_INVALID_ARG;
+  if (o->mean >= dcx::MEAN_MID && !o->macc_amax) return DCX_ERR_INVALID_ARG;
+  if (o->y_silu_h2 && !o->y_ash) return DCX_ERR_INVALID_ARG;
+  return conv_forward(c, DCX_GEMM_X6, x, batch, lin, stream, [&](ConvCall& cc, bool h3) -> int {
+    if (!h3) return fail(&c->scratch, DCX_ERR_INVALID_ARG, "dcx_conv_forward_h3: not an h3 conv (dcx_conv_set_h3, Cout % 128)");
+    cc.y = o->y;
+    cc.y2 = o->y_silu;
+    cc.y6s = o->y_silu_h2;
+    cc.ys_lay = dcx::LAYOUT_H2;
+    cc.res = o->res;
+    cc.macc = o->macc;
+    cc.epi = o->epi;
+    cc.mean = o->mean;
+    cc.yb = prog_conv(c->w, cc.x.r);
+    if (o->res) prog_add(cc.yb, 1.0f, Rng{nullptr, 0, o->res_amax, 0.f});
+    if (o->mean >= dcx::MEAN_MID) prog_add(cc.yb, 1.0f, Rng{nullptr, 0, o->macc_amax, 0.f});
+    cc.y_amax = o->y_amax;
+    cc.y_ash = o->y_silu_h2 ? o->y_ash : nullptr;
+    cc.ragged(o->lens, (int)lin);
+    return DCX_OK;
+  });
 }
 
 void dcx_conv_destroy(dcx_conv* c) {
@@ -586,6 +627,14 @@
 }
 
 const char* dcx_conv_last_kernel(const dcx_conv* c) { return c ? c->scratch.last_kname : ""; }
+
+int dcx_epi_form_launches(int64_t* counts, int32_t n, int32_t reset) {
+  if (!counts || n != dcx::kEpiFormCounters) return DCX_ERR_INVALID_ARG;
+  long long v[dcx::kEpiFormCounters];
+  dcx::epi_form_launches(v, reset != 0);
+  for (int i = 0; i < n; ++i) counts[i] = v[i];
+  return DCX_OK;
+}
 
 int dcx_conv_set_knob(dcx_conv* c, const char* name, int32_t value) {
   if (!c || !name) return DCX_ERR_INVALID_ARG;
diff --git a/distilcodec_nabeel_amd/csrc/dcx_conv_common.h b/distilcodec_nabeel_amd/csrc/dcx_conv_common.h
--- a/distilcodec_nabeel_amd/csrc/dcx_conv_common.h
+++ b/distilcodec_nabeel_amd/csrc/dcx_conv_common.h
@@ -167,9 +167,207 @@
   return e;
 }
 
-template <int BM, int BN, int WM, int WN, int LDS_FLOATS, int NT, int RROW = 2, bool RAG = true, typename AccT>
+struct EpiGeneric {
+  static constexpr bool fixed = false;
+};
+template <int EPI, int MEAN, bool Y, bool Y2, bool Y6H, bool Y6SH, bool TRACK, bool ROWWISE = false>
+struct EpiForm {
+  static constexpr bool fixed = true;
+  static constexpr int epi = EPI, mean = MEAN;
+  static constexpr bool y = Y, y2 = Y2, y6h = Y6H, y6sh = Y6SH, track = TRACK, rowwise = ROWWISE;
+};
+template <typename F>
+inline bool epi_form_is(const ConvParams& p) {
+  const bool h2o = F::y6h || F::y6sh;
+  return p.epi == F::epi && p.mean_mode == F::mean && !p.round_bf16 && (p.y != nullptr) == F::y &&
+         (p.y2 != nullptr) == F::y2 && (p.y6 != nullptr) == F::y6h && (p.y6s != nullptr) == F::y6sh &&
+         (!p.y6 || p.y_layout == LAYOUT_H2) && (!p.y6s || p.ys_layout == LAYOUT_H2) && (p.y_amax != nullptr) == F::track &&
+         (h2o ? (p.yb.rowwise != 0) == F::rowwise : true) && (F::epi != EPI_GELU || p.w6 != nullptr) &&
+         (F::mean == MEAN_NONE || p.macc != nullptr);
+}
+
+template <int BM, int BN, int WM, int WN, int LDS_FLOATS, int NT, int RROW, bool RAG, typename F, typename AccT>
+__device__ __forceinline__ void epilogue_form(const ConvParams& p, const ConvParams& pr, AccT& acc, int q0, int co0, int b,
+                                              int ph, float* smem, const EpiPre& pre) {
+  constexpr int WR = BM / WM, WC = BN / WN;
+  static_assert(sizeof(acc[0][0]) == 16 && sizeof(acc) == WR * WC * 4 / 64, "16 x 16 accumulator blocks");
+  constexpr int LDSW = BN + 4;
+  constexpr int RPP = (BM * LDSW <= LDS_FLOATS) ? BM
+                      : (BM / 2 * LDSW <= LDS_FLOATS) ? BM / 2
+                      : (BM / 4 * LDSW <= LDS_FLOATS) ? BM / 4 : WR;
+  static_assert(RPP % WR == 0 && RPP * LDSW <= LDS_FLOATS, "epilogue pass does not fit LDS");
+  const int tid = threadIdx.x, lane = tid & 63, wave = tid >> 6;
+  const int wm = wave / WN, wn = wave % WN;
+  const long long ob = (long long)b * p.y_bstride;
+  constexpr bool RIN = RROW & 1, ROUT = RROW & 2;
+  constexpr bool h2o = F::y6h || F::y6sh, h2row = ROUT && h2o && F::rowwise;
+  constexpr bool need_r = F::epi == EPI_GAMMA_RES || F::epi == EPI_RES;
+  constexpr bool need_m = F::mean == MEAN_MID || F::mean == MEAN_LAST;
+  static_assert(!((F::mean == MEAN_FIRST || F::mean == MEAN_MID) && (F::y || F::y2 || h2o || F::track)), "mean form");
+  unsigned short* const y6 = F::y6h ? p.y6 + ob * 2 : nullptr;
+  unsigned short* const y6s = F::y6sh ? p.y6s + ob * 2 : nullptr;
+  const float osc = __builtin_bit_cast(
+      float, __builtin_amdgcn_readfirstlane(__builtin_bit_cast(int, __builtin_ldexpf(1.0f, h2o && !h2row ? pre.osh : 0))));
+  float vmax = 0.f;
+  const int lq_live = RAG ? clip_rows(pr.clip_len, pr.len_mul, b, p.Lq) : p.Lq;
+  constexpr int G = 8, NH = 2;
+  static_assert(NT % (BN / G) == 0, "each thread keeps one channel group");
+  const int cg = (tid % (BN / G)) * G, trow = tid / (BN / G), co = co0 + cg;
+  const int hsw = (lane >> 3) & 1;
+  f32x4 bias4[NH], gamma4[NH];
+#pragma unroll
+  for (int h = 0; h < NH; ++h) {
+    bias4[h] = p.bias ? *reinterpret_cast<const f32x4*>(p.bias + co + 4 * h) : f32x4{0.f, 0.f, 0.f, 0.f};
+    gamma4[h] = F::epi == EPI_GAMMA_RES ? *reinterpret_cast<const f32x4*>(p.gamma + co + 4 * h) : f32x4{0.f, 0.f, 0.f, 0.f};
+  }
+  constexpr int RSTEP = NT / (BN / G), ROWS_T = RPP / RSTEP;
+  static_assert(RPP % RSTEP == 0, "epilogue rows per thread");
+  constexpr auto div_cap = [](int n, int cap) {
+    int d = n < cap ? n : cap;
+    while (n % d) --d;
+    return d;
+  };
+  constexpr int IB = div_cap(ROWS_T, need_r || need_m ? 4 / NH : 8 / NH);
+  auto row_bound = [&](int q) { return fmaf(pr.yb.g[0], fmaxf(pr.yb.m[0][(long long)b * p.Lq + q], pr.yb.f[0]), pr.yb.c); };
+
+  auto pass = [&](int r0, auto fullt) {
+    constexpr bool FULL = decltype(fullt)::value;
+    f32x4 r[IB][NH], m[IB][NH];
+    float rin[RIN ? IB : 1], rbnd[h2row ? IB : 1];
+    auto load = [&](int rb) {
+#pragma unroll
+      for (int k = 0; k < IB; ++k) {
+        const int qq = q0 + r0 + trow + (rb + k) * RSTEP;
+        const int q = FULL ? qq : min(qq, p.Lq - 1);
+        const long long o = ob + ((long long)q * p.out_mul + ph) * p.ldy + co;
+#pragma unroll
+        for (int h = 0; h < NH; ++h) {
+          if constexpr (need_r) r[k][h] = *reinterpret_cast<const f32x4*>(p.res + o + 4 * h);
+          if constexpr (need_m) m[k][h] = *reinterpret_cast<const f32x4*>(p.macc + o + 4 * h);
+        }
+        if constexpr (RIN) rin[k] = pr.x_ash_row ? __builtin_ldexpf(1.0f, -pr.x_ash_row[(long long)b * p.Lin + q]) : 1.0f;
+        if constexpr (h2row) rbnd[k] = row_bound(q);
+      }
+    };
+    load(0);
+    __syncthreads();
+    if (wm * WR >= r0 && wm * WR < r0 + RPP) {
+#pragma unroll
+      for (int i = 0; i < WR / 16; ++i)
+#pragma unroll
+        for (int j = 0; j < WC / 16; ++j)
+#pragma unroll
+          for (int e = 0; e < 4; ++e) {
+            const int row = wm * WR + i * 16 + 4 * (lane >> 4) + e - r0;
+            smem[row * LDSW + wn * WC + j * 16 + (lane & 15)] = acc[i][j][e];
+          }
+    }
+    __syncthreads();
+#pragma unroll
+    for (int rb = 0; rb < ROWS_T; rb += IB) {
+      f32x4 x[IB][NH];
+      float rsc[IB];
+#pragma unroll
+      for (int k = 0; k < IB; ++k) {
+        const int rl = trow + (rb + k) * RSTEP;
+        const int q = q0 + r0 + rl;
+        const bool dead = RAG && q >= lq_live;
+        const float rin_ = RIN ? rin[RIN ? k : 0] : 1.0f;
+        const f32x4 u = *reinterpret_cast<const f32x4*>(smem + rl * LDSW + cg + 4 * hsw);
+        const f32x4 v = *reinterpret_cast<const f32x4*>(smem + rl * LDSW + cg + 4 * (1 - hsw));
+        x[k][0] = (hsw ? v : u) * rin_ + bias4[0];
+        x[k][1] = (hsw ? u : v) * rin_ + bias4[1];
+#pragma unroll
+        for (int h = 0; h < NH; ++h) {
+          if constexpr (F::epi == EPI_GELU) {
+#pragma unroll
+            for (int e = 0; e < 4; e += 2) {
+              const f32x2 g = gelu_bf16_f2(f32x2{x[k][h][e], x[k][h][e + 1]});
+              x[k][h][e] = g[0];
+              x[k][h][e + 1] = g[1];
+            }
+          } else if constexpr (F::epi == EPI_GAMMA_RES) {
+            x[k][h] = r[k][h] + gamma4[h] * x[k][h];
+          } else if constexpr (F::epi == EPI_RES) {
+            x[k][h] = r[k][h] + x[k][h];
+          } else {
+            static_assert(F::epi == EPI_BIAS, "epilogue form");
+          }
+          if (dead) x[k][h] = f32x4{0.f, 0.f, 0.f, 0.f};
+          if constexpr (F::mean == MEAN_MID) x[k][h] = dead ? x[k][h] : m[k][h] + x[k][h];
+          if constexpr (F::mean == MEAN_LAST) x[k][h] = dead ? x[k][h] : (m[k][h] + x[k][h]) / 3.0f;
+        }
+        rsc[k] = osc;
+        if constexpr (h2row) rsc[k] = rbnd[k];
+      }
+      if (rb + IB < ROWS_T) load(rb + IB);
+#pragma unroll
+      for (int k = 0; k < IB; ++k) {
+        const int q = q0 + r0 + trow + (rb + k) * RSTEP;
+        if (!FULL && q >= p.Lq) continue;
+        const long long orow = (long long)q * p.out_mul + ph;
+        const long long o = ob + orow * p.ldy + co;
+        if constexpr (F::mean == MEAN_FIRST || F::mean == MEAN_MID) {
+#pragma unroll
+          for (int h = 0; h < NH; ++h) *reinterpret_cast<f32x4*>(p.macc + o + 4 * h) = x[k][h];
+          continue;
+        }
+        float sc = rsc[k];
+        if constexpr (h2row) {
+          const float bnd = rsc[k];
+          const int sh = h2_shift(bnd);
+          sc = __builtin_ldexpf(1.0f, sh);
+          if (cg == 0 && pr.y_ash) pr.y_ash[(long long)b * p.Lq + q] = sh;
+          if (pr.rflag && !(bnd <= 3.0e38f)) atomicOr(pr.rflag, RANGE_NONFINITE);
+        }
+        if constexpr (F::track) {
+          const float ts = h2row ? sc : 1.0f;
+#pragma unroll
+          for (int h = 0; h < NH; ++h)
+#pragma unroll
+            for (int e = 0; e < 4; ++e) vmax = fmaxf(vmax, fabsf(x[k][h][e]) * ts);
+        }
+        if constexpr (F::y) {
+#pragma unroll
+          for (int h = 0; h < NH; ++h) *reinterpret_cast<f32x4*>(p.y + o + 4 * h) = x[k][h];
+        }
+        float xv[8];
+#pragma unroll
+        for (int e = 0; e < 8; ++e) xv[e] = x[k][e >> 2][e & 3];
+        if constexpr (F::y6h) store_h2_8<false>(y6, orow, p.Cout, co, xv, sc);
+        if constexpr (F::y2 || F::y6sh) {
+          float sv[8];
+#pragma unroll
+          for (int e = 0; e < 8; ++e) sv[e] = silu_f(xv[e]);
+          if constexpr (F::y2) {
+            *reinterpret_cast<f32x4*>(p.y2 + o) = f32x4{sv[0], sv[1], sv[2], sv[3]};
+            *reinterpret_cast<f32x4*>(p.y2 + o + 4) = f32x4{sv[4], sv[5], sv[6], sv[7]};
+          }
+          if constexpr (F::y6sh) store_h2_8<false>(y6s, orow, p.Cout, co, sv, sc);
+        }
+      }
+    }
+  };
+#pragma unroll 1
+  for (int r0 = 0; r0 < BM; r0 += RPP) {
+    if (q0 + r0 + RPP <= p.Lq) pass(r0, std::true_type{});
+    else pass(r0, std::false_type{});
+  }
+  if constexpr (F::track)
+    range_report_wg(vmax, h2row ? nullptr : pr.y_amax, b, h2row ? 65504.0f : h2o ? 65504.0f / osc : __builtin_inff(),
+                    pr.rflag, pre.acur, smem, NT);
+}
+
+template <int BM, int BN, int WM, int WN, int LDS_FLOATS, int NT, int RROW = 2, bool RAG = true, typename F = EpiGeneric,
+          typename AccT>
 __device__ __forceinline__ void epilogue_lds(const ConvParams& p, const ConvParams& pr, AccT& acc, int q0, int co0,
                                              int b, int ph, float* smem, const EpiPre* pre = nullptr) {
+#ifndef DCX_EPI4
+  if constexpr (F::fixed) {
+    epilogue_form<BM, BN, WM, WN, LDS_FLOATS, NT, RROW, RAG, F>(p, pr, acc, q0, co0, b, ph, smem, *pre);
+    return;
+  }
+#endif
   constexpr int WR = BM / WM, WC = BN / WN;
   constexpr int TM = WR / 32, TN = WC / 32;
   constexpr bool M16 = sizeof(acc[0][0]) == 16;
diff --git a/distilcodec_nabeel_amd/csrc/dcx_conv_h3.hip b/distilcodec_nabeel_amd/csrc/dcx_conv_h3.hip
--- a/distilcodec_nabeel_amd/csrc/dcx_conv_h3.hip
+++ b/distilcodec_nabeel_amd/csrc/dcx_conv_h3.hip
@@ -1,3 +1,5 @@
+#include <atomic>
+
 #include "dcx_conv_common.h"
 #include "dcx_conv_launch.h"
 #include "dcx_conv_pingpong.h"
@@ -9,6 +11,45 @@
 DCX_DIAG_FILE(h3)
 
 typedef _Float16 f16x8 __attribute__((ext_vector_type(8)));
+
+using EpiC1 = EpiForm<EPI_BIAS, MEAN_NONE, false, false, false, true, true>;
+using EpiUp = EpiForm<EPI_BIAS, MEAN_NONE, true, false, false, true, true>;
+using EpiC2 = EpiForm<EPI_RES, MEAN_NONE, true, false, false, true, true>;
+using EpiMeanF = EpiForm<EPI_RES, MEAN_FIRST, false, false, false, false, false>;
+using EpiMeanM = EpiForm<EPI_RES, MEAN_MID, false, false, false, false, false>;
+using EpiMeanLH = EpiForm<EPI_RES, MEAN_LAST, false, false, false, true, true>;
+using EpiMeanLF = EpiForm<EPI_RES, MEAN_LAST, false, true, false, false, true>;
+using EpiPw1 = EpiForm<EPI_GELU, MEAN_NONE, false, false, true, false, false, true>;
+using EpiPw2 = EpiForm<EPI_GAMMA_RES, MEAN_NONE, true, false, false, false, false>;
+
+static std::atomic<long long> g_form_launches[kEpiFormCounters];
+template <typename F>
+constexpr int epi_form_id() {
+  return std::is_same_v<F, EpiC1> ? 0 : std::is_same_v<F, EpiUp> ? 1 : std::is_same_v<F, EpiC2> ? 2
+       : std::is_same_v<F, EpiMeanF> ? 3 : std::is_same_v<F, EpiMeanM> ? 4 : std::is_same_v<F, EpiMeanLH> ? 5
+       : std::is_same_v<F, EpiMeanLF> ? 6 : std::is_same_v<F, EpiPw1> ? 7 : std::is_same_v<F, EpiPw2> ? 8
+                                                                                                     : kEpiFormCounters - 1;
+}
+void epi_form_launches(long long* out, bool reset) {
+  for (int i = 0; i < kEpiFormCounters; ++i) out[i] = reset ? g_form_launches[i].exchange(0) : g_form_launches[i].load();
+}
+template <typename... Fs, typename Fn>
+static hipError_t with_epi_form(const ConvParams& p, bool generic, Fn&& f) {
+  hipError_t e = hipSuccess;
+  bool done = false;
+  if (!generic)
+    ((done = done || (epi_form_is<Fs>(p) ? (++g_form_launches[epi_form_id<Fs>()], e = f(Fs{}), true) : false)), ...);
+  if (!done) ++g_form_launches[kEpiFormCounters - 1];
+  return done ? e : f(EpiGeneric{});
+}
+static bool group_generic(const ConvGroup& g) {
+  if (knobs(g.p[0]).epi_generic) return true;
+  for (int k = 1; k < kMaxGroup; ++k)
+    if (g.start[k + 1] > g.start[k] && !(epi_form_is<EpiC1>(g.p[k]) == epi_form_is<EpiC1>(g.p[0]) &&
+                                         epi_form_is<EpiC2>(g.p[k]) == epi_form_is<EpiC2>(g.p[0])))
+      return true;
+  return false;
+}
 
 template <int BM, int BN>
 __device__ __forceinline__ bool ragged_tile_done(const ConvParams& p, const ConvParams& pr, int wg, int b, int ph) {
@@ -141,7 +182,7 @@
   x3dq_tile<BN, 64, RAG>(p, pr, local, b, 0);
 }
 
-template <int HALO, bool SPLIT, int BN = 256, bool RAG = false, bool GROUPED = false>
+template <int HALO, bool SPLIT, int BN = 256, bool RAG = false, bool GROUPED = false, typename F = EpiGeneric>
 __device__ __forceinline__ void x3dw_tile(const ConvParams& p, const ConvParams& pr, const int wg, const int b, const int ph) {
   constexpr int BM = BN == 256 ? 256 : 384, WN = BN / 128, WM = 8 / WN;
   constexpr int WR = BM / WM, WC = 128, TM = WR / 16, TN = WC / 16;
@@ -155,6 +196,7 @@
   static_assert(LDS_B + 16 <= 160 * 1024, "LDS");
   __shared__ __attribute__((aligned(16))) unsigned short lds[LDS_B / 2 + 8];
   unsigned int* const rd_cnt = reinterpret_cast<unsigned int*>(lds + LDS_B / 2);
+  DCX_TILET(tile_t0);
 
   const int tid = threadIdx.x, lane = tid & 63;
   [[maybe_unused]] const int wave = tid >> 6;
@@ -274,6 +316,7 @@
       __builtin_ldexpf(1.0f, -(p.w3_shift + (pr.x_ash ? pr.x_ash[b] : pr.x_ash_c))))));
   asm volatile("s_waitcnt vmcnt(0)" ::: "memory");
   seg_barrier();
+  DCX_TILET(tile_t1);
   in_loop = true;
 #ifdef DCX_SEG_DIAG
   unsigned long long sd[6] = {};
@@ -352,27 +395,29 @@
   }
 #endif
   asm volatile("s_waitcnt vmcnt(0)" ::: "memory");
+  DCX_TILET(tile_t2);
 #pragma unroll
   for (int i = 0; i < TM; ++i)
 #pragma unroll
     for (int j = 0; j < TN; ++j) acc[i][j] *= unscale;
-  epilogue_lds<BM, BN, WM, WN, LDS_B / 4, 512, HALO == 0 ? 3 : 0, RAG>(p, pr, acc, q0, co0, b, ph, reinterpret_cast<float*>(lds), &epre);
-}
-
-template <int HALO, bool SPLIT, int BN = 256, bool RAG = false>
+  epilogue_lds<BM, BN, WM, WN, LDS_B / 4, 512, HALO == 0 ? 3 : 0, RAG, F>(p, pr, acc, q0, co0, b, ph, reinterpret_cast<float*>(lds), &epre);
+  DCX_TILE_END(nsteps);
+}
+
+template <int HALO, bool SPLIT, int BN = 256, bool RAG = false, typename F = EpiGeneric>
 __global__ void __launch_bounds__(512, 2) conv_gemm_x3dw(const ConvParams p) {
   constexpr int BM = BN == 256 ? 256 : 384;
   int wg, b, ph;
   flat_tile(((p.Lq + BM - 1) / BM) * (p.Cout / BN), p.batch, wg, b, ph);
-  x3dw_tile<HALO, SPLIT, BN, RAG>(p, p, wg, b, ph);
-}
-
-template <bool SPLIT, int BN = 256, bool RAG = false>
+  x3dw_tile<HALO, SPLIT, BN, RAG, false, F>(p, p, wg, b, ph);
+}
+
+template <bool SPLIT, int BN = 256, bool RAG = false, typename F = EpiGeneric>
 __global__ void __launch_bounds__(512, 2) conv_gemm_x3dw_group(const ConvGroup g) {
   ConvParams p;
   int local, b;
   const ConvParams& pr = group_member(g, p, local, b);
-  x3dw_tile<64, SPLIT, BN, RAG, true>(p, pr, local, b, 0);
+  x3dw_tile<64, SPLIT, BN, RAG, true, F>(p, pr, local, b, 0);
 }
 
 bool x3dq_ok(const ConvParams& p, int bn, bool wide) {
@@ -410,67 +455,71 @@
 template hipError_t launch_x3dq<256>(const ConvParams&, int, int, hipStream_t, const char**);
 template hipError_t launch_x3dq<128>(const ConvParams&, int, int, hipStream_t, const char**);
 
+template <int BM, int BN, bool RAG>
+static hipError_t launch_x3dw_halo(const ConvParams& p, bool sp, int batch, int phases, hipStream_t s) {
+  if (!sp) {
+    ++g_form_launches[kEpiFormCounters - 1];
+    return launch_flat<BM, BN>(conv_gemm_x3dw<64, false, BN, RAG>, p, batch, phases, 512, s);
+  }
+  return with_epi_form<EpiC1, EpiUp, EpiC2, EpiMeanF, EpiMeanM, EpiMeanLH, EpiMeanLF>(p, knobs(p).epi_generic, [&](auto f) {
+    return launch_flat<BM, BN>(conv_gemm_x3dw<64, true, BN, RAG, decltype(f)>, p, batch, phases, 512, s);
+  });
+}
+
 hipError_t launch_x3dw(const ConvParams& p, int bsel, int batch, int phases, hipStream_t s, const char** kname) {
   const bool sp = knobs(p).h3_split;
-  if (p.clip_len) {
-    if (p.taps == 1) return hipErrorNotSupported;
-    if (bsel == 384) {
-      if (kname) *kname = "conv_gemm_x3dw<384,128,halo>";
-      return sp ? launch_flat<384, 128>(conv_gemm_x3dw<64, true, 128, true>, p, batch, phases, 512, s)
-                : launch_flat<384, 128>(conv_gemm_x3dw<64, false, 128, true>, p, batch, phases, 512, s);
-    }
-    if (kname) *kname = "conv_gemm_x3dw<256,256,halo>";
-    return sp ? launch_flat<256, 256>(conv_gemm_x3dw<64, true, 256, true>, p, batch, phases, 512, s)
-              : launch_flat<256, 256>(conv_gemm_x3dw<64, false, 256, true>, p, batch, phases, 512, s);
-  }
+  if (p.clip_len && p.taps == 1) return hipErrorNotSupported;
   if (bsel == 384) {
     if (kname) *kname = "conv_gemm_x3dw<384,128,halo>";
-    return sp ? launch_flat<384, 128>(conv_gemm_x3dw<64, true, 128>, p, batch, phases, 512, s)
-              : launch_flat<384, 128>(conv_gemm_x3dw<64, false, 128>, p, batch, phases, 512, s);
+    return p.clip_len ? launch_x3dw_halo<384, 128, true>(p, sp, batch, phases, s)
+                      : launch_x3dw_halo<384, 128, false>(p, sp, batch, phases, s);
   }
   if (p.taps == 1) {
     if (kname) *kname = "conv_gemm_x3dw<256,256>";
-    return sp ? launch_flat<256, 256>(conv_gemm_x3dw<0, true>, p, batch, phases, 512, s)
-              : launch_flat<256, 256>(conv_gemm_x3dw<0, false>, p, batch, phases, 512, s);
+    if (!sp) {
+      ++g_form_launches[kEpiFormCounters - 1];
+      return launch_flat<256, 256>(conv_gemm_x3dw<0, false>, p, batch, phases, 512, s);
+    }
+    return with_epi_form<EpiPw1, EpiPw2>(p, knobs(p).epi_generic, [&](auto f) {
+      return launch_flat<256, 256>(conv_gemm_x3dw<0, true, 256, false, decltype(f)>, p, batch, phases, 512, s);
+    });
   }
   if (kname) *kname = "conv_gemm_x3dw<256,256,halo>";
-  return sp ? launch_flat<256, 256>(conv_gemm_x3dw<64, true>, p, batch, phases, 512, s)
-            : launch_flat<256, 256>(conv_gemm_x3dw<64, false>, p, batch, phases, 512, s);
+  return p.clip_len ? launch_x3dw_halo<256, 256, true>(p, sp, batch, phases, s)
+                    : launch_x3dw_halo<256, 256, false>(p, sp, batch, phases, s);
+}
+
+template <int BN, bool RAG>
+static void launch_x3dw_group(const ConvGroup& g, bool split, unsigned blocks, hipStream_t s) {
+  if (!split) {
+    ++g_form_launches[kEpiFormCounters - 1];
+    hipLaunchKernelGGL((conv_gemm_x3dw_group<false, BN, RAG>), dim3(blocks), dim3(512), 0, s, g);
+    return;
+  }
+  (void)with_epi_form<EpiC1, EpiC2>(g.p[0], group_generic(g), [&](auto f) {
+    hipLaunchKernelGGL((conv_gemm_x3dw_group<true, BN, RAG, decltype(f)>), dim3(blocks), dim3(512), 0, s, g);
+    return hipSuccess;
+  });
 }
 
 hipError_t launch_h3_group(const ConvGroup& g, int bsel, bool split, unsigned blocks, hipStream_t s, const char** kname) {
-  if (g.p[0].clip_len) {
-    if (bsel == 384) {
-      if (kname) *kname = "conv_gemm_x3dw_group<384,128,halo>";
-      if (split) hipLaunchKernelGGL((conv_gemm_x3dw_group<true, 128, true>), dim3(blocks), dim3(512), 0, s, g);
-      else hipLaunchKernelGGL((conv_gemm_x3dw_group<false, 128, true>), dim3(blocks), dim3(512), 0, s, g);
-    } else if (bsel == 512) {
-      if (kname) *kname = "conv_gemm_x3dw_group<256,256,halo>";
-      if (split) hipLaunchKernelGGL((conv_gemm_x3dw_group<true, 256, true>), dim3(blocks), dim3(512), 0, s, g);
-      else hipLaunchKernelGGL((conv_gemm_x3dw_group<false, 256, true>), dim3(blocks), dim3(512), 0, s, g);
-    } else if (bsel == 256) {
-      if (kname) *kname = "conv_gemm_x3dq_group<128,256,halo>";
-      hipLaunchKernelGGL((conv_gemm_x3dq_group<256, true>), dim3(blocks), dim3(512), 0, s, g);
-    } else {
-      if (kname) *kname = "conv_gemm_x3dq_group<256,128,halo>";
-      hipLaunchKernelGGL((conv_gemm_x3dq_group<128, true>), dim3(blocks), dim3(512), 0, s, g);
-    }
-    return hipGetLastError();
-  }
+  const bool rag = g.p[0].clip_len != nullptr;
   if (bsel == 384) {
     if (kname) *kname = "conv_gemm_x3dw_group<384,128,halo>";
-    if (split) hipLaunchKernelGGL((conv_gemm_x3dw_group<true, 128>), dim3(blocks), dim3(512), 0, s, g);
-    else hipLaunchKernelGGL((conv_gemm_x3dw_group<false, 128>), dim3(blocks), dim3(512), 0, s, g);
+    if (rag) launch_x3dw_group<128, true>(g, split, blocks, s);
+    else launch_x3dw_group<128, false>(g, split, blocks, s);
   } else if (bsel == 512) {
     if (kname) *kname = "conv_gemm_x3dw_group<256,256,halo>";
-    if (split) hipLaunchKernelGGL(conv_gemm_x3dw_group<true>, dim3(blocks), dim3(512), 0, s, g);
-    else hipLaunchKernelGGL(conv_gemm_x3dw_group<false>, dim3(blocks), dim3(512), 0, s, g);
+    if (rag) launch_x3dw_group<256, true>(g, split, blocks, s);
+    else launch_x3dw_group<256, false>(g, split, blocks, s);
   } else if (bsel == 256) {
     if (kname) *kname = "conv_gemm_x3dq_group<128,256,halo>";
-    hipLaunchKernelGGL((conv_gemm_x3dq_group<256>), dim3(blocks), dim3(512), 0, s, g);
+    if (rag) hipLaunchKernelGGL((conv_gemm_x3dq_group<256, true>), dim3(blocks), dim3(512), 0, s, g);
+    else hipLaunchKernelGGL((conv_gemm_x3dq_group<256>), dim3(blocks), dim3(512), 0, s, g);
   } else {
     if (kname) *kname = "conv_gemm_x3dq_group<256,128,halo>";
-    hipLaunchKernelGGL((conv_gemm_x3dq_group<128>), dim3(blocks), dim3(512), 0, s, g);
+    if (rag) hipLaunchKernelGGL((conv_gemm_x3dq_group<128, true>), dim3(blocks), dim3(512), 0, s, g);
+    else hipLaunchKernelGGL((conv_gemm_x3dq_group<128>), dim3(blocks), dim3(512), 0, s, g);
   }
   return hipGetLastError();
 }
diff --git a/distilcodec_nabeel_amd/csrc/dcx_dispatch.cpp b/distilcodec_nabeel_amd/csrc/dcx_dispatch.cpp
--- a/distilcodec_nabeel_amd/csrc/dcx_dispatch.cpp
+++ b/distilcodec_nabeel_amd/csrc/dcx_dispatch.cpp
@@ -44,7 +44,8 @@
     {"DCX_SPLIT_GROUP_OFF", &dcx::Knobs::split_group_off}, {"DCX_H3", &dcx::Knobs::h3},
     {"DCX_H3_BN", &dcx::Knobs::h3_bn},                    {"DCX_H3_1X1", &dcx::Knobs::h3_1x1},
     {"DCX_H3_SPLIT", &dcx::Knobs::h3_split},              {"DCX_H3_PAIRS", &dcx::Knobs::h3_pairs},
-    {"DCX_RP_RING", &dcx::Knobs::rp_ring},                {"DCX_ENC_STREAMS", &dcx::Knobs::enc_streams}};
+    {"DCX_RP_RING", &dcx::Knobs::rp_ring},                {"DCX_ENC_STREAMS", &dcx::Knobs::enc_streams},
+    {"DCX_EPI_GENERIC", &dcx::Knobs::epi_generic},        {"DCX_CONV_GROUP", &dcx::Knobs::conv_group}};
 
 int dcx::Knobs::*knob_slot(const std::string& n) {
   for (const auto& k : kKnobs)
@@ -309,7 +310,7 @@
     const int rc = run_conv_group_split(h, w, c, p, n, fl, by, s);
     if (rc != 1) return rc;
   }
-  if (same && n > 1) {
+  if (same && n > 1 && h->knobs.conv_group) {
 #ifdef DCX_DIAG_DUP
     if (const int dm = diag_dup_mode()) {
       ConvParams q[dcx::kMaxGroup];
diff --git a/distilcodec_nabeel_amd/csrc/dcx_kernels.h b/distilcodec_nabeel_amd/csrc/dcx_kernels.h
--- a/distilcodec_nabeel_amd/csrc/dcx_kernels.h
+++ b/distilcodec_nabeel_amd/csrc/dcx_kernels.h
@@ -91,6 +91,8 @@
   int h3_pairs = 1;
   int h3_1x1 = 1;
   int rp_ring = 1;
+  int epi_generic = 0;
+  int conv_group = 1;
   int enc_streams = 2;
 };
 
@@ -191,6 +193,8 @@
 hipError_t launch_conv(const ConvParams& p, int batch, int phases, hipStream_t s, const char** kname);
 hipError_t launch_conv_group(const ConvParams* ps, int n, int batch, hipStream_t s, const char** kname);
 hipError_t launch_res_pair(const ResPairParams& p, hipStream_t s, const char** kname);
+constexpr int kEpiFormCounters = 10;
+void epi_form_launches(long long* out, bool reset);
 hipError_t launch_splitk_epilogue(const ConvParams& p, const float* partials, int splits, long long stride, int batch,
                                   int phases, hipStream_t s);
 hipError_t launch_conv_split_group(const ConvParams* ps, int n, int batch, hipStream_t s, const char** kname);
diff --git a/distilcodec_nabeel_amd/engine.py b/distilcodec_nabeel_amd/engine.py
--- a/distilcodec_nabeel_amd/engine.py
+++ b/distilcodec_nabeel_amd/engine.py
@@ -17,7 +17,7 @@
     "DCX_RP_R": 0, "DCX_RP_OLD": 0, "DCX_RP_G64": 0, "DCX_GELU_LUT": -1,
     "DCX_BF16_PERSIST": 1, "DCX_BF16_REG_EPI": 1, "DCX_DWCONV_TILED": 0, "DCX_SPLIT_MIN_STEPS": 0,
     "DCX_SPLIT_GROUP_OFF": 0, "DCX_H3": 1, "DCX_H3_BN": 0, "DCX_H3_1X1": 1, "DCX_H3_SPLIT": 1, "DCX_H3_PAIRS": 1, "DCX_RP_RING": 1,
-    "DCX_ENC_STREAMS": 2,
+    "DCX_ENC_STREAMS": 2, "DCX_EPI_GENERIC": 0, "DCX_CONV_GROUP": 1,
 }
 
 GEMM_MODES = {"f32": _native.DCX_GEMM_F32, "x6": _native.DCX_GEMM_X6, "bf16": _native.DCX_GEMM_BF16}
@@ -151,6 +151,11 @@
             for k, v in saved.items():
                 self.set_knob(k, v)
 
+    def epi_form_launches(self, reset: bool = False) -> list[int]:
+        v = (ctypes.c_int64 * 10)()
+        self._check(self.L.dcx_epi_form_launches(v, 10, int(reset)))
+        return list(v)
+
     def range_flags(self, reset: bool = False) -> int:
         v = ctypes.c_int32(0)
         self._check(self.L.dcx_range_flags(self.h, ctypes.byref(v), int(reset)))
@@ -310,7 +315,10 @@
         self._check(self.L.dcx_module_io(self.h, name.encode(), ctypes.byref(ci), ctypes.byref(co), ctypes.byref(r)))
         return ci.value, co.value, r.value
 
-    def module(self, name: str, x: torch.Tensor) -> torch.Tensor:
+    def module_workspace_size(self, name: str, batch: int, rows: int) -> int:
+        return int(self.L.dcx_module_workspace_size(self.h, name.encode(), batch, rows))
+
+    def module(self, name: str, x: torch.Tensor, ws: torch.Tensor | None = None) -> torch.Tensor:
         cin, cout, rate = self.module_io(name)
         x = self._dev(x, torch.float32)
         if x.ndim != 3 or x.shape[2] != cin:
@@ -324,7 +332,7 @@
             y = torch.empty(B, L, dtype=torch.int32, device=self.device)
         else:
             y = torch.empty(B, L * rate, cout, device=self.device)
-        ws = torch.empty(need, dtype=torch.uint8, device=self.device)
+        ws = torch.empty(need, dtype=torch.uint8, device=self.device) if ws is None else self._workspace_of(need, ws)
         with torch.cuda.device(self.device):
             self._check(self.L.dcx_module_forward(self.h, n, self._ptr(x), B, L, C, self._ptr(y), self._ptr(ws), ws.numel(),
                                                   self._stream()))
@@ -415,3 +423,33 @@
         if rc != _native.DCX_OK:
             raise _native.NativeError(rc, "dcx_conv_forward failed")
         return (y, ys) if want_silu else y
+
+    def forward_h3(self, x: torch.Tensor, want_y: bool = False, want_silu: bool = False, want_silu_h2: bool = False,
+                   want_amax: bool = False, res: torch.Tensor | None = None, in_place: bool = False,
+                   macc: torch.Tensor | None = None, mean: int = 0, lens: torch.Tensor | None = None) -> dict:
+        B, L, C = x.shape
+        assert C == self.cin and x.is_cuda and x.dtype == torch.float32 and x.is_contiguous() and self.stride == 1
+        dev = x.device
+        out = {}
+        if want_y:
+            out["y"] = res if in_place else torch.empty(B, L, self.cout, device=dev)
+        if want_silu:
+            out["y_silu"] = torch.empty(B, L, self.cout, device=dev)
+        if want_silu_h2:
+            out["y_silu_h2"] = torch.zeros(B, L, self.cout * 2, dtype=torch.int16, device=dev)
+            out["y_ash"] = torch.zeros(B, dtype=torch.int32, device=dev)
+        if want_amax:
+            out["y_amax"] = torch.zeros(B, device=dev)
+        keep = [res.abs().amax(dim=(1, 2)).contiguous() if res is not None else None,
+                macc.abs().amax(dim=(1, 2)).contiguous() if macc is not None and mean >= 2 else None]
+        ptr = lambda t: t.data_ptr() if t is not None else None
+        o = _native.ConvH3Out(ptr(out.get("y")), ptr(out.get("y_silu")), ptr(out.get("y_silu_h2")), ptr(out.get("y_ash")),
+                              ptr(out.get("y_amax")), ptr(res), ptr(keep[0]), ptr(macc), ptr(keep[1]), ptr(lens),
+                              3 if res is not None else 0, mean)
+        rc = self.L.dcx_conv_forward_h3(self.h, ctypes.c_void_p(x.data_ptr()), B, L, ctypes.byref(o),
+                                        ctypes.c_void_p(torch.cuda.current_stream(dev).cuda_stream))
+        if rc != _native.DCX_OK:
+            raise _native.NativeError(rc, "dcx_conv_forward_h3 failed")
+        if macc is not None:
+            out["macc"] = macc
+        return out
diff --git a/include/distilcodec_amd.h b/include/distilcodec_amd.h
--- a/include/distilcodec_amd.h
+++ b/include/distilcodec_amd.h
@@ -129,6 +129,21 @@
                      float* y_silu, const float* res, int32_t epi, void* stream);
 void dcx_conv_destroy(dcx_conv* c);
 const char* dcx_conv_last_kernel(const dcx_conv* c);
+typedef struct dcx_conv_h3_out {
+  float* y;
+  float* y_silu;
+  uint16_t* y_silu_h2;
+  int32_t* y_ash;
+  float* y_amax;
+  const float* res;
+  const float* res_amax;
+  float* macc;
+  const float* macc_amax;
+  const int32_t* lens;
+  int32_t epi, mean;
+} dcx_conv_h3_out;
+int dcx_conv_forward_h3(dcx_conv* c, const float* x, int32_t batch, int64_t lin, const dcx_conv_h3_out* o, void* stream);
+int dcx_epi_form_launches(int64_t* counts, int32_t n, int32_t reset);
 int dcx_conv_set_knob(dcx_conv* c, const char* name, int32_t value);
 int dcx_conv_set_h3(dcx_conv* c, int32_t on);
 
```

New measurement: 52.47 million (median of 6 runs). 2.8% higher.
